# autosome-ru/pasio

Measured on NVIDIA B200. Metric: whole-contig segmentation throughput, default pasio pipeline (nt/s); DP cell updates/s in dp_cells_per_s, higher is better.
Workload: dtype f64

## Files before the change

include/pasio_b200.h:

```cpp
#ifndef PASIO_B200_H
#define PASIO_B200_H

#include <stdint.h>

#ifdef __cplusplus
extern "C" {
#endif

typedef struct pasio_ctx pasio_ctx;

typedef enum pasio_status {
    PASIO_OK = 0,
    PASIO_E_CUDA = -1,
    PASIO_E_ARG = -2,
    PASIO_E_COUNTS = -3,
    PASIO_E_CANDIDATES = -4,
    PASIO_E_TABLE_TOO_SHORT = -5,
    PASIO_E_STATE = -6,
    PASIO_E_TOO_LARGE = -7,
    PASIO_E_NOMEM = -8
} pasio_status;

enum { PASIO_TAB_LOG = 0,
       PASIO_TAB_LGAMMA = 1,
       PASIO_TAB_LGAMMA_ALPHA = 2   };

enum { PASIO_CONSTRAINT_NONE = 0, PASIO_CONSTRAINT_ZEROS = 1, PASIO_CONSTRAINT_CONSTANTS = 2 };

enum { PASIO_TUNE_WINDOW_PRUNE = 0,
       PASIO_TUNE_WINDOW_PHASES = 1,
       PASIO_TUNE_EXACT_PRUNE = 2,
       PASIO_TUNE_EXACT_LAG = 3,
       PASIO_TUNE_EXACT_RING = 4,
       PASIO_TUNE_LOGFAC_EXACT = 5,
       PASIO_TUNE_WINDOW_SPECULATE = 6,
       PASIO_TUNE_UPLOAD_NARROW = 7,
       PASIO_TUNE_LOGFAC_EAGER = 8,
       PASIO_TUNE_EXACT_NBLOCK = 9,
       PASIO_TUNE_COUNT = 10 };

int pasio_ctx_create(int device, pasio_ctx **out);
int pasio_ctx_destroy(pasio_ctx *ctx);
const char *pasio_last_error(const pasio_ctx *ctx);
int pasio_abi_version(void);

int pasio_set_params(pasio_ctx *ctx, int alpha_is_int, double alpha, double beta,
                     double segment_creation_cost);
int pasio_table_upload(pasio_ctx *ctx, int table_id, const double *values, int64_t n);
int pasio_table_need(const pasio_ctx *ctx, int64_t *n_log, int64_t *n_lgamma, int64_t *n_lgamma_alpha);

int pasio_contig_load(pasio_ctx *ctx, const int64_t *counts, int64_t n,
                      const int64_t *offsets, int64_t n_contigs);
int pasio_contig_load_rle(pasio_ctx *ctx, const int64_t *starts, const int64_t *values,
                          int64_t n_runs, const int64_t *offsets, int64_t n_contigs);
int pasio_contig_load_round(pasio_ctx *ctx, const int64_t *counts, int64_t n, int64_t window_size,
                            int64_t window_shift, int constraint, int64_t *n_in, int64_t *n_out, int64_t *cells);

int pasio_contig_load_device(pasio_ctx *ctx, const int64_t *d_counts_device, int64_t n,
                             const int64_t *offsets, int64_t n_contigs);
int pasio_contig_info(const pasio_ctx *ctx, int64_t *n, int64_t *total_count, int64_t *n_contigs);
int pasio_cumsum_at(pasio_ctx *ctx, const int64_t *positions, int64_t m, int64_t *out);

int pasio_candidates_set(pasio_ctx *ctx, const int64_t *cands, int64_t m);
int pasio_candidates_count(const pasio_ctx *ctx, int64_t *m);
int pasio_candidates_download(pasio_ctx *ctx, int64_t *out, int64_t capacity, int64_t *m);

int pasio_filter_candidates(pasio_ctx *ctx, int constraint, int64_t *n_in, int64_t *n_out);

int pasio_round(pasio_ctx *ctx, int64_t window_size, int64_t window_shift, int constraint,
                int64_t *n_in, int64_t *n_out, int64_t *cells);
int pasio_round_stats(const pasio_ctx *ctx, int64_t *cells, int64_t *cells_skipped);
int pasio_exact_task_plan(int64_t n_candidates, int lag, int nblock, int32_t *triples, int64_t cap, int64_t *n_tasks);
int pasio_upload_stats(const pasio_ctx *ctx, int64_t *wire_bytes);
int pasio_set_tuning(pasio_ctx *ctx, int key, int value);
int pasio_rounds(pasio_ctx *ctx, int64_t window_size, int64_t window_shift, int constraint,
                 int64_t max_rounds, int64_t *rounds_done, int64_t *n_out, int64_t *cells,
                 int64_t *sizes, int64_t sizes_cap);
int pasio_set_penalties(pasio_ctx *ctx, const double *split_number_penalty, int64_t n_split_number_penalty,
                        double first_column_refund, const double *length_penalty, int64_t n_length_penalty);

int pasio_square_split(pasio_ctx *ctx, int64_t *out_splits, int64_t cap, int64_t *n_splits,
                       double *score, double *prefix_scores, int64_t *previous_splits);
int pasio_square_split_regularized(pasio_ctx *ctx, const double *length_penalty, int64_t n_length_penalty,
                                   const double *split_number_penalty, int64_t n_split_number_penalty,
                                   double first_column_refund, int64_t *out_splits, int64_t cap, int64_t *n_splits,
                                   double *score, double *prefix_scores, int64_t *previous_splits);
int pasio_suffix_scores(pasio_ctx *ctx, int64_t stop, double *out);

int pasio_segment_scores(pasio_ctx *ctx, double *scores, int64_t *segment_counts,
                         double *mean_counts, double *logfac_cumsum, int64_t capacity,
                         int64_t *n_segments);

int pasio_segment_scores_sum(pasio_ctx *ctx, double *total);

int pasio_segment_lmm(pasio_ctx *ctx, double *lmm, int64_t capacity, double *sum_logfac);
int pasio_logfac_prefetch(pasio_ctx *ctx);

int pasio_host_alloc(int64_t bytes, void **out);
int pasio_host_free(void *ptr);

int64_t pasio_bedgraph_runs(const int64_t *starts, const int64_t *stops, const int64_t *counts,
                            const uint8_t *new_chrom, int64_t n, int split_at_gaps, int64_t *run_len,
                            int64_t *run_val, int64_t *group_line, int64_t *group_run, int64_t *n_runs);

int64_t pasio_bedgraph_count_lines(const char *buf, int64_t len);
int pasio_bedgraph_parse(const char *buf, int64_t len, int64_t cap, int64_t *starts, int64_t *stops,
                         int64_t *counts, int64_t *name_off, int32_t *name_len, uint8_t *new_chrom,
                         int64_t *n_out, int64_t *float_counts);
int64_t pasio_format_segments(const char *chrom, int64_t offset, const int64_t *splits, int64_t n_splits,
                              const double *means, const double *lmm, int mode, char *out, int64_t cap);

int64_t pasio_format_segments_batch(const char *names, const int64_t *name_off, const int64_t *shift,
                                    const int64_t *first_split, int64_t n_contigs, const int64_t *splits,
                                    const double *means, const double *lmm, int mode, char *out, int64_t cap);


int pasio_timing_reset(pasio_ctx *ctx, int enable);
void *pasio_stream(pasio_ctx *ctx);
int pasio_fp64_peak(pasio_ctx *ctx, double *instr_per_sec);
int pasio_timing_get(pasio_ctx *ctx, int family, double *ms, int64_t *launches);

#ifdef __cplusplus
}
#endif
#endif
```

pasio_b200/_native.py:

```python
import ctypes
import os
import threading

import numpy as np

_HERE = os.path.dirname(os.path.abspath(__file__))
LIB_PATH = os.environ.get('PASIO_B200_LIB') or os.path.join(_HERE, 'libpasio_b200.so')

OK = 0
E_CUDA, E_ARG, E_COUNTS, E_CANDIDATES, E_TABLE_TOO_SHORT, E_STATE, E_TOO_LARGE, E_NOMEM = range(-1, -9, -1)
TAB_LOG, TAB_LGAMMA, TAB_LGAMMA_ALPHA = 0, 1, 2
CONSTRAINTS = {'none': 0, 'zeros': 1, 'constants': 2}
TUNE = {'window_prune': 0, 'window_phases': 1, 'exact_prune': 2, 'exact_lag': 3, 'exact_ring': 4, 'logfac_exact': 5,
        'window_speculate': 6, 'upload_narrow': 7,
        'logfac_eager': 8, 'exact_nblock': 9}
TIMING_FAMILIES = ['scan', 'window_dp', 'compact', 'exact_dp', 'score', 'h2d', 'd2h']

_i64 = ctypes.c_int64
_i64p = ctypes.POINTER(ctypes.c_int64)
_f64p = ctypes.POINTER(ctypes.c_double)
_vp = ctypes.c_void_p

SIGNATURES = {
    'pasio_ctx_create': (ctypes.c_int, [ctypes.c_int, ctypes.POINTER(_vp)]),
    'pasio_ctx_destroy': (ctypes.c_int, [_vp]),
    'pasio_last_error': (ctypes.c_char_p, [_vp]),
    'pasio_abi_version': (ctypes.c_int, []),
    'pasio_set_params': (ctypes.c_int, [_vp, ctypes.c_int, ctypes.c_double, ctypes.c_double, ctypes.c_double]),
    'pasio_table_upload': (ctypes.c_int, [_vp, ctypes.c_int, _f64p, _i64]),
    'pasio_table_need': (ctypes.c_int, [_vp, _i64p, _i64p, _i64p]),
    'pasio_contig_load': (ctypes.c_int, [_vp, _i64p, _i64, _i64p, _i64]),
    'pasio_contig_load_round': (ctypes.c_int, [_vp, _i64p, _i64, _i64, _i64, ctypes.c_int, _i64p, _i64p, _i64p]),
    'pasio_contig_load_rle': (ctypes.c_int, [_vp, _i64p, _i64p, _i64, _i64p, _i64]),
    'pasio_contig_load_device': (ctypes.c_int, [_vp, _vp, _i64, _i64p, _i64]),
    'pasio_contig_info': (ctypes.c_int, [_vp, _i64p, _i64p, _i64p]),
    'pasio_cumsum_at': (ctypes.c_int, [_vp, _i64p, _i64, _i64p]),
    'pasio_candidates_set': (ctypes.c_int, [_vp, _i64p, _i64]),
    'pasio_candidates_count': (ctypes.c_int, [_vp, _i64p]),
    'pasio_candidates_download': (ctypes.c_int, [_vp, _i64p, _i64, _i64p]),
    'pasio_filter_candidates': (ctypes.c_int, [_vp, ctypes.c_int, _i64p, _i64p]),
    'pasio_round': (ctypes.c_int, [_vp, _i64, _i64, ctypes.c_int, _i64p, _i64p, _i64p]),
    'pasio_round_stats': (ctypes.c_int, [_vp, _i64p, _i64p]),
    'pasio_exact_task_plan': (ctypes.c_int, [_i64, ctypes.c_int, ctypes.c_int, ctypes.POINTER(ctypes.c_int32), _i64, _i64p]),
    'pasio_upload_stats': (ctypes.c_int, [_vp, _i64p]),
    'pasio_set_tuning': (ctypes.c_int, [_vp, ctypes.c_int, ctypes.c_int]),
    'pasio_rounds': (ctypes.c_int, [_vp, _i64, _i64, ctypes.c_int, _i64, _i64p, _i64p, _i64p, _i64p, _i64]),
    'pasio_set_penalties': (ctypes.c_int, [_vp, _f64p, _i64, ctypes.c_double, _f64p, _i64]),
    'pasio_square_split': (ctypes.c_int, [_vp, _i64p, _i64, _i64p, _f64p, _f64p, _i64p]),
    'pasio_square_split_regularized': (ctypes.c_int, [_vp, _f64p, _i64, _f64p, _i64, ctypes.c_double, _i64p, _i64, _i64p, _f64p,
                                                     _f64p, _i64p]),
    'pasio_suffix_scores': (ctypes.c_int, [_vp, _i64, _f64p]),
    'pasio_segment_scores': (ctypes.c_int, [_vp, _f64p, _i64p, _f64p, _f64p, _i64, _i64p]),
    'pasio_segment_scores_sum': (ctypes.c_int, [_vp, _f64p]),
    'pasio_segment_lmm': (ctypes.c_int, [_vp, _f64p, _i64, _f64p]),
    'pasio_logfac_prefetch': (ctypes.c_int, [_vp]),
    'pasio_host_alloc': (ctypes.c_int, [_i64, ctypes.POINTER(_vp)]),
    'pasio_host_free': (ctypes.c_int, [_vp]),
    'pasio_bedgraph_count_lines': (_i64, [ctypes.c_void_p, _i64]),
    'pasio_bedgraph_parse': (ctypes.c_int, [ctypes.c_void_p, _i64, _i64, _i64p, _i64p, _i64p, _i64p,
                                            ctypes.POINTER(ctypes.c_int32), ctypes.POINTER(ctypes.c_uint8), _i64p, _i64p]),
    'pasio_bedgraph_runs': (_i64, [_i64p, _i64p, _i64p, ctypes.POINTER(ctypes.c_uint8), _i64, ctypes.c_int, _i64p, _i64p, _i64p,
                                   _i64p, _i64p]),
    'pasio_format_segments': (_i64, [ctypes.c_char_p, _i64, _i64p, _i64, _f64p, _f64p, ctypes.c_int,
                                     ctypes.c_char_p, _i64]),
    'pasio_format_segments_batch': (_i64, [ctypes.c_char_p, _i64p, _i64p, _i64p, _i64, _i64p, _f64p, _f64p, ctypes.c_int,
                                           ctypes.c_char_p, _i64]),
    'pasio_timing_reset': (ctypes.c_int, [_vp, ctypes.c_int]),
    'pasio_timing_get': (ctypes.c_int, [_vp, ctypes.c_int, _f64p, _i64p]),
    'pasio_stream': (_vp, [_vp]),
    'pasio_fp64_peak': (ctypes.c_int, [_vp, _f64p]),
}

_lib = None
_lib_lock = threading.Lock()


def load_library():
    global _lib
    with _lib_lock:
        if _lib is None:
            if not os.path.exists(LIB_PATH):
                raise RuntimeError('pasio_b200: %s is missing -- build it with `python -c "import __graft_entry__ as g; '
                                   'g.build()"` or `make -C pasio_b200/csrc`; there is no CPU fallback' % LIB_PATH)
            lib = ctypes.CDLL(LIB_PATH)
            for name, (res, args) in SIGNATURES.items():
                fn = getattr(lib, name)
                fn.restype = res
                fn.argtypes = args
            _lib = lib
    return _lib


def _ptr(arr, ct):
    return arr.ctypes.data_as(ctypes.POINTER(ct))


class PasioDeviceError(RuntimeError):
    pass


class _PinnedPool(object):

    def __init__(self, lib):
        self.lib = lib
        self.free = {}
        self.lock = threading.Lock()
        self.total = 0

    @staticmethod
    def _capacity(nbytes):
        cap = 1 << 16
        while cap < nbytes:
            cap <<= 1
        return cap

    def empty(self, n, dtype):
        import weakref
        dtype = np.dtype(dtype)
        nbytes = max(1, int(n) * dtype.itemsize)
        cap = self._capacity(nbytes)
        with self.lock:
            bucket = self.free.get(cap)
            ptr = bucket.pop() if bucket else None
        if ptr is None:
            if self.total + cap > (8 << 30):
                return np.empty(int(n), dtype=dtype)
            out = _vp()
            if self.lib.pasio_host_alloc(cap, ctypes.byref(out)) != OK:
                return np.empty(int(n), dtype=dtype)
            ptr = out.value
            self.total += cap
        buf = (ctypes.c_char * cap).from_address(ptr)
        arr = np.frombuffer(buf, dtype=dtype, count=int(n))
        weakref.finalize(buf, self._give_back, cap, ptr)
        return arr

    def _give_back(self, cap, ptr):
        with self.lock:
            self.free.setdefault(cap, []).append(ptr)


class Engine(object):

    def __init__(self, device=0):
        self.lib = load_library()
        handle = _vp()
        rc = self.lib.pasio_ctx_create(int(device), ctypes.byref(handle))
        if rc != OK:
            raise PasioDeviceError('pasio_b200: cannot create a device context (%s); the LogML path has no CPU '
                                   'fallback' % self.lib.pasio_last_error(None).decode())
        self.ctx = handle
        self.device = device
        self._params = None
        self._tables = {}
        self._scorer_source = None
        self._penalty_spec = None
        self._penalties = None
        self._penalty_host = None
        self._loaded = None
        self._loaded_print = None
        self._cands_print = None
        self._loaded_offsets = None
        self._cands_obj = None
        self._pool = _PinnedPool(self.lib)

    def close(self):
        if self.ctx:
            self.lib.pasio_ctx_destroy(self.ctx)
            self.ctx = None

    def _check(self, rc):
        if rc == OK:
            return
        msg = self.lib.pasio_last_error(self.ctx).decode()
        if rc in (E_COUNTS, E_CANDIDATES):
            raise AssertionError(msg)
        if rc == E_ARG:
            raise ValueError(msg)
        if rc == E_NOMEM:
            raise MemoryError(msg)
        raise PasioDeviceError('pasio_b200 error %d: %s' % (rc, msg))

    def use_scorer(self, source, penalties=None):
        alpha = source.alpha
        is_int = isinstance(alpha, (int, np.integer)) and not isinstance(alpha, bool)
        params = (int(is_int), float(alpha), float(source.log_computer.shift), float(source.segment_creation_cost))
        if params != self._params:
            self._check(self.lib.pasio_set_params(self.ctx, *params))
            self._params = params
        comps = {TAB_LOG: source.log_computer, TAB_LGAMMA: source.log_gamma_computer,
                 TAB_LGAMMA_ALPHA: source.log_gamma_alpha_computer}
        for tid, comp in comps.items():
            have = self._tables.get(tid)
            if have is None or have[0] is not comp:
                self._upload_table(tid, comp, comp.cache_size)
# ... 47 lines not shown
        n = len(arr)
        if n == 0:
            return (0,)
        step = max(1, n // 4096)
        return (n, int(arr[0]), int(arr[-1]), int(np.asarray(arr[::step]).sum()))

    def load(self, counts, offsets=None):
        if (self._loaded is counts and offsets is None and self._loaded_offsets is None
                and self._loaded_print == self._fingerprint(counts)):
            return
        assert isinstance(counts, np.ndarray)
        assert counts.dtype == int
        assert len(counts) > 0
        c = np.ascontiguousarray(counts)
        self._loaded = None
        self._cands_obj = None
        if offsets is None:
            rc = self.lib.pasio_contig_load(self.ctx, _ptr(c, ctypes.c_int64), len(c), None, 1)
        else:
            off = np.ascontiguousarray(offsets, dtype=np.int64)
            rc = self.lib.pasio_contig_load(self.ctx, _ptr(c, ctypes.c_int64), len(c), _ptr(off, ctypes.c_int64),
                                            len(off) - 1)
        self._check(rc)
        self._loaded = counts
        self._loaded_print = self._fingerprint(counts)
        self._loaded_offsets = None if offsets is None else np.array(offsets, dtype=np.int64)

    def load_and_round(self, counts, window_size, window_shift, constraint, want_logfac=False):
        assert isinstance(counts, np.ndarray)
        assert counts.dtype == int
        assert len(counts) > 0
        c = np.ascontiguousarray(counts)
        self._loaded = None
        self._cands_obj = None
        n_in, n_out, cells = _i64(0), _i64(0), _i64(0)
        self.set_tuning('logfac_eager', 1 if want_logfac else 0)
        self._sync_penalties()
        try:
            rc = self.lib.pasio_contig_load_round(self.ctx, _ptr(c, ctypes.c_int64), len(c), window_size, window_shift,
                                                  CONSTRAINTS[constraint], ctypes.byref(n_in), ctypes.byref(n_out),
                                                  ctypes.byref(cells))
        finally:
            if want_logfac:
                self.set_tuning('logfac_eager', 0)
        if rc != E_TABLE_TOO_SHORT:
            self._check(rc)
        self._loaded = counts
        self._loaded_print = self._fingerprint(counts)
        self._loaded_offsets = None
        if rc == E_TABLE_TOO_SHORT:
            self._grow_tables()
            return self.round(window_size, window_shift, constraint)
        return n_in.value, n_out.value, cells.value

    def load_device(self, device_ptr, n, owner=None, offsets=None):
        self._loaded = None
        self._cands_obj = None
        if offsets is None:
            rc = self.lib.pasio_contig_load_device(self.ctx, _vp(device_ptr), n, None, 1)
        else:
            off = np.ascontiguousarray(offsets, dtype=np.int64)
            rc = self.lib.pasio_contig_load_device(self.ctx, _vp(device_ptr), n, _ptr(off, ctypes.c_int64), len(off) - 1)
        self._check(rc)
        self._loaded = owner if owner is not None else object()
        self._loaded_offsets = None if offsets is None else np.array(offsets, dtype=np.int64)

    def invalidate(self):
        self._loaded = None
        self._cands_obj = None

    def stream_handle(self):
        return self.lib.pasio_stream(self.ctx)

    def fp64_peak(self):
        v = ctypes.c_double(0)
        self._check(self.lib.pasio_fp64_peak(self.ctx, ctypes.byref(v)))
        return v.value

    def load_rle(self, starts, values, offsets=None):
        starts = np.ascontiguousarray(starts, dtype=np.int64)
        values = np.ascontiguousarray(values, dtype=np.int64)
        self._loaded = None
        self._cands_obj = None
        if offsets is None:
            rc = self.lib.pasio_contig_load_rle(self.ctx, _ptr(starts, ctypes.c_int64), _ptr(values, ctypes.c_int64),
                                                len(values), None, 1)
        else:
            off = np.ascontiguousarray(offsets, dtype=np.int64)
            rc = self.lib.pasio_contig_load_rle(self.ctx, _ptr(starts, ctypes.c_int64), _ptr(values, ctypes.c_int64),
                                                len(values), _ptr(off, ctypes.c_int64), len(off) - 1)
        self._check(rc)
        self._loaded = object()
        self._loaded_offsets = None if offsets is None else np.array(offsets, dtype=np.int64)

    def info(self):
        n, total, k = _i64(0), _i64(0), _i64(0)
        self._check(self.lib.pasio_contig_info(self.ctx, ctypes.byref(n), ctypes.byref(total), ctypes.byref(k)))
        return n.value, total.value, k.value

    def set_candidates(self, cands):
        if cands is None:
            self._check(self.lib.pasio_candidates_set(self.ctx, None, 0))
            self._cands_obj = None
            return
        if self._cands_obj is cands and self._cands_print == self._fingerprint(cands):
            return
        c = np.ascontiguousarray(cands, dtype=np.int64)
        self._cands_obj = None
        self._check(self.lib.pasio_candidates_set(self.ctx, _ptr(c, ctypes.c_int64), len(c)))
        self._cands_obj = cands
        self._cands_print = self._fingerprint(cands)

    def candidates(self):
        m = _i64(0)
        self._check(self.lib.pasio_candidates_count(self.ctx, ctypes.byref(m)))
        out = self._pool.empty(m.value, np.int64)
        self._check(self.lib.pasio_candidates_download(self.ctx, _ptr(out, ctypes.c_int64), len(out), None))
        self._cands_obj = out
        self._cands_print = self._fingerprint(out)
        return out

    def candidate_count(self):
        m = _i64(0)
        self._check(self.lib.pasio_candidates_count(self.ctx, ctypes.byref(m)))
        return m.value

    def filter_candidates(self, constraint):
        a, b = _i64(0), _i64(0)
        self._cands_obj = None
        self._check(self.lib.pasio_filter_candidates(self.ctx, CONSTRAINTS[constraint], ctypes.byref(a), ctypes.byref(b)))
        return a.value, b.value

    def round(self, window_size, window_shift, constraint):
        n_in, n_out, cells = _i64(0), _i64(0), _i64(0)
        self._cands_obj = None
        self._sync_penalties()
        self._retry(lambda: self.lib.pasio_round(self.ctx, window_size, window_shift, CONSTRAINTS[constraint],
                                                 ctypes.byref(n_in), ctypes.byref(n_out), ctypes.byref(cells)))
        return n_in.value, n_out.value, cells.value

    def set_tuning(self, key, value):
        self._check(self.lib.pasio_set_tuning(self.ctx, TUNE[key], int(value)))

    def upload_stats(self):
        b = _i64(0)
        self._check(self.lib.pasio_upload_stats(self.ctx, ctypes.byref(b)))
        return b.value

    def round_stats(self):
        a, b = _i64(0), _i64(0)
        self._check(self.lib.pasio_round_stats(self.ctx, ctypes.byref(a), ctypes.byref(b)))
        return a.value, b.value

    def rounds(self, window_size, window_shift, constraint, num_rounds=None, first=None):
        n, _, _ = self.info()
        limit = max(1, n if num_rounds is None else num_rounds)
        self._cands_obj = None
        sizes, cells_total = [], 0
        if first is not None:
            sizes.append(first[0])
            cells_total += first[2]
            limit -= 1
            if first[0] == first[1] or limit == 0:
                return sizes, self.candidate_count(), cells_total
        while limit > 0:
            done, n_out, cells = _i64(0), _i64(0), _i64(0)
            buf = np.zeros(64, dtype=np.int64)
            step = min(limit, 64)
            self._sync_penalties()
            rc = self.lib.pasio_rounds(self.ctx, window_size, window_shift, CONSTRAINTS[constraint], step,
                                       ctypes.byref(done), ctypes.byref(n_out), ctypes.byref(cells),
                                       _ptr(buf, ctypes.c_int64), len(buf))
            sizes.extend(buf[:done.value].tolist())
            cells_total += cells.value
            limit -= done.value
            if rc == E_TABLE_TOO_SHORT:
                self._grow_tables()
                continue
            self._check(rc)
            if done.value < step or (done.value > 0 and sizes[-1] == n_out.value):
                break
        return sizes, self.candidate_count(), cells_total

    def _check_exact_limits(self):
        n, total, _ = self.info()
        if total + (self._params[1] if self._params else 0) >= 2 ** 31 - 2:
            raise PasioDeviceError('pasio_b200: the exact SquareSplitter DP over a whole contig needs the total count (%d) below '
                                   '2^31; use the default `rounds` algorithm for deep-coverage contigs' % total)

    def square_split(self, want_arrays=False):
        self._check_exact_limits()
        m = self.candidate_count()
        splits = np.empty(m, dtype=np.int64)
        n_splits, score = _i64(0), ctypes.c_double(0.0)
        P = np.empty(m) if want_arrays else None
        prev = np.empty(m, dtype=np.int64) if want_arrays else None
        self._cands_obj = None
        self._retry(lambda: self.lib.pasio_square_split(
            self.ctx, _ptr(splits, ctypes.c_int64), m, ctypes.byref(n_splits), ctypes.byref(score),
            _ptr(P, ctypes.c_double) if want_arrays else None,
            _ptr(prev, ctypes.c_int64) if want_arrays else None))
        out = splits[:n_splits.value].copy()
        self._cands_obj = out
        self._cands_print = self._fingerprint(out)
        if want_arrays:
            return np.float64(score.value), out, P, prev
        return np.float64(score.value), out

    def square_split_regularized(self, length_penalty=None, split_number_penalty=None, first_column_refund=0.0):
        self._check_exact_limits()
        m = self.candidate_count()
        splits = np.empty(m, dtype=np.int64)
        n_splits, score = _i64(0), ctypes.c_double(0.0)
        lp = None if length_penalty is None else np.ascontiguousarray(length_penalty, dtype=np.float64)
        sp = None if split_number_penalty is None else np.ascontiguousarray(split_number_penalty, dtype=np.float64)
        self._cands_obj = None
        self._retry(lambda: self.lib.pasio_square_split_regularized(
            self.ctx, None if lp is None else _ptr(lp, ctypes.c_double), 0 if lp is None else len(lp),
            None if sp is None else _ptr(sp, ctypes.c_double), 0 if sp is None else len(sp), float(first_column_refund),
            _ptr(splits, ctypes.c_int64), m, ctypes.byref(n_splits), ctypes.byref(score), None, None))
        out = splits[:n_splits.value].copy()
        self._cands_obj = out
        self._cands_print = self._fingerprint(out)
        return np.float64(score.value), out

    def suffix_scores(self, stop):
        out = np.empty(stop)
        if stop > 0:
            self._retry(lambda: self.lib.pasio_suffix_scores(self.ctx, stop, _ptr(out, ctypes.c_double)))
        return out

    def cumsum_at_candidates(self):
        m = self.candidate_count()
        out = np.empty(m, dtype=np.int64)
        self._check(self.lib.pasio_cumsum_at(self.ctx, None, m, _ptr(out, ctypes.c_int64)))
        return out

    def segment_scores(self, scores=True, counts=False, means=False, logfac=False):
        m = self.candidate_count()
        nseg = m - 1
        s = self._pool.empty(nseg, np.float64) if scores else None
        c = self._pool.empty(nseg, np.int64) if counts else None
        mu = self._pool.empty(nseg, np.float64) if means else None
        lf = self._pool.empty(m, np.float64) if logfac else None
        nout = _i64(0)
        self._retry(lambda: self.lib.pasio_segment_scores(
            self.ctx, _ptr(s, ctypes.c_double) if scores else None, _ptr(c, ctypes.c_int64) if counts else None,
            _ptr(mu, ctypes.c_double) if means else None, _ptr(lf, ctypes.c_double) if logfac else None,
            max(nseg, m if logfac else 0), ctypes.byref(nout)))
        return s, c, mu, lf

    def segment_scores_sum(self):
        total = ctypes.c_double(0.0)
        self._retry(lambda: self.lib.pasio_segment_scores_sum(self.ctx, ctypes.byref(total)))
        return np.float64(total.value)

    def logfac_prefetch(self):
        self._check(self.lib.pasio_logfac_prefetch(self.ctx))

    def segment_lmm(self):
        nseg = self.candidate_count() - 1
        out = self._pool.empty(nseg, np.float64)
        total = ctypes.c_double(0.0)
        self._retry(lambda: self.lib.pasio_segment_lmm(self.ctx, _ptr(out, ctypes.c_double), nseg, ctypes.byref(total)))
        return out, total.value

    def timing_reset(self, enable=True):
        self._check(self.lib.pasio_timing_reset(self.ctx, int(enable)))

    def timing(self):
        out = {}
        for k, name in enumerate(TIMING_FAMILIES):
            ms, n = ctypes.c_double(0), _i64(0)
            self._check(self.lib.pasio_timing_get(self.ctx, k, ctypes.byref(ms), ctypes.byref(n)))
            out[name] = (ms.value, n.value)
        return out


def parse_bedgraph_text(data, front=0, length=None):
    lib = load_library()
    nbytes = len(data) if length is None else int(length)
    if isinstance(data, bytearray):
        data = (ctypes.c_char * len(data)).from_buffer(data) if len(data) else None
    cap = lib.pasio_bedgraph_count_lines(data, nbytes)
    starts = np.empty(front + cap, dtype=np.int64)
    stops = np.empty(front + cap, dtype=np.int64)
    counts = np.empty(front + cap, dtype=np.int64)
    name_off = np.empty(front + cap, dtype=np.int64)
    name_len = np.empty(front + cap, dtype=np.int32)
    new_chrom = np.empty(front + cap, dtype=np.uint8)
    n, nfloat = _i64(0), _i64(0)
    rc = lib.pasio_bedgraph_parse(data, nbytes, cap, _ptr(starts[front:], ctypes.c_int64), _ptr(stops[front:], ctypes.c_int64),
                                  _ptr(counts[front:], ctypes.c_int64), _ptr(name_off[front:], ctypes.c_int64),
                                  _ptr(name_len[front:], ctypes.c_int32), _ptr(new_chrom[front:], ctypes.c_uint8),
                                  ctypes.byref(n), ctypes.byref(nfloat))
    if rc != OK:
        raise ValueError('malformed bedgraph line %d (need: chrom start stop count)' % (n.value + 1))
    k = front + n.value
    return dict(starts=starts[:k], stops=stops[:k], counts=counts[:k], name_off=name_off[:k], name_len=name_len[:k],
                new_chrom=new_chrom[:k], n_float=nfloat.value)


def bedgraph_runs(rec, split_at_gaps):
    lib = load_library()
    n = len(rec['starts'])
    run_len = np.empty(2 * n, dtype=np.int64)
# ... 87 lines not shown
```

pasio_b200/csrc/api.cu:

```cuda
#include "common.cuh"

#include <algorithm>
#include <thread>
#include <atomic>
#include <chrono>
#include <memory>
#include <cstdarg>
#include <cstdlib>
#include <cstdio>
#include <cstring>

static thread_local std::string g_create_error;

int pasio_fail(pasio_ctx *ctx, int code, const char *fmt, ...)
{
    char buf[512];
    va_list ap;
    va_start(ap, fmt);
    vsnprintf(buf, sizeof buf, fmt, ap);
    va_end(ap);
    if (ctx) ctx->err = buf; else g_create_error = buf;
    return code;
}

// ... 234 lines not shown
    }

    void work(int t)
    {
        cudaSetDevice(ctx->device);
        bool used[2] = {false, false};
        int which = 0;
        while (!cancel.load(std::memory_order_relaxed)) {
            const i64 sidx = next_slice.fetch_add(1);
            if (sidx >= n_slices) break;
            const i64 e0 = sidx * (i64)SLICE, e1 = std::min<i64>(n, e0 + (i64)SLICE), len = e1 - e0;
            const int buf = 2 * t + which;
            which ^= 1;
            int32_t *hst = (int32_t *)ctx->nstage_host + (size_t)buf * SLICE;
            int32_t *dev = (int32_t *)ctx->nstage_dev + (size_t)buf * SLICE;
            i64 *dst = ctx->counts.as<i64>() + e0;
            bool ok = true;
            if (plain_mode.load(std::memory_order_relaxed)) {
                ok = cudaMemcpyAsync(dst, src + e0, (size_t)len * 8, cudaMemcpyHostToDevice, ctx->stream_copy) == cudaSuccess;
                wire_bytes.fetch_add(len * 8);
                which ^= 1;
                if (!ok) { cudaGetLastError(); failed.store(1); cancel.store(1); }
                const i64 qp = e0 / chunk_elems;
                if (left_in_chunk[(size_t)qp].fetch_sub(1) == 1) {
                    if (cudaEventRecord(ctx->chunk_events[(size_t)qp], ctx->stream_copy) != cudaSuccess) { cudaGetLastError(); failed.store(1); }
                    recorded[(size_t)qp].store(1, std::memory_order_release);
                }
                continue;
            }
            if (used[buf & 1]) ok = cudaEventSynchronize(ctx->nstage_free[(size_t)buf]) == cudaSuccess;
            const uint64_t bits = ok ? pasio_narrow_slice8(reinterpret_cast<uint8_t *>(hst), src + e0, (size_t)len) : 0;
            const bool sw = limit_bits < 25;
            const int lim8 = sw ? limit_bits : 8, lim16 = sw ? limit_bits + 3 : 16, lim32 = sw ? limit_bits + 6 : 31;
            if (ok && (bits >> lim8) == 0 && (len & 15) == 0) {
                ok = cudaMemcpyAsync(dev, hst, (size_t)len, cudaMemcpyHostToDevice, ctx->stream_copy) == cudaSuccess;
                if (ok) {
                    ok = cudaEventRecord(ctx->nstage_free[(size_t)buf], ctx->stream_copy) == cudaSuccess;
                    used[buf & 1] = true;
                    const i64 n16 = len / 16;
                    widen_counts8_kernel<<<(unsigned)std::min<i64>((n16 + 255) / 256, 296), 256, 0, ctx->stream_copy>>>(
                        reinterpret_cast<const uint4 *>(dev), reinterpret_cast<longlong2 *>(dst), n16);
                    ok = ok && cudaGetLastError() == cudaSuccess;
                    wire_bytes.fetch_add(len);
                }
            } else if (ok && (bits >> lim16) == 0 && (len & 7) == 0) {
                pasio_narrow_slice16(reinterpret_cast<uint16_t *>(hst), src + e0, (size_t)len);
                ok = cudaMemcpyAsync(dev, hst, (size_t)len * 2, cudaMemcpyHostToDevice, ctx->stream_copy) == cudaSuccess;
                if (ok) {
                    ok = cudaEventRecord(ctx->nstage_free[(size_t)buf], ctx->stream_copy) == cudaSuccess;
                    used[buf & 1] = true;
                    const i64 n8 = len / 8;
                    widen_counts16_kernel<<<(unsigned)std::min<i64>((n8 + 255) / 256, 296), 256, 0, ctx->stream_copy>>>(
                        reinterpret_cast<const uint4 *>(dev), reinterpret_cast<longlong2 *>(dst), n8);
                    ok = ok && cudaGetLastError() == cudaSuccess;
                    wire_bytes.fetch_add(len * 2);
                }
            } else if (ok && (bits >> lim32) == 0 && (len & 3) == 0) {
                narrow_slice(hst, src + e0, (size_t)len);
                ok = cudaMemcpyAsync(dev, hst, (size_t)len * 4, cudaMemcpyHostToDevice, ctx->stream_copy) == cudaSuccess;
                if (ok) {
                    ok = cudaEventRecord(ctx->nstage_free[(size_t)buf], ctx->stream_copy) == cudaSuccess;
                    used[buf & 1] = true;
                    const i64 n4 = len / 4;
                    widen_counts_kernel<<<(unsigned)std::min<i64>((n4 + 255) / 256, 296), 256, 0, ctx->stream_copy>>>(
                        reinterpret_cast<const int4 *>(dev), reinterpret_cast<longlong2 *>(dst), n4);
                    ok = ok && cudaGetLastError() == cudaSuccess;
                    wire_bytes.fetch_add(len * 4);
                }
            } else if (ok) {
                ok = cudaMemcpyAsync(dst, src + e0, (size_t)len * 8, cudaMemcpyHostToDevice, ctx->stream_copy) == cudaSuccess;
                wire_bytes.fetch_add(len * 8);
            }
            if (!ok) { cudaGetLastError(); failed.store(1); cancel.store(1); }
            if (src_pinned && packed_elems.fetch_add(len) + len >= ((i64)64 << 20) && !decided.exchange(1)) {
                const double secs = std::chrono::duration<double>(std::chrono::steady_clock::now() - t_start).count();
                if ((double)packed_elems.load() * 8.0 < PLAIN_RATE * secs) plain_mode.store(1);
            }
            const i64 q = e0 / chunk_elems;
            if (left_in_chunk[(size_t)q].fetch_sub(1) == 1) {
                if (cudaEventRecord(ctx->chunk_events[(size_t)q], ctx->stream_copy) != cudaSuccess) { cudaGetLastError(); failed.store(1); }
                recorded[(size_t)q].store(1, std::memory_order_release);
            }
        }
    }

    bool wait_recorded(i64 q)
    {
        while (!recorded[(size_t)q].load(std::memory_order_acquire)) {
            if (failed.load() || cancel.load()) return false;
            std::this_thread::sleep_for(std::chrono::microseconds(20));
        }
        return !failed.load();
    }

    void finish()
    {
        for (auto &th : threads) th.join();
        threads.clear();
    }
    ~NarrowUpload()
    {
        if (!threads.empty()) { cancel.store(1); finish(); }
    }
};
}

static void drop_borrowed_counts(pasio_ctx *ctx)
{
    if (ctx->counts_borrowed) { ctx->counts.p = nullptr; ctx->counts.bytes = 0; ctx->counts_borrowed = false; }
}

#define NEED_CTX(ctx) do { if (!(ctx)) return PASIO_E_ARG; cudaSetDevice((ctx)->device); } while (0)

extern "C" int pasio_abi_version(void) { return PASIO_ABI_VERSION; }

extern "C" const char *pasio_last_error(const pasio_ctx *ctx)
{
    return ctx ? ctx->err.c_str() : g_create_error.c_str();
}

extern "C" int pasio_ctx_create(int device, pasio_ctx **out)
{
    if (!out) return pasio_fail(nullptr, PASIO_E_ARG, "out is NULL");
    *out = nullptr;
    int count = 0;
    cudaError_t e = cudaGetDeviceCount(&count);
    if (e != cudaSuccess || count == 0)
        return pasio_fail(nullptr, PASIO_E_CUDA, "no CUDA device: %s (pasio_b200 has no CPU fallback)",
                          e != cudaSuccess ? cudaGetErrorString(e) : "device count is 0");
    if (device < 0 || device >= count)
        return pasio_fail(nullptr, PASIO_E_ARG, "device %d out of range (have %d)", device, count);
    cudaDeviceProp prop;
    e = cudaGetDeviceProperties(&prop, device);
    if (e != cudaSuccess) return pasio_fail(nullptr, PASIO_E_CUDA, "cudaGetDeviceProperties: %s", cudaGetErrorString(e));
    if (prop.major != 10)
        return pasio_fail(nullptr, PASIO_E_CUDA, "device %d is sm_%d%d; this library is built for sm_100a only",
                          device, prop.major, prop.minor);
    e = cudaSetDevice(device);
    if (e != cudaSuccess) return pasio_fail(nullptr, PASIO_E_CUDA, "cudaSetDevice: %s", cudaGetErrorString(e));
    pasio_ctx *ctx = new pasio_ctx();
    ctx->device = device;
    ctx->sm_count = prop.multiProcessorCount;
    ctx->smem_optin = (int)prop.sharedMemPerBlockOptin;
    int prio_lo = 0, prio_hi = 0;
    cudaDeviceGetStreamPriorityRange(&prio_lo, &prio_hi);
    if (cudaStreamCreateWithPriority(&ctx->stream, cudaStreamNonBlocking, prio_hi) != cudaSuccess ||
        cudaStreamCreateWithPriority(&ctx->stream2, cudaStreamNonBlocking, 0) != cudaSuccess ||
        cudaStreamCreateWithFlags(&ctx->stream_copy, cudaStreamNonBlocking) != cudaSuccess ||
        cudaStreamCreateWithPriority(&ctx->stream_lx, cudaStreamNonBlocking, 0) != cudaSuccess ||
        cudaEventCreateWithFlags(&ctx->ev_lx0, cudaEventDisableTiming) != cudaSuccess ||
        cudaEventCreateWithFlags(&ctx->ev_lx1, cudaEventDisableTiming) != cudaSuccess ||
        cudaEventCreateWithFlags(&ctx->ev_fork, cudaEventDisableTiming) != cudaSuccess ||
        cudaEventCreateWithFlags(&ctx->ev_join, cudaEventDisableTiming) != cudaSuccess ||
        cudaMallocHost((void **)&ctx->h_scalars, 16 * sizeof(i64)) != cudaSuccess ||
        pasio_reserve(ctx, ctx->scalars, 16 * sizeof(i64)) != PASIO_OK) {
        g_create_error = "context allocation failed: " + ctx->err;
        delete ctx;
        return PASIO_E_CUDA;
    }
    memset(ctx->h_scalars, 0, 16 * sizeof(i64));
    auto env_int = [](const char *name, int dflt) { const char *v = getenv(name); return v ? atoi(v) : dflt; };
    ctx->tune[PASIO_TUNE_WINDOW_PRUNE] = env_int("PASIO_WD_PRUNE", 1);
    ctx->tune[PASIO_TUNE_WINDOW_PHASES] = env_int("PASIO_WD_PHASES", 1);
    ctx->tune[PASIO_TUNE_EXACT_PRUNE] = env_int("PASIO_XD_PRUNE", 1);
    ctx->tune[PASIO_TUNE_EXACT_LAG] = env_int("PASIO_XD_LAG", 5);
    ctx->tune[PASIO_TUNE_EXACT_RING] = env_int("PASIO_XD_RING", 1);
    ctx->tune[PASIO_TUNE_LOGFAC_EXACT] = env_int("PASIO_B200_EXACT_LMM", 1);
    ctx->tune[PASIO_TUNE_WINDOW_SPECULATE] = env_int("PASIO_WD_SPECULATE", 1);
    ctx->tune[PASIO_TUNE_UPLOAD_NARROW] = env_int("PASIO_B200_UPLOAD_NARROW", 1);
    ctx->tune[PASIO_TUNE_LOGFAC_EAGER] = env_int("PASIO_B200_LOGFAC_EAGER", 0);
    ctx->tune[PASIO_TUNE_EXACT_NBLOCK] = env_int("PASIO_XD_NBLOCK", 3);
    if (ctx->tune[PASIO_TUNE_EXACT_LAG] < 3 || ctx->tune[PASIO_TUNE_EXACT_LAG] > 5) ctx->tune[PASIO_TUNE_EXACT_LAG] = 5;
    *out = ctx;
    return PASIO_OK;
}

extern "C" int pasio_ctx_destroy(pasio_ctx *ctx)
{
    if (!ctx) return PASIO_OK;
    cudaSetDevice(ctx->device);
    cudaStreamSynchronize(ctx->stream);
    drop_borrowed_counts(ctx);
    DevBuf *bufs[] = {&ctx->tab[0], &ctx->tab[1], &ctx->tab[2], &ctx->counts, &ctx->cg, &ctx->cpbits, &ctx->keepbits,
                      &ctx->bounds, &ctx->brank, &ctx->cand[0], &ctx->cand[1], &ctx->candC[0], &ctx->candC[1], &ctx->win_st, &ctx->win_en, &ctx->win_small, &ctx->win_medium, &ctx->win_large, &ctx->win_flags,
                      &ctx->blocksum, &ctx->tilestate, &ctx->scalars, &ctx->dpL, &ctx->dpC, &ctx->dpP, &ctx->dpPrev,
                      &ctx->dpPart, &ctx->dpPartArg, &ctx->dpMark, &ctx->dpJump, &ctx->fscan, &ctx->logfac_full,
                      &ctx->xpRing, &ctx->xpRec, &ctx->xpTasks, &ctx->regLR, &ctx->regNR, &ctx->lxPos, &ctx->lxSum, &ctx->lxFirst, &ctx->lxState};
    for (DevBuf *b : bufs) if (b->p) cudaFree(b->p);
    for (auto &s : ctx->spans) { cudaEventDestroy(s.a); cudaEventDestroy(s.b); }
    for (auto e : ctx->event_pool) cudaEventDestroy(e);
    if (ctx->h_scalars) cudaFreeHost(ctx->h_scalars);
    for (int k = 0; k < 3; ++k) {
        if (ctx->stage[k]) cudaFreeHost(ctx->stage[k]);
        if (k == 0) {
            if (ctx->nstage_host) cudaFreeHost(ctx->nstage_host);
            if (ctx->nstage_dev) cudaFree(ctx->nstage_dev);
            for (cudaEvent_t e : ctx->nstage_free) cudaEventDestroy(e);
        }
        if (ctx->stage_free[k]) cudaEventDestroy(ctx->stage_free[k]);
    }
    if (ctx->ev_fork) cudaEventDestroy(ctx->ev_fork);
    if (ctx->ev_join) cudaEventDestroy(ctx->ev_join);
    if (ctx->stream2) cudaStreamDestroy(ctx->stream2);
    if (ctx->stream_copy) cudaStreamDestroy(ctx->stream_copy);
    if (ctx->stream_lx) { cudaStreamSynchronize(ctx->stream_lx); cudaStreamDestroy(ctx->stream_lx); }
    if (ctx->ev_lx0) cudaEventDestroy(ctx->ev_lx0);
    if (ctx->ev_lx1) cudaEventDestroy(ctx->ev_lx1);
    for (auto e : ctx->chunk_events) cudaEventDestroy(e);
    cudaStreamDestroy(ctx->stream);
    delete ctx;
    return PASIO_OK;
}

extern "C" int pasio_set_params(pasio_ctx *ctx, int alpha_is_int, double alpha, double beta, double pen)
{
    NEED_CTX(ctx);
    if (!(alpha >= 0) || !(beta >= 0)) return pasio_fail(ctx, PASIO_E_ARG, "alpha and beta must be >= 0");
    if (alpha_is_int && (alpha != (double)(i64)alpha || alpha > 1e9))
        return pasio_fail(ctx, PASIO_E_ARG, "alpha_is_int set but alpha=%g is not a small integer", alpha);
    ctx->alpha_is_int = alpha_is_int ? 1 : 0;
    ctx->alpha = alpha;
    ctx->alpha_int = alpha_is_int ? (i64)alpha : 0;
    ctx->beta = beta;
    ctx->pen = pen;
    ctx->have_params = true;
    return PASIO_OK;
}

extern "C" int pasio_table_upload(pasio_ctx *ctx, int id, const double *values, int64_t n)
{
    NEED_CTX(ctx);
    if (id < 0 || id > 2 || !values || n < 1) return pasio_fail(ctx, PASIO_E_ARG, "bad table upload (id=%d n=%lld)", id, (long long)n);
    PASIO_TRY(pasio_reserve(ctx, ctx->tab[id], (size_t)n * 8));
    PASIO_TRY(h2d(ctx, ctx->tab[id].p, values, (size_t)n * 8));
    CUDA_TRY(ctx, cudaStreamSynchronize(ctx->stream));
    ctx->ntab[id] = n;
    return PASIO_OK;
}

extern "C" int pasio_table_need(const pasio_ctx *ctx, int64_t *n_log, int64_t *n_lgamma, int64_t *n_lgamma_alpha)
{
    if (!ctx) return PASIO_E_ARG;
    if (n_log) *n_log = ctx->need[PASIO_TAB_LOG];
    if (n_lgamma) *n_lgamma = ctx->need[PASIO_TAB_LGAMMA];
    if (n_lgamma_alpha) *n_lgamma_alpha = ctx->need[PASIO_TAB_LGAMMA_ALPHA];
    return PASIO_OK;
}

static bool penalties_on(const pasio_ctx *ctx) { return ctx->pen_num || ctx->pen_len; }

static int check_dp_tables(pasio_ctx *ctx, i64 max_span, i64 max_cnt, bool with_penalties = false)
{
    if (!ctx->have_params) return pasio_fail(ctx, PASIO_E_STATE, "pasio_set_params has not been called");
    if (max_cnt + ctx->alpha_int >= 2147483647LL)
        return pasio_fail(ctx, PASIO_E_TOO_LARGE, "count %lld does not fit the 32-bit DP index", (long long)max_cnt);
    const i64 need_log = max_span + 1;
    const int gid = ctx->alpha_is_int ? PASIO_TAB_LGAMMA : PASIO_TAB_LGAMMA_ALPHA;
    const i64 need_g = max_cnt + ctx->alpha_int + 1;
    bool bad = false;
    if (ctx->ntab[PASIO_TAB_LOG] < need_log) { ctx->need[PASIO_TAB_LOG] = need_log; bad = true; }
    if (ctx->ntab[gid] < need_g) { ctx->need[gid] = need_g; bad = true; }
    if (with_penalties && ctx->pen_len && ctx->n_pen_lr < need_log) { ctx->need[PASIO_TAB_LOG] = need_log; bad = true; }
    if (bad)
        return pasio_fail(ctx, PASIO_E_TABLE_TOO_SHORT, "tables too short: need log>=%lld, lgamma[%d]>=%lld (have %lld, %lld%s)",
                          (long long)need_log, gid, (long long)need_g, (long long)ctx->ntab[PASIO_TAB_LOG],
                          (long long)ctx->ntab[gid], with_penalties && ctx->pen_len ? ", length penalty as long as log" : "");
    return PASIO_OK;
}

extern "C" int pasio_set_penalties(pasio_ctx *ctx, const double *split_number_penalty, int64_t n_split_number_penalty,
                                   double first_column_refund, const double *length_penalty, int64_t n_length_penalty)
{
    NEED_CTX(ctx);
    if ((split_number_penalty && n_split_number_penalty < 1) || (length_penalty && n_length_penalty < 1))
        return pasio_fail(ctx, PASIO_E_ARG, "a penalty table needs at least one entry");
    ctx->pen_num = ctx->pen_len = false;
    if (split_number_penalty) {
        PASIO_TRY(pasio_reserve(ctx, ctx->penNR, (size_t)n_split_number_penalty * 8));
        PASIO_TRY(h2d(ctx, ctx->penNR.p, split_number_penalty, (size_t)n_split_number_penalty * 8));
    }
    if (length_penalty) {
        PASIO_TRY(pasio_reserve(ctx, ctx->penLR, (size_t)n_length_penalty * 8));
        PASIO_TRY(h2d(ctx, ctx->penLR.p, length_penalty, (size_t)n_length_penalty * 8));
    }
    CUDA_TRY(ctx, cudaStreamSynchronize(ctx->stream));
    ctx->pen_num = split_number_penalty != nullptr;
    ctx->n_pen_nr = ctx->pen_num ? n_split_number_penalty : 0;
    ctx->pen_refund = ctx->pen_num ? first_column_refund : 0.0;
    ctx->pen_len = length_penalty != nullptr;
    ctx->n_pen_lr = ctx->pen_len ? n_length_penalty : 0;
    return PASIO_OK;
}

static int finish_load(pasio_ctx *ctx, const int64_t *offsets, int64_t n_contigs)
{
    const i64 n = ctx->n;
    ctx->h_bounds.resize((size_t)n_contigs + 1);
    if (offsets) {
        for (i64 c = 0; c <= n_contigs; ++c) {
            if (offsets[c] < 0 || offsets[c] > n || (c > 0 && offsets[c] <= offsets[c - 1]))
                return pasio_fail(ctx, PASIO_E_ARG, "contig offsets must be strictly ascending within [0, n] (empty contigs are not allowed)");
            ctx->h_bounds[(size_t)c] = (int32_t)offsets[c];
        }
        if (offsets[0] != 0 || offsets[n_contigs] != n)
            return pasio_fail(ctx, PASIO_E_ARG, "offsets[0] must be 0 and offsets[n_contigs] must be n");
    } else {
        ctx->h_bounds[0] = 0;
        ctx->h_bounds[1] = (int32_t)n;
    }
    ctx->n_contigs = n_contigs;
    const size_t bit_bytes = (size_t)((n + 1 + 4095) / 4096) * 512 + 16;
    PASIO_TRY(pasio_reserve(ctx, ctx->cg, (size_t)(n + 2) * 8));
    PASIO_TRY(pasio_reserve(ctx, ctx->cpbits, bit_bytes));
// ... 120 lines not shown
    if (window_size < 1 || window_shift < 1 || window_size > 2147483000LL || window_shift > 2147483000LL)
        return pasio_fail(ctx, PASIO_E_ARG, "window_size and window_shift must be positive");
    if (constraint < 0 || constraint > 2) return pasio_fail(ctx, PASIO_E_ARG, "unknown constraint %d", constraint);
    PASIO_TRY(check_load_args(ctx, n, nullptr, 1));
    ctx->n = n;
    drop_borrowed_counts(ctx);
    PASIO_TRY(pasio_reserve(ctx, ctx->counts, (size_t)n * 8 + 16));
    ctx->h_bounds.assign({0, (int32_t)n});
    ctx->n_contigs = 1;
    const size_t bit_alloc = (size_t)((n + 1 + 4095) / 4096) * 512 + 16;
    PASIO_TRY(pasio_reserve(ctx, ctx->cg, (size_t)(n + 2) * 8));
    PASIO_TRY(pasio_reserve(ctx, ctx->cpbits, bit_alloc));
    PASIO_TRY(pasio_reserve(ctx, ctx->keepbits, bit_alloc));
    PASIO_TRY(pasio_reserve(ctx, ctx->bounds, 2 * 4));
    PASIO_TRY(pasio_reserve(ctx, ctx->brank, 2 * 4));
    PASIO_TRY(h2d(ctx, ctx->bounds.p, ctx->h_bounds.data(), 2 * 4));
    const size_t bit_bytes = (size_t)((n + 1 + 31) / 32 + 2) * 4;
    CUDA_TRY(ctx, cudaMemsetAsync(ctx->keepbits.p, 0, bit_bytes, ctx->stream));
    i64 n_tiles = 0, tile_elems = 0;
    PASIO_TRY(launch_scan_prepare(ctx, &n_tiles, &tile_elems));
    ctx->implicit_all = true;
    ctx->m = n + 1;
    ctx->cur = 0;
    ctx->n_small = ctx->n_medium = ctx->n_large = -1;

    const i64 chunk_tiles = (i64)(32 << 20) / tile_elems;
    const i64 n_chunks = (n_tiles + chunk_tiles - 1) / chunk_tiles;
    while ((i64)ctx->chunk_events.size() < n_chunks) {
        cudaEvent_t e;
        CUDA_TRY(ctx, cudaEventCreateWithFlags(&e, cudaEventDisableTiming));
        ctx->chunk_events.push_back(e);
    }
    CUDA_TRY(ctx, cudaEventRecord(ctx->ev_fork, ctx->stream));
    CUDA_TRY(ctx, cudaStreamWaitEvent(ctx->stream_copy, ctx->ev_fork, 0));
    i64 queued = 0;
    auto queue_copies = [&](i64 upto) -> int {
        for (; queued < upto && queued < n_chunks; ++queued) {
            const i64 e0 = queued * chunk_tiles * tile_elems, e1 = std::min<i64>(n, (queued + 1) * chunk_tiles * tile_elems);
            if (e1 > e0) {
                TimingScope ts(ctx, TF_H2D, 1, ctx->stream_copy);
                PASIO_TRY(upload(ctx, ctx->counts.as<i64>() + e0, counts + e0, (size_t)(e1 - e0) * 8, ctx->stream_copy));
            }
            CUDA_TRY(ctx, cudaEventRecord(ctx->chunk_events[(size_t)queued], ctx->stream_copy));
        }
        return PASIO_OK;
    };

    const bool eager = ctx->tune[PASIO_TUNE_LOGFAC_EXACT] && ctx->tune[PASIO_TUNE_LOGFAC_EAGER] && ctx->ntab[PASIO_TAB_LGAMMA] > 2;
    if (eager) {
        CUDA_TRY(ctx, cudaStreamWaitEvent(ctx->stream_lx, ctx->ev_fork, 0));
        PASIO_TRY(launch_logfac_exact_begin(ctx, ctx->stream_lx));
    }
    NarrowUpload narrow;
    std::unique_ptr<TimingScope> narrow_span;
    bool narrow_on = false;
    if (ctx->tune[PASIO_TUNE_UPLOAD_NARROW] && n >= ((i64)1 << 24) && (chunk_tiles * tile_elems) % (i64)NarrowUpload::SLICE == 0) {
        narrow_span.reset(new TimingScope(ctx, TF_H2D, 1, ctx->stream_copy));
        if (ctx->tune[PASIO_TUNE_UPLOAD_NARROW] >= 2 && ctx->tune[PASIO_TUNE_UPLOAD_NARROW] < 31) narrow.limit_bits = ctx->tune[PASIO_TUNE_UPLOAD_NARROW];
        narrow_on = narrow.start(ctx, counts, n, chunk_tiles * tile_elems, n_chunks) == 0;
        if (!narrow_on) narrow_span.reset();
    }
    auto stop_upload = [&]() {
        if (narrow_on) { narrow.cancel.store(1); narrow.finish(); narrow_span.reset(); }
        if (eager) cudaStreamSynchronize(ctx->stream_lx);
    };

    const i64 nwin_total = (ctx->m - 1 + window_shift - 1) / window_shift;
    i64 w_done = 0;
    int table_rc = ctx->have_params ? PASIO_OK : pasio_fail(ctx, PASIO_E_STATE, "pasio_set_params has not been called");
    bool first_dp = true;
    for (i64 c = 0; c < n_chunks; ++c) {
        if (narrow_on) {
            if (!narrow.wait_recorded(c)) {
                stop_upload();
                cudaStreamSynchronize(ctx->stream_copy);
                return pasio_fail(ctx, PASIO_E_CUDA, "narrowed upload failed: %s", cudaGetErrorString(cudaGetLastError()));
            }
        } else {
            PASIO_TRY(queue_copies(c + 3));
        }
        CUDA_TRY(ctx, cudaStreamWaitEvent(ctx->stream, ctx->chunk_events[(size_t)c], 0));
        if (eager) {
            CUDA_TRY(ctx, cudaStreamWaitEvent(ctx->stream_lx, ctx->chunk_events[(size_t)c], 0));
            PASIO_TRY(launch_logfac_exact_chunk(ctx, c * chunk_tiles * tile_elems, std::min<i64>(n, (c + 1) * chunk_tiles * tile_elems),
                                                ctx->stream_lx));
        }
        const i64 t1 = std::min<i64>(n_tiles, (c + 1) * chunk_tiles);
        PASIO_TRY(launch_scan_tiles(ctx, t1 - c * chunk_tiles));
        const i64 scanned = t1 * tile_elems;
        i64 w_ready = nwin_total;
        if (c + 1 < n_chunks) {
            w_ready = scanned > window_size ? (scanned - window_size - 1) / window_shift + 1 : 0;
            if (w_ready > nwin_total) w_ready = nwin_total;
        }
        if (table_rc == PASIO_OK && w_ready > w_done) {
            i64 max_span = 0, max_cnt = 0;
            CUDA_TRY(ctx, cudaMemcpyAsync(ctx->h_scalars + 1, ctx->scalars.as<i64>() + 1, 8, cudaMemcpyDeviceToHost, ctx->stream));
            PASIO_TRY(launch_window_prepass(ctx, w_ready - w_done, (int)window_size, (int)window_shift, &max_span, &max_cnt,
                                            constraint, w_done));
            if (ctx->h_scalars[1]) {
                stop_upload();
                cudaStreamSynchronize(ctx->stream_copy);
                return pasio_fail(ctx, PASIO_E_COUNTS, "counts must be >= 0");
            }
            table_rc = check_dp_tables(ctx, max_span, max_cnt, true);
            if (table_rc == PASIO_OK) {
                if (penalties_on(ctx))
                    PASIO_TRY(launch_window_dp_reg(ctx, w_ready - w_done, (int)window_size, (int)window_shift, constraint, !first_dp));
                else
                    PASIO_TRY(launch_window_dp(ctx, w_ready - w_done, (int)window_size, (int)window_shift, constraint, w_done,
                                               !first_dp));
                first_dp = false;
            } else if (table_rc != PASIO_E_TABLE_TOO_SHORT) {
                return table_rc;
            }
            w_done = w_ready;
        }
    }
    if (narrow_on) {
        narrow.finish();
        narrow_span.reset();
        ctx->last_wire_bytes = narrow.wire_bytes.load();
        if (narrow.failed.load()) {
            cudaStreamSynchronize(ctx->stream_copy);
            return pasio_fail(ctx, PASIO_E_CUDA, "narrowed upload failed: %s", cudaGetErrorString(cudaGetLastError()));
        }
    } else {
        ctx->last_wire_bytes = n * 8;
    }
    PASIO_TRY(d2h(ctx, ctx->h_scalars, ctx->scalars.p, 3 * sizeof(i64)));
    CUDA_TRY(ctx, cudaStreamSynchronize(ctx->stream_copy));
    if (ctx->h_scalars[1]) return pasio_fail(ctx, PASIO_E_COUNTS, "counts must be >= 0");
    ctx->total = ctx->h_scalars[0];
    ctx->max_count = ctx->h_scalars[2];
    ctx->have_contig = true;
    if (eager) {
        CUDA_TRY(ctx, cudaEventRecord(ctx->ev_lx1, ctx->stream_lx));
        ctx->logfac_ready = true;
        ctx->logfac_is_exact = true;
        ctx->logfac_pending = true;
        ctx->logfac_eager = true;
    }
    PASIO_TRY(launch_boundary_ranks(ctx));
    ctx->h_brank = ctx->h_bounds;
    if (n_in) *n_in = ctx->m;
    if (n_out) *n_out = ctx->m;
    if (cells) *cells = 0;
    if (table_rc != PASIO_OK) return table_rc;

    const int nxt = 1 - ctx->cur;
    PASIO_TRY(pasio_reserve(ctx, ctx->cand[nxt], (size_t)ctx->m * 4));
    i64 m_new = 0;
    PASIO_TRY(launch_compact_keepbits(ctx, nxt, &m_new));
    PASIO_TRY(d2h(ctx, ctx->h_scalars + 10, ctx->scalars.as<i64>() + 10, 24));
    if (cells) *cells = ctx->h_scalars[10];
    ctx->last_cells = ctx->h_scalars[10];
    ctx->last_cells_skipped = ctx->h_scalars[12];
    ctx->cur = nxt;
    ctx->implicit_all = false;
    ctx->m = m_new;
    if (n_out) *n_out = m_new;
    return refresh_boundary_ranks(ctx);
}

extern "C" int pasio_contig_info(const pasio_ctx *ctx, int64_t *n, int64_t *total_count, int64_t *n_contigs)
{
    if (!ctx || !ctx->have_contig) return PASIO_E_STATE;
    if (n) *n = ctx->n;
    if (total_count) *total_count = ctx->total;
    if (n_contigs) *n_contigs = ctx->n_contigs;
    return PASIO_OK;
}

extern "C" int pasio_cumsum_at(pasio_ctx *ctx, const int64_t *positions, int64_t m, int64_t *out)
{
    NEED_CTX(ctx);
    if (!ctx->have_contig) return pasio_fail(ctx, PASIO_E_STATE, "no contig loaded");
    if (m < 0 || !out) return pasio_fail(ctx, PASIO_E_ARG, "bad arguments");
    if (m == 0) return PASIO_OK;
    PASIO_TRY(pasio_reserve(ctx, ctx->dpP, (size_t)m * 8));
    if (positions) {
        for (i64 k = 0; k < m; ++k)
            if (positions[k] < 0 || positions[k] > ctx->n) return pasio_fail(ctx, PASIO_E_ARG, "position out of range");
        PASIO_TRY(pasio_reserve(ctx, ctx->dpJump, (size_t)m * 8));
        PASIO_TRY(h2d(ctx, ctx->dpJump.p, positions, (size_t)m * 8));
        PASIO_TRY(launch_gather_i64(ctx, ctx->cg.as<i64>(), nullptr, ctx->dpJump.as<i64>(), m, ctx->dpP.as<i64>()));
    } else {
        if (m != ctx->m) return pasio_fail(ctx, PASIO_E_ARG, "m must equal the candidate count");
        PASIO_TRY(launch_gather_i64(ctx, ctx->cg.as<i64>(), cur_cand(ctx), nullptr, m, ctx->dpP.as<i64>()));
    }
    return d2h(ctx, out, ctx->dpP.p, (size_t)m * 8);
}

__global__ void narrow_candidates_kernel(const i64 *__restrict__ in, i64 m, i64 n, int32_t *__restrict__ out, i64 *bad)
{
    for (i64 k = (i64)blockIdx.x * blockDim.x + threadIdx.x; k < m; k += (i64)gridDim.x * blockDim.x) {
        i64 v = in[k];
        if (v < 0 || v > n) { *bad = 1; v = 0; }
        out[k] = (int32_t)v;
    }
}

static int refresh_boundary_ranks(pasio_ctx *ctx)
{
    PASIO_TRY(launch_boundary_ranks(ctx));
    if (ctx->n_contigs > 1) {
        ctx->h_brank.resize((size_t)ctx->n_contigs + 1);
        PASIO_TRY(d2h(ctx, ctx->h_brank.data(), ctx->brank.p, (size_t)(ctx->n_contigs + 1) * 4));
    }
    return PASIO_OK;
}

extern "C" int pasio_candidates_set(pasio_ctx *ctx, const int64_t *cands, int64_t m)
{
    NEED_CTX(ctx);
    if (!ctx->have_contig) return pasio_fail(ctx, PASIO_E_STATE, "no contig loaded");
    if (!cands) {
        ctx->implicit_all = true;
        ctx->m = ctx->n + 1;
        return refresh_boundary_ranks(ctx);
    }
    if (m < 2 || m > ctx->n + 1) return pasio_fail(ctx, PASIO_E_CANDIDATES, "need 2 <= len(candidates) <= n+1");
    PASIO_TRY(pasio_reserve(ctx, ctx->dpJump, (size_t)m * 8));
    PASIO_TRY(pasio_reserve(ctx, ctx->cand[ctx->cur], (size_t)m * 4));
    PASIO_TRY(h2d(ctx, ctx->dpJump.p, cands, (size_t)m * 8));
    i64 *d_bad = ctx->scalars.as<i64>() + 5;
    CUDA_TRY(ctx, cudaMemsetAsync(d_bad, 0, 8, ctx->stream));
    narrow_candidates_kernel<<<ctx->sm_count * 4, 256, 0, ctx->stream>>>(ctx->dpJump.as<i64>(), m, ctx->n,
                                                                        ctx->cand[ctx->cur].as<int32_t>(), d_bad);
    CUDA_TRY(ctx, cudaGetLastError());
    PASIO_TRY(d2h(ctx, ctx->h_scalars + 5, d_bad, 8));
    if (ctx->h_scalars[5]) { ctx->implicit_all = true; ctx->m = ctx->n + 1; return pasio_fail(ctx, PASIO_E_CANDIDATES, "candidate out of range"); }
    ctx->implicit_all = false;
    ctx->m = m;
    PASIO_TRY(pasio_reserve(ctx, ctx->candC[ctx->cur], (size_t)m * 8));
    PASIO_TRY(launch_gather_i64(ctx, ctx->cg.as<i64>(), ctx->cand[ctx->cur].as<int32_t>(), nullptr, m, ctx->candC[ctx->cur].as<i64>()));
    PASIO_TRY(refresh_boundary_ranks(ctx));
    i64 bad = 0;
    PASIO_TRY(launch_validate_candidates(ctx, &bad));
    if (bad) {
        ctx->implicit_all = true;
        ctx->m = ctx->n + 1;
        refresh_boundary_ranks(ctx);
        return pasio_fail(ctx, PASIO_E_CANDIDATES,
                          "candidates must start at 0, end at len(counts), ascend strictly and contain every contig boundary");
    }
    return PASIO_OK;
}

extern "C" int pasio_candidates_count(const pasio_ctx *ctx, int64_t *m)
{
    if (!ctx || !ctx->have_contig || !m) return PASIO_E_STATE;
    *m = ctx->m;
    return PASIO_OK;
}

__global__ void widen_candidates_kernel(const int32_t *__restrict__ in, i64 m, i64 *__restrict__ out)
{
    for (i64 k = (i64)blockIdx.x * blockDim.x + threadIdx.x; k < m; k += (i64)gridDim.x * blockDim.x)
        out[k] = in ? (i64)in[k] : k;
}

extern "C" int pasio_candidates_download(pasio_ctx *ctx, int64_t *out, int64_t capacity, int64_t *m)
{
    NEED_CTX(ctx);
    if (!ctx->have_contig) return pasio_fail(ctx, PASIO_E_STATE, "no contig loaded");
    if (m) *m = ctx->m;
    if (!out) return PASIO_OK;
    if (capacity < ctx->m) return pasio_fail(ctx, PASIO_E_ARG, "capacity %lld < %lld candidates", (long long)capacity, (long long)ctx->m);
    PASIO_TRY(pasio_reserve(ctx, ctx->dpJump, (size_t)ctx->m * 8));
    widen_candidates_kernel<<<ctx->sm_count * 4, 256, 0, ctx->stream>>>(cur_cand(ctx), ctx->m, ctx->dpJump.as<i64>());
    CUDA_TRY(ctx, cudaGetLastError());
    return d2h(ctx, out, ctx->dpJump.p, (size_t)ctx->m * 8);
}

extern "C" int pasio_filter_candidates(pasio_ctx *ctx, int constraint, int64_t *n_in, int64_t *n_out)
{
    NEED_CTX(ctx);
    if (!ctx->have_contig) return pasio_fail(ctx, PASIO_E_STATE, "no contig loaded");
    if (ctx->n_contigs != 1) return pasio_fail(ctx, PASIO_E_STATE, "pasio_filter_candidates works on a single-contig context");
    if (constraint < 0 || constraint > 2) return pasio_fail(ctx, PASIO_E_ARG, "unknown constraint %d", constraint);
    if (n_in) *n_in = ctx->m;
    PASIO_TRY(launch_filter_candidates(ctx, constraint));
    const int nxt = 1 - ctx->cur;
    PASIO_TRY(pasio_reserve(ctx, ctx->cand[nxt], (size_t)ctx->m * 4));
    i64 m_new = 0;
    PASIO_TRY(launch_compact_keepbits(ctx, nxt, &m_new));
    ctx->cur = nxt;
    ctx->implicit_all = false;
    ctx->m = m_new;
    if (n_out) *n_out = m_new;
    return refresh_boundary_ranks(ctx);
}

static int build_window_table(pasio_ctx *ctx, i64 wsize, i64 wshift, i64 *nwin_out)
{
    if (ctx->n_contigs == 1) {
        *nwin_out = (ctx->m - 1 + wshift - 1) / wshift;
        return PASIO_OK;
    }
    ctx->h_win_st.clear();
    ctx->h_win_en.clear();
    for (i64 c = 0; c < ctx->n_contigs; ++c) {
        const i64 b0 = ctx->h_brank[(size_t)c], b1 = ctx->h_brank[(size_t)c + 1];
        const i64 mc = b1 - b0 + 1;
        for (i64 st = 0; st < mc - 1; st += wshift) {
            i64 en = st + wsize + 1;
            if (en > mc) en = mc;
            ctx->h_win_st.push_back((int32_t)(b0 + st));
            ctx->h_win_en.push_back((int32_t)(b0 + en));
        }
    }
    const size_t nw = ctx->h_win_st.size();
    PASIO_TRY(pasio_reserve(ctx, ctx->win_st, nw * 4));
    PASIO_TRY(pasio_reserve(ctx, ctx->win_en, nw * 4));
    PASIO_TRY(h2d(ctx, ctx->win_st.p, ctx->h_win_st.data(), nw * 4));
    PASIO_TRY(h2d(ctx, ctx->win_en.p, ctx->h_win_en.data(), nw * 4));
    CUDA_TRY(ctx, cudaStreamSynchronize(ctx->stream));
    *nwin_out = (i64)nw;
    return PASIO_OK;
}

extern "C" int pasio_round(pasio_ctx *ctx, int64_t window_size, int64_t window_shift, int constraint,
                           int64_t *n_in, int64_t *n_out, int64_t *cells)
{
    NEED_CTX(ctx);
    if (!ctx->have_contig) return pasio_fail(ctx, PASIO_E_STATE, "no contig loaded");
    if (window_size < 1 || window_shift < 1 || window_size > 2147483000LL || window_shift > 2147483000LL)
        return pasio_fail(ctx, PASIO_E_ARG, "window_size and window_shift must be positive");
    if (constraint < 0 || constraint > 2) return pasio_fail(ctx, PASIO_E_ARG, "unknown constraint %d", constraint);
    if (n_in) *n_in = ctx->m;
    if (n_out) *n_out = ctx->m;
    if (cells) *cells = 0;
    i64 nwin = 0;
    PASIO_TRY(build_window_table(ctx, window_size, window_shift, &nwin));
    i64 max_span = 0, max_cnt = 0;
    PASIO_TRY(launch_window_prepass(ctx, nwin, (int)window_size, (int)window_shift, &max_span, &max_cnt, constraint));
    static const bool debug = getenv("PASIO_DEBUG") != nullptr;
    if (debug)
        fprintf(stderr, "[pasio_round] n=%lld contigs=%lld m=%lld implicit=%d nwin=%lld size=%lld shift=%lld max_span=%lld max_cnt=%lld ntab=%lld,%lld,%lld\n",
                (long long)ctx->n, (long long)ctx->n_contigs, (long long)ctx->m, (int)ctx->implicit_all, (long long)nwin,
                (long long)window_size, (long long)window_shift, (long long)max_span, (long long)max_cnt,
                (long long)ctx->ntab[0], (long long)ctx->ntab[1], (long long)ctx->ntab[2]);
    if (max_cnt > ctx->total || max_span > ctx->n)
        return pasio_fail(ctx, PASIO_E_CUDA, "internal inconsistency before the window DP: window count %lld / span %lld exceed "
                          "contig total %lld / length %lld (m=%lld, implicit=%d, windows=%lld)", (long long)max_cnt,
                          (long long)max_span, (long long)ctx->total, (long long)ctx->n, (long long)ctx->m,
                          (int)ctx->implicit_all, (long long)nwin);
    PASIO_TRY(check_dp_tables(ctx, max_span, max_cnt, true));

    const size_t bit_bytes = (size_t)((ctx->n + 1 + 31) / 32 + 2) * 4;
    CUDA_TRY(ctx, cudaMemsetAsync(ctx->keepbits.p, 0, bit_bytes, ctx->stream));
    if (penalties_on(ctx)) PASIO_TRY(launch_window_dp_reg(ctx, nwin, (int)window_size, (int)window_shift, constraint));
    else PASIO_TRY(launch_window_dp(ctx, nwin, (int)window_size, (int)window_shift, constraint));

    const int nxt = 1 - ctx->cur;
    PASIO_TRY(pasio_reserve(ctx, ctx->cand[nxt], (size_t)ctx->m * 4));
    i64 m_new = 0;
    PASIO_TRY(launch_compact_keepbits(ctx, nxt, &m_new));
    PASIO_TRY(d2h(ctx, ctx->h_scalars + 10, ctx->scalars.as<i64>() + 10, 24));
    if (cells) *cells = ctx->h_scalars[10];
    ctx->last_cells = ctx->h_scalars[10];
    ctx->last_cells_skipped = ctx->h_scalars[12];
    ctx->cur = nxt;
    ctx->implicit_all = false;
    ctx->m = m_new;
    if (n_out) *n_out = m_new;
    return refresh_boundary_ranks(ctx);
}

extern "C" int pasio_rounds(pasio_ctx *ctx, int64_t window_size, int64_t window_shift, int constraint,
                            int64_t max_rounds, int64_t *rounds_done, int64_t *n_out, int64_t *cells,
                            int64_t *sizes, int64_t sizes_cap)
{
    NEED_CTX(ctx);
    if (!ctx->have_contig) return pasio_fail(ctx, PASIO_E_STATE, "no contig loaded");
    i64 limit = max_rounds <= 0 ? ctx->n : max_rounds;
    if (limit < 1) limit = 1;
    i64 done = 0, total_cells = 0;
    int rc = PASIO_OK;
    while (done < limit) {
        int64_t a = 0, b = 0, c = 0;
        rc = pasio_round(ctx, window_size, window_shift, constraint, &a, &b, &c);
        if (rc != PASIO_OK) break;
        if (sizes && done < sizes_cap) sizes[done] = a;
        ++done;
        total_cells += c;
        if (a == b) break;
    }
    if (rounds_done) *rounds_done = done;
    if (n_out) *n_out = ctx->m;
    if (cells) *cells = total_cells;
    return rc;
}

extern "C" int pasio_upload_stats(const pasio_ctx *ctx, int64_t *wire_bytes)
{
    if (!ctx || !wire_bytes) return PASIO_E_ARG;
    *wire_bytes = ctx->last_wire_bytes;
    return PASIO_OK;
}

extern "C" int pasio_round_stats(const pasio_ctx *ctx, int64_t *cells, int64_t *cells_skipped)
{
    if (!ctx) return PASIO_E_ARG;
    if (cells) *cells = ctx->last_cells;
    if (cells_skipped) *cells_skipped = ctx->last_cells_skipped;
    return PASIO_OK;
}

extern "C" int pasio_set_tuning(pasio_ctx *ctx, int key, int value)
{
    if (!ctx) return PASIO_E_ARG;
    if (key < 0 || key >= PASIO_TUNE_COUNT) return pasio_fail(ctx, PASIO_E_ARG, "unknown tuning key %d", key);
    if (key == PASIO_TUNE_EXACT_LAG && (value < 3 || value > 5)) return pasio_fail(ctx, PASIO_E_ARG, "exact lag must be 3, 4 or 5");
    ctx->tune[key] = value;
    if (key == PASIO_TUNE_LOGFAC_EXACT) {
        if (ctx->logfac_pending) { cudaStreamSynchronize(ctx->stream_lx); ctx->logfac_pending = false; }
        ctx->logfac_ready = false;
        ctx->logfac_eager = false;
    }
    return PASIO_OK;
}

static int finish_square_split(pasio_ctx *ctx, i64 N, int64_t *out_splits, int64_t cap, int64_t *n_splits, double *score,
                               double *prefix_scores, int64_t *previous_splits)
{
    if (score) PASIO_TRY(d2h(ctx, score, ctx->dpP.as<double>() + (N - 1), 8));
    if (prefix_scores) PASIO_TRY(d2h(ctx, prefix_scores, ctx->dpP.p, (size_t)N * 8));
    if (previous_splits) {
        std::vector<int> tmp((size_t)N);
        PASIO_TRY(d2h(ctx, tmp.data(), ctx->dpPrev.p, (size_t)N * 4));
        for (i64 k = 0; k < N; ++k) previous_splits[k] = tmp[(size_t)k];
    }
    PASIO_TRY(launch_backtrace_mark(ctx, N));
    const int nxt = 1 - ctx->cur;
    PASIO_TRY(pasio_reserve(ctx, ctx->cand[nxt], (size_t)N * 4));
    i64 m_new = 0;
    PASIO_TRY(launch_compact_keepbits(ctx, nxt, &m_new));
    ctx->cur = nxt;
    ctx->implicit_all = false;
    ctx->m = m_new;
    PASIO_TRY(refresh_boundary_ranks(ctx));
    if (n_splits) *n_splits = m_new;
    if (out_splits) {
        if (cap < m_new) return pasio_fail(ctx, PASIO_E_ARG, "capacity %lld < %lld splits", (long long)cap, (long long)m_new);
        return pasio_candidates_download(ctx, out_splits, cap, nullptr);
    }
    return PASIO_OK;
}

extern "C" int pasio_square_split(pasio_ctx *ctx, int64_t *out_splits, int64_t cap, int64_t *n_splits,
                                  double *score, double *prefix_scores, int64_t *previous_splits)
{
    NEED_CTX(ctx);
    if (!ctx->have_contig) return pasio_fail(ctx, PASIO_E_STATE, "no contig loaded");
    if (ctx->n_contigs != 1) return pasio_fail(ctx, PASIO_E_STATE, "pasio_square_split works on a single-contig context");
    const i64 N = ctx->m;
    PASIO_TRY(check_dp_tables(ctx, ctx->n, ctx->total));
    PASIO_TRY(launch_gather_candidates(ctx));
    PASIO_TRY(launch_exact_dp(ctx, N));
    return finish_square_split(ctx, N, out_splits, cap, n_splits, score, prefix_scores, previous_splits);
}

extern "C" int pasio_square_split_regularized(pasio_ctx *ctx, const double *length_penalty, int64_t n_length_penalty,
                                              const double *split_number_penalty, int64_t n_split_number_penalty,
                                              double first_column_refund, int64_t *out_splits, int64_t cap, int64_t *n_splits,
                                              double *score, double *prefix_scores, int64_t *previous_splits)
{
    NEED_CTX(ctx);
    if (!ctx->have_contig) return pasio_fail(ctx, PASIO_E_STATE, "no contig loaded");
    if (ctx->n_contigs != 1) return pasio_fail(ctx, PASIO_E_STATE, "pasio_square_split_regularized works on a single-contig context");
    const i64 N = ctx->m;
    if (length_penalty && n_length_penalty < ctx->n + 1)
        return pasio_fail(ctx, PASIO_E_ARG, "length penalty table needs %lld entries (0 .. contig length)", (long long)(ctx->n + 1));
    if (split_number_penalty && n_split_number_penalty < N)
        return pasio_fail(ctx, PASIO_E_ARG, "split-number penalty table needs %lld entries (one per candidate)", (long long)N);
    PASIO_TRY(check_dp_tables(ctx, ctx->n, ctx->total));
    PASIO_TRY(launch_gather_candidates(ctx));
    const double *d_lr = nullptr, *d_nr = nullptr;
    if (length_penalty) {
        PASIO_TRY(pasio_reserve(ctx, ctx->regLR, (size_t)(ctx->n + 1) * 8));
        PASIO_TRY(h2d(ctx, ctx->regLR.p, length_penalty, (size_t)(ctx->n + 1) * 8));
        d_lr = ctx->regLR.as<double>();
    }
    if (split_number_penalty) {
        PASIO_TRY(pasio_reserve(ctx, ctx->regNR, (size_t)N * 8));
        PASIO_TRY(h2d(ctx, ctx->regNR.p, split_number_penalty, (size_t)N * 8));
        d_nr = ctx->regNR.as<double>();
    }
    PASIO_TRY(launch_regularized_dp(ctx, N, d_lr, d_nr, first_column_refund));
    CUDA_TRY(ctx, cudaStreamSynchronize(ctx->stream));
    return finish_square_split(ctx, N, out_splits, cap, n_splits, score, prefix_scores, previous_splits);
}

extern "C" int pasio_suffix_scores(pasio_ctx *ctx, int64_t stop, double *out)
{
    NEED_CTX(ctx);
    if (!ctx->have_contig) return pasio_fail(ctx, PASIO_E_STATE, "no contig loaded");
    if (stop < 0 || stop >= ctx->m || !out) return pasio_fail(ctx, PASIO_E_ARG, "stop out of range");
    if (stop == 0) return PASIO_OK;
    i64 ends[2] = {0, stop};
    i64 pos[2] = {0, stop};
    if (!ctx->implicit_all) {
        int32_t p32[2];
        PASIO_TRY(d2h(ctx, &p32[0], ctx->cand[ctx->cur].as<int32_t>() + ends[0], 4));
        PASIO_TRY(d2h(ctx, &p32[1], ctx->cand[ctx->cur].as<int32_t>() + ends[1], 4));
        pos[0] = p32[0];
        pos[1] = p32[1];
    }
    i64 c[2];
    PASIO_TRY(d2h(ctx, &c[0], ctx->cg.as<i64>() + pos[0], 8));
    PASIO_TRY(d2h(ctx, &c[1], ctx->cg.as<i64>() + pos[1], 8));
    PASIO_TRY(check_dp_tables(ctx, pos[1] - pos[0], c[1] - c[0]));
    PASIO_TRY(pasio_reserve(ctx, ctx->dpP, (size_t)stop * 8));
    PASIO_TRY(launch_suffix_row(ctx, stop, ctx->dpP.as<double>()));
    return d2h(ctx, out, ctx->dpP.p, (size_t)stop * 8);
}

static int ensure_logfac(pasio_ctx *ctx)
{
    if (ctx->logfac_pending) {
        CUDA_TRY(ctx, cudaStreamWaitEvent(ctx->stream, ctx->ev_lx1, 0));
        ctx->logfac_pending = false;
    }
    if (ctx->logfac_eager) {
        ctx->logfac_eager = false;
        CUDA_TRY(ctx, cudaEventSynchronize(ctx->ev_lx1));
        bool usable = false;
        PASIO_TRY(logfac_exact_chunks_result(ctx, &usable));
        if (!usable) ctx->logfac_ready = false;
    }
    if (ctx->logfac_ready) return PASIO_OK;
    if (ctx->tune[PASIO_TUNE_LOGFAC_EXACT]) {
        PASIO_TRY(launch_logfac_exact(ctx));
    } else {
        PASIO_TRY(pasio_reserve(ctx, ctx->logfac_full, (size_t)(ctx->n + 1) * 8));
        PASIO_TRY(launch_logfac_scan(ctx, ctx->logfac_full.as<double>()));
    }
    ctx->logfac_ready = true;
    ctx->logfac_is_exact = ctx->tune[PASIO_TUNE_LOGFAC_EXACT] != 0;
    return PASIO_OK;
}

extern "C" int pasio_logfac_prefetch(pasio_ctx *ctx)
{
    NEED_CTX(ctx);
    if (!ctx->have_contig) return pasio_fail(ctx, PASIO_E_STATE, "no contig loaded");
    if (ctx->logfac_ready || ctx->logfac_pending || !ctx->tune[PASIO_TUNE_LOGFAC_EXACT]) return PASIO_OK;
    if (ctx->max_count + 2 > ctx->ntab[PASIO_TAB_LGAMMA]) return PASIO_OK;
    CUDA_TRY(ctx, cudaEventRecord(ctx->ev_lx0, ctx->stream));
    CUDA_TRY(ctx, cudaStreamWaitEvent(ctx->stream_lx, ctx->ev_lx0, 0));
    PASIO_TRY(launch_logfac_exact(ctx, ctx->stream_lx));
    CUDA_TRY(ctx, cudaEventRecord(ctx->ev_lx1, ctx->stream_lx));
    ctx->logfac_ready = true;
    ctx->logfac_is_exact = true;
    ctx->logfac_pending = true;
    return PASIO_OK;
}

// ... 204 lines not shown
```

pasio_b200/csrc/common.cuh:

```cuda
#pragma once

#include <cuda_runtime.h>
#include <stdint.h>
#include <string>
#include <vector>

#include "../../include/pasio_b200.h"

typedef long long i64;
typedef unsigned long long u64;

#define PASIO_ABI_VERSION 1

struct DevBuf {
    void *p = nullptr;
    size_t bytes = 0;
    template <typename T> T *as() const { return reinterpret_cast<T *>(p); }
};

enum TimingFamily { TF_SCAN = 0, TF_WINDOW_DP = 1, TF_COMPACT = 2, TF_EXACT_DP = 3, TF_SCORE = 4,
                    TF_H2D = 5, TF_D2H = 6, TF_COUNT = 7 };

struct TimedSpan { int family; cudaEvent_t a, b; };

struct pasio_ctx {
    int device = 0;
    int sm_count = 0;
    int smem_optin = 0;
    cudaStream_t stream = nullptr;
    cudaStream_t stream2 = nullptr;
    cudaEvent_t ev_fork = nullptr, ev_join = nullptr;
    cudaStream_t stream_copy = nullptr;
    cudaStream_t stream_lx = nullptr;
    cudaEvent_t ev_lx0 = nullptr, ev_lx1 = nullptr;
    bool logfac_eager = false;
    bool logfac_pending = false;
    std::vector<cudaEvent_t> chunk_events;
    void *stage[3] = {nullptr, nullptr, nullptr};
    cudaEvent_t stage_free[3] = {nullptr, nullptr, nullptr};
    bool stage_used[3] = {false, false, false};
    int stage_next = 0;
    void *nstage_host = nullptr;
    void *nstage_dev = nullptr;
    std::vector<cudaEvent_t> nstage_free;
    int nstage_threads = 0;
    i64 last_wire_bytes = 0;
    std::string err;

    bool have_params = false;
    int alpha_is_int = 1;
    i64 alpha_int = 1;
    double alpha = 1.0, beta = 1.0, pen = 0.0;

    DevBuf tab[3];
    i64 ntab[3] = {0, 0, 0};
    i64 need[3] = {0, 0, 0};

    bool have_contig = false;
    i64 n = 0;
    i64 total = 0;
    i64 max_count = 0;
    bool logfac_ready = false;
    bool logfac_is_exact = false;
    i64 n_contigs = 0;
    std::vector<int32_t> h_bounds;
    DevBuf counts;
    bool counts_borrowed = false;
    DevBuf cg;
    DevBuf cpbits;
    DevBuf keepbits;
    DevBuf bounds;
    DevBuf brank;

    bool implicit_all = true;
    DevBuf cand[2];
    DevBuf candC[2];
    int cur = 0;
    i64 m = 0;

    DevBuf win_st, win_en;
    DevBuf win_flags;
    DevBuf win_small, win_medium, win_large;
    i64 n_small = 0, n_medium = 0, n_large = 0;
    i64 n_large_p1 = 0;
    std::vector<int32_t> h_win_st, h_win_en, h_brank;

    DevBuf blocksum, tilestate, scalars, dpL, dpC, dpP, dpPrev, dpPart, dpPartArg, dpMark, dpJump, fscan, logfac_full;
    DevBuf xpRing, xpRec, xpTasks, regLR, regNR;

    bool pen_num = false, pen_len = false;
    DevBuf penNR, penLR;
    i64 n_pen_nr = 0, n_pen_lr = 0;
    double pen_refund = 0.0;
    DevBuf lxPos, lxSum, lxFirst, lxState;
    i64 lx_terms = 0;
    i64 scan_tiles_done = 0;

    int tune[PASIO_TUNE_COUNT];
    i64 *h_scalars = nullptr;

    i64 last_cells = 0, last_cells_skipped = 0;
    std::vector<i64> pw_leaf_start;
    i64 pw_n = -1;
    std::vector<double> pw_leaf_sum;

    bool timing = false;
    std::vector<TimedSpan> spans;
    std::vector<cudaEvent_t> event_pool;
    double fam_ms[TF_COUNT] = {0};
    i64 fam_launches[TF_COUNT] = {0};
};

int pasio_fail(pasio_ctx *ctx, int code, const char *fmt, ...);
int pasio_reserve(pasio_ctx *ctx, DevBuf &b, size_t bytes);

#define CUDA_TRY(ctx, call)                                                                     \
    do {                                                                                        \
        cudaError_t e__ = (call);                                                               \
        if (e__ != cudaSuccess)                                                                 \
            return pasio_fail((ctx), PASIO_E_CUDA, "%s failed: %s (%s:%d)", #call,              \
                              cudaGetErrorString(e__), __FILE__, __LINE__);                     \
    } while (0)

#define PASIO_TRY(call)                    \
    do {                                   \
        int rc__ = (call);                 \
        if (rc__ != PASIO_OK) return rc__; \
    } while (0)

struct TimingScope {
    pasio_ctx *ctx;
    int idx;
    cudaStream_t on;
    TimingScope(pasio_ctx *c, int family, i64 launches = 1, cudaStream_t stream = nullptr);
    ~TimingScope();
};


int launch_scan_counts(pasio_ctx *ctx);
int launch_scan_prepare(pasio_ctx *ctx, i64 *n_tiles, i64 *tile_elems);
int launch_scan_tiles(pasio_ctx *ctx, i64 tiles);
int launch_expand_rle(pasio_ctx *ctx, const i64 *d_starts, const i64 *d_values, i64 n_runs);
int launch_logfac_scan(pasio_ctx *ctx, double *d_out, cudaStream_t stream = nullptr);

int launch_compact_keepbits(pasio_ctx *ctx, int slot, i64 *h_count);
int launch_boundary_ranks(pasio_ctx *ctx);
int launch_window_prepass(pasio_ctx *ctx, i64 nwin, int wsize, int wshift, i64 *h_max_span, i64 *h_max_cnt,
                          int classify_constraint = -1, i64 w_begin = 0);
constexpr int WD_SMALL_MAX_CANDIDATES = 160, WD_MEDIUM_MAX_CANDIDATES = 512;
int small_window_max_candidates();
int medium_window_max_candidates();
int launch_validate_candidates(pasio_ctx *ctx, i64 *h_bad);
int launch_filter_candidates(pasio_ctx *ctx, int constraint);

int launch_window_dp(pasio_ctx *ctx, i64 nwin, int wsize, int wshift, int constraint, i64 w_begin = 0,
                     bool keep_cell_counters = false);
int window_dp_max_candidates(pasio_ctx *ctx);

int launch_window_dp_reg(pasio_ctx *ctx, i64 nwin, int wsize, int wshift, int constraint, bool keep_cell_counters = false);
int window_dp_reg_max_candidates(pasio_ctx *ctx);

int launch_exact_dp(pasio_ctx *ctx, i64 N);
int launch_exact_dp_pruned(pasio_ctx *ctx, i64 N, int lag);
int launch_regularized_dp(pasio_ctx *ctx, i64 N, const double *d_lr, const double *d_nr, double add0);
int launch_gather_candidates(pasio_ctx *ctx);
int launch_backtrace_mark(pasio_ctx *ctx, i64 N);
int launch_suffix_row(pasio_ctx *ctx, i64 stop, double *d_out);

int launch_segment_scores(pasio_ctx *ctx, double *d_scores, i64 *d_segcounts, double *d_means);
int launch_pairwise_leaves(pasio_ctx *ctx, const double *d_values, const i64 *d_leaf_start, i64 n_leaves, double *d_leaf_sum);
int launch_gather_i64(pasio_ctx *ctx, const i64 *d_src, const int32_t *d_idx32, const i64 *d_idx64, i64 m, i64 *d_out);
int launch_gather_f64_at_cands(pasio_ctx *ctx, const double *d_src, double *d_out);
int launch_lmm(pasio_ctx *ctx, const double *d_scores, const double *d_logfac_full, double *d_lmm);

int launch_logfac_exact(pasio_ctx *ctx, cudaStream_t stream = nullptr);
int launch_logfac_exact_begin(pasio_ctx *ctx, cudaStream_t stream);
int launch_logfac_exact_chunk(pasio_ctx *ctx, i64 p0, i64 p1, cudaStream_t stream);
int logfac_exact_chunks_result(pasio_ctx *ctx, bool *usable);
int launch_lmm_exact(pasio_ctx *ctx, const double *d_scores, double *d_lmm);
int launch_logfac_at_candidates_exact(pasio_ctx *ctx, double *d_out);
int logfac_exact_total(pasio_ctx *ctx, double *h_out);

static inline const int32_t *cur_cand(const pasio_ctx *ctx) {
    return ctx->implicit_all ? nullptr : ctx->cand[ctx->cur].as<int32_t>();
}
static inline const i64 *cur_cand_cg(const pasio_ctx *ctx) {
    return ctx->implicit_all ? nullptr : ctx->candC[ctx->cur].as<i64>();
}

struct WinGeom {
    const int32_t *st_tab;
    const int32_t *en_tab;
    i64 m;
    int wsize, wshift;
};
WinGeom make_geom(const pasio_ctx *ctx, int wsize, int wshift);

#ifdef __CUDACC__
__device__ __forceinline__ void window_range(const WinGeom &g, i64 w, i64 &st, i64 &en) {
    if (g.st_tab) {
        st = __ldg(g.st_tab + w);
        en = __ldg(g.en_tab + w);
    } else {
        st = w * g.wshift;
        en = min(st + (i64)g.wsize + 1, g.m);
    }
}
__device__ __forceinline__ double u32_to_double(int v) {
    return __dsub_rn(__hiloint2double(0x43300000, v), 4503599627370496.0);
}
__device__ __forceinline__ bool bit_test(const uint32_t *__restrict__ bits, i64 p) {
    return (__ldg(bits + (p >> 5)) >> (p & 31)) & 1u;
}
#endif
```

pasio_b200/csrc/dp_core.cuh:

```cuda
#pragma once
#include "common.cuh"

template <bool AI>
struct RowConst {
    int cjx;
    int lj;
    double aj;
};

template <bool AI>
__device__ __forceinline__ RowConst<AI> make_row(int cj, int lj, int alpha_int, double alpha)
{
    RowConst<AI> r;
    r.lj = lj;
    if (AI) {
        r.cjx = cj + alpha_int;
        r.aj = 0.0;
    } else {
        r.cjx = cj;
        r.aj = __dadd_rn(alpha, u32_to_double(cj));
    }
    return r;
}

// ... 20 lines not shown
{
#pragma unroll
    for (int off = RPW; off < 32; off <<= 1) {
        const double ob = __shfl_xor_sync(0xffffffffu, best, off);
        const int oa = __shfl_xor_sync(0xffffffffu, arg, off);
        if (ob > best || (ob == best && oa < arg)) { best = ob; arg = oa; }
    }
}

template <bool AI, int U, int RPL, bool LGS = false>
__device__ __forceinline__ void sweep_columns(int i0, int i1, int phase, int stride, const ColRec *sCol,
                                              const RowConst<AI> (&r)[RPL],
                                              const double *__restrict__ gtab, const double *__restrict__ ltab,
                                              double (&best)[RPL], int (&arg)[RPL])
{
    int i = i0 + phase;
    for (; i + (U - 1) * stride < i1; i += U * stride) {
        double g[U][RPL], lg[U][RPL], pc[U];
        int sx[U][RPL];
#pragma unroll
        for (int u = 0; u < U; ++u) {
            const ColRec a = sCol[i + u * stride];
            pc[u] = a.P;
#pragma unroll
            for (int k = 0; k < RPL; ++k) {
                const int idx = r[k].cjx - a.C;
                g[u][k] = __ldg(gtab + idx);
                lg[u][k] = LGS ? ltab[r[k].lj - a.L] : __ldg(ltab + (r[k].lj - a.L));
                sx[u][k] = AI ? idx : a.C;
            }
        }
#pragma unroll
        for (int u = 0; u < U; ++u)
#pragma unroll
            for (int k = 0; k < RPL; ++k) {
                const double s = AI ? u32_to_double(sx[u][k]) : __dsub_rn(r[k].aj, u32_to_double(sx[u][k]));
                const double t = __dadd_rn(__dsub_rn(g[u][k], __dmul_rn(s, lg[u][k])), pc[u]);
                if (t > best[k]) { best[k] = t; arg[k] = i + u * stride; }
            }
    }
    for (; i < i1; i += stride) {
        const ColRec a = sCol[i];
#pragma unroll
        for (int k = 0; k < RPL; ++k) {
            const double t = __dadd_rn(self_score<AI, LGS>(a.C, a.L, r[k], gtab, ltab), a.P);
            if (t > best[k]) { best[k] = t; arg[k] = i; }
        }
    }
}

constexpr int DP_JB = 32;
constexpr int DP_RPW = 4;

template <bool AI, int NW, int U, int RPL>
__device__ __forceinline__ void block_rect_tri(int jb, int N, int col0, const ColRec *sCol,
                                               double *sPartV, int *sPartA, double *sTri,
                                               const double *__restrict__ gtab, const double *__restrict__ ltab,
                                               int alpha_int, double alpha)
{
    constexpr int RPW = DP_RPW;
    constexpr int CPW = 32 / RPW;
    constexpr int NG = DP_JB / (RPW * RPL);
    constexpr int NQ = NW / NG;
    static_assert(NW % NG == 0 && NQ >= 1, "warps must tile the row groups");
    const int lane = threadIdx.x & 31, warp = threadIdx.x >> 5;
    const int grp = warp % NG, q = warp / NG;
    const int rr = lane % RPW, cc = lane / RPW;
    {
        RowConst<AI> r[RPL];
        double best[RPL];
        int arg[RPL];
        const int ncol = jb - col0;
        const int chunk = (ncol + NQ - 1) / NQ;
        const int i0 = col0 + q * chunk;
        const int i1 = min(i0 + chunk, jb);
#pragma unroll
        for (int k = 0; k < RPL; ++k) {
            const int j = min(jb + grp * RPW * RPL + k * RPW + rr, N - 1);
            const ColRec me = sCol[j];
            r[k] = make_row<AI>(me.C, me.L, alpha_int, alpha);
            best[k] = -INFINITY;
            arg[k] = i0 + cc;
        }
        sweep_columns<AI, U, RPL>(i0, i1, cc, CPW, sCol, r, gtab, ltab, best, arg);
#pragma unroll
        for (int k = 0; k < RPL; ++k) {
            merge_column_phases<RPW>(best[k], arg[k]);
            if (cc == 0) {
                const int row = grp * RPW * RPL + k * RPW + rr;
                sPartV[q * 32 + row] = best[k];
                sPartA[q * 32 + row] = arg[k];
            }
        }
    }
    {
        const ColRec me = sCol[min(jb + lane, N - 1)];
        const RowConst<AI> r = make_row<AI>(me.C, me.L, alpha_int, alpha);
        static_assert(DP_JB % NW == 0, "warps must tile the triangle rows");
        double w[DP_JB / NW];
#pragma unroll
        for (int kk = 0; kk < DP_JB / NW; ++kk) {
            const int k = warp + kk * NW;
            w[kk] = 0.0;
            if (k < lane && jb + lane < N) {
                const ColRec a = sCol[jb + k];
                w[kk] = self_score<AI>(a.C, a.L, r, gtab, ltab);
            }
        }
#pragma unroll
        for (int kk = 0; kk < DP_JB / NW; ++kk) {
            const int k = warp + kk * NW;
            if (k < lane && jb + lane < N) sTri[k * DP_JB + lane] = w[kk];
        }
    }
    __syncthreads();
}

template <int NQ>
__device__ __forceinline__ void block_chain(int jb, int N, ColRec *sCol, unsigned short *sPrev16, int *sPrev32,
                                            const double *sPartV, const int *sPartA, const double *sTri, double pen,
                                            double init_best, int init_arg, int arg_offset, double *sLB)
{
    const int lane = threadIdx.x & 31;
    double best = init_best;
    int arg = init_arg;
#pragma unroll
    for (int w = 0; w < NQ; ++w) {
        const double v = sPartV[w * 32 + lane];
        if (v > best) { best = v; arg = sPartA[w * 32 + lane] + arg_offset; }
    }
    double mine = 0.0, lb = 0.0;
    const int rows = min(DP_JB, N - jb);
#pragma unroll 8
    for (int k = 0; k < rows; ++k) {
        const double pf = __dadd_rn(best, pen);
        const double pk = __shfl_sync(0xffffffffu, pf, k);
        if (lane == k) { mine = pf; lb = best; }
        if (lane > k) {
            const double t = __dadd_rn(sTri[k * DP_JB + lane], pk);
            if (t > best) { best = t; arg = jb + k + arg_offset; }
        }
    }
    if (jb + lane < N) {
        sCol[jb + lane].P = mine;
        if (sPrev16) sPrev16[jb + lane] = (unsigned short)arg;
        else sPrev32[jb + lane] = arg;
        if (sLB) sLB[lane] = lb;
    }
}

template <int NQ>
__device__ __forceinline__ bool block_chain_speculative(int jb, int N, ColRec *sCol, unsigned short *sPrev16,
                                                        const double *sPartV, const int *sPartA, const double *sTri,
                                                        double pen, double init_best, int init_arg)
{
    const int lane = threadIdx.x & 31;
    double best = init_best;
    int arg = init_arg;
#pragma unroll
    for (int w = 0; w < NQ; ++w) {
        const double v = sPartV[w * 32 + lane];
        if (v > best) { best = v; arg = sPartA[w * 32 + lane]; }
    }
    const int rows = min(DP_JB, N - jb);
    const double below = (lane >= 1 && lane < rows) ? sTri[(lane - 1) * DP_JB + lane] : 0.0;
    double pk = __shfl_sync(0xffffffffu, __dadd_rn(best, pen), 0);
    double mine = pk;
#pragma unroll 8
    for (int k = 0; k < rows; ++k) {
        if (lane == k) mine = pk;
        if (lane > k) {
            const double t = __dadd_rn(sTri[k * DP_JB + lane], pk);
            if (t > best) { best = t; arg = jb + k; }
        }
        const double dn = __shfl_sync(0xffffffffu, below, (k + 1) & 31);
        pk = __dadd_rn(__dadd_rn(dn, pk), pen);
    }
    const bool as_assumed = lane == 0 || lane >= rows || arg == jb + lane - 1;
    if (!__all_sync(0xffffffffu, as_assumed)) return false;
    if (lane < rows) {
        sCol[jb + lane].P = mine;
        sPrev16[jb + lane] = (unsigned short)arg;
    }
    return true;
}

template <bool AI, int NW, int U, int RPL>
__device__ __forceinline__ void dp_block_step(int jb, int N, int col0, ColRec *sCol,
                                              unsigned short *sPrev16, int *sPrev32,
                                              double *sPartV, int *sPartA, double *sTri,
                                              const double *__restrict__ gtab, const double *__restrict__ ltab,
                                              int alpha_int, double alpha, double pen,
                                              double init_best, int init_arg, int arg_offset)
{
    constexpr int NQ = NW / (DP_JB / (DP_RPW * RPL));
    block_rect_tri<AI, NW, U, RPL>(jb, N, col0, sCol, sPartV, sPartA, sTri, gtab, ltab, alpha_int, alpha);
    if ((threadIdx.x >> 5) == 0)
        block_chain<NQ>(jb, N, sCol, sPrev16, sPrev32, sPartV, sPartA, sTri, pen, init_best, init_arg, arg_offset, nullptr);
    __syncthreads();
}
```

pasio_b200/csrc/window_dp.cu:

```cuda
#include "dp_core.cuh"
#include "bound.cuh"
#include <cstdio>
#include <cstdlib>

namespace {

constexpr int WD_THREADS = 256;
constexpr int WD_WARPS = WD_THREADS / 32;
constexpr int WD_FARW = WD_WARPS - 1;
constexpr int NEAR_Q = 4;
constexpr int PR_CB = 32;
constexpr int PR_FB = 8;
constexpr int PR_MIN_N = 256;
constexpr int PR_DENSE = 28;

#ifdef PASIO_WD_PROF
__device__ unsigned long long g_wd_prof[16];
struct ProfAcc { long long t0; long long a0, a1, a2, a3, a4, a5, a6, a7; };
#define PROF_DECL ProfAcc prof = {clock64(), 0, 0, 0, 0, 0, 0, 0, 0}
__device__ __forceinline__ long long prof_clock()
{
    unsigned dummy;
    long long t;
    asm volatile("ld.volatile.shared.u32 %0, [%1];" : "=r"(dummy) : "r"(0u) : "memory");
    asm volatile("mov.u64 %0, %%clock64;" : "=l"(t) : "r"(dummy) : "memory");
    return t;
}
#define PROF_T(i) do { const long long t1__ = prof_clock(); prof.a##i += t1__ - prof.t0; prof.t0 = t1__; } while (0)
#define PROF_FLUSH do { if (threadIdx.x == 0 || threadIdx.x == 32) { unsigned long long *g__ = g_wd_prof + (threadIdx.x ? 8 : 0); \
    atomicAdd(g__ + 0, (unsigned long long)prof.a0); atomicAdd(g__ + 1, (unsigned long long)prof.a1); \
    atomicAdd(g__ + 2, (unsigned long long)prof.a2); atomicAdd(g__ + 3, (unsigned long long)prof.a3); \
    atomicAdd(g__ + 4, (unsigned long long)prof.a4); atomicAdd(g__ + 5, (unsigned long long)prof.a5); \
    atomicAdd(g__ + 6, (unsigned long long)prof.a6); atomicAdd(g__ + 7, (unsigned long long)prof.a7); } \
    prof.a0 = prof.a1 = prof.a2 = prof.a3 = prof.a4 = prof.a5 = prof.a6 = prof.a7 = 0; } while (0)
#define PROF_ARGS , ProfAcc &prof
#define PROF_PASS , prof
#else
#define PROF_DECL
#define PROF_T(i) do { } while (0)
#define PROF_FLUSH do { } while (0)
#define PROF_ARGS
#define PROF_PASS
#endif

struct WinDpParams {
    WinGeom geom;
    i64 nwin;
    const int32_t *cand;
    const i64 *cg;
    const i64 *cgc;
    const uint32_t *cpbits;
    uint32_t *keepbits;
    const double *gtab;
    const double *ltab;
    int constraint;
    int alpha_int;
    double alpha;
    double pen;
    int cap;
    u64 *cells;
    u64 *cells_skipped;
    unsigned *work_counter;
    const int32_t *list;
    i64 w_begin;
    i64 n_p1, list_len;
    unsigned char *done_flags;
    int p1_stride;
    int skip_covered;
    int speculate;
    int n_lg;
};

__host__ __device__ inline size_t window_smem_bytes(int cap)
{
    const size_t capr = (size_t)((cap + 31) & ~31);
    return capr * 16
           + NEAR_Q * 32 * 8
           + DP_JB * DP_JB * 8
           + NEAR_Q * 32 * 4
           + 24 * 4
           + capr * 2
           + (capr / PR_CB) * sizeof(CoarseRec)
           + 2 * 32 * sizeof(float4)
           + capr * 2
           + 2 * ((capr / PR_CB) * 2 + 16)
           + 2 * WD_FARW * 32 * (8 + 4)
           + 8 * 8;
}

__device__ __forceinline__ int2 col_lc(const ColRec *sCol, int i)
{
    return *reinterpret_cast<const int2 *>(sCol + i);
}

template <bool AI>
__device__ __forceinline__ void compute_row_lb(int jbp, int jb, int N, const ColRec *sCol, float4 *sRow, double *sRowStat,
                                               double delta_path, double pen,
                                               const double *__restrict__ gtab, const double *__restrict__ ltab,
                                               int alpha_int, double alpha)
{
    const int lane = threadIdx.x & 31;
    const int jrow = min(jb + lane, N - 1);
    const int2 me = col_lc(sCol, jrow);
    const RowConst<AI> rme = make_row<AI>(me.y, me.x, alpha_int, alpha);
    const int jp = jbp + lane;
    const int2 pm = col_lc(sCol, jp), pb = col_lc(sCol, jp - 1), before = col_lc(sCol, jrow - 1);
    const RowConst<AI> rp = make_row<AI>(pm.y, pm.x, alpha_int, alpha);
    const double wp = self_score<AI>(pb.y, pb.x, rp, gtab, ltab) + pen;
    double run = self_score<AI>(before.y, before.x, rme, gtab, ltab) + (lane ? pen : 0.0);
    const double tot_prev = warp_sum(wp);
#pragma unroll
    for (int d = 1; d < 32; d <<= 1) {
        const double o = __shfl_up_sync(0xffffffffu, run, d);
        if (lane >= d) run += o;
    }
    double path = (sCol[jbp - 1].P + tot_prev) + run - delta_path;
    if (!(fabs(path) < 1e30)) path = -INFINITY;
    float lbf = (float)path;
    sRow[lane] = make_float4(lbf, (float)me.y, (float)me.x, 0.f);
    double ab = (jb + lane < N && path > -1e300) ? fabs(path) : 0.0;
#pragma unroll
    for (int off = 16; off > 0; off >>= 1) ab = fmax(ab, __shfl_xor_sync(0xffffffffu, ab, off));
    if (lane == 0) *sRowStat = ab;
}

__device__ __forceinline__ double tilted_row_min(const float4 *sRow, int r0, int r1, double a, double b, double lbabs,
                                                 int c_max, int l_max)
{
    const float af = (float)a, bf = (float)b;
    float m = INFINITY;
#pragma unroll 4
    for (int r = r0; r <= r1; ++r) {
        const float4 rr = sRow[r];
        m = fminf(m, fmaf(af, rr.y, fmaf(bf, rr.z, rr.x)));
    }
    const double err = (lbabs + fabs(a) * (double)c_max + fabs(b) * (double)l_max) * 9.5367431640625e-07;
    return (double)m - err;
}

template <bool AI>
__device__ __forceinline__ u64 far_pass(int jb, int N, int nfar, const ColRec *sCol, const CoarseRec *sCoarse,
                                        const float4 *sRow, double lbabs, unsigned short *sList, unsigned short *sDense,
                                        unsigned short *sSurv, int *sListCount ,
                                        double *sFarVW, int *sFarAW, double delta,
                                        const double *__restrict__ gtab, const double *__restrict__ ltab,
                                        int alpha_int, double alpha PROF_ARGS)
{
    const int lane = threadIdx.x & 31, w7 = (threadIdx.x >> 5) - 1;
    const int nrows = min(DP_JB, N - jb);
    const int2 rowF = col_lc(sCol, jb), rowL = col_lc(sCol, jb + nrows - 1);
    const int2 me = col_lc(sCol, min(jb + lane, N - 1));
    const RowConst<AI> rme = make_row<AI>(me.y, me.x, alpha_int, alpha);

    double best = -INFINITY;
    int arg = 0x7fffffff;
    if (w7 == 0 && lane < nrows) {
        const ColRec a0 = sCol[0];
        best = __dadd_rn(self_score<AI>(a0.C, a0.L, rme, gtab, ltab), a0.P);
        arg = 0;
    }
    u64 skipped = 0;

    const int rg = lane >> 2, q = lane & 3;
    const int r0 = 4 * rg, r1 = min(r0 + 3, nrows - 1);
    const bool act2 = r0 < nrows;
    const int2 gF = col_lc(sCol, jb + min(r0, nrows - 1)), gL = col_lc(sCol, jb + r1);

    auto level2 = [&](int cb1) {
        const CoarseRec *rec = sCoarse + cb1;
        const double a = rec->a, b = rec->b;
        bool surv2 = false;
        if (act2) {
            const int i0 = 1 + PR_CB * cb1 + PR_FB * q;
            const int2 cF = col_lc(sCol, i0), cL = col_lc(sCol, i0 + PR_FB - 1);
            const double m2 = tilted_box_max<AI>(gF.y - cL.y, gL.y - cF.y, gF.x - cL.x, gL.x - cF.x, a, b,
                                                 gtab, ltab, alpha_int, alpha);
            const double m3 = tilted_row_min(sRow, r0, r1, a, b, lbabs, gL.y, gL.x);
            surv2 = !(rec->mpt8[q] + m2 - m3 + delta < 0.0);
            if (!surv2) skipped += (u64)(PR_FB * (r1 - r0 + 1));
        }
        const unsigned mask2 = __ballot_sync(0xffffffffu, surv2);
        const int n2 = __popc(mask2);
        if (n2 >= PR_DENSE) {
            if (act2 && !surv2) skipped -= (u64)(PR_FB * (r1 - r0 + 1));
            if (lane == 0) sDense[atomicAdd(sListCount + 1, 1)] = (unsigned short)cb1;
        } else if (n2) {
            int slot = 0;
            if (lane == 0) slot = atomicAdd(sListCount, n2);
            slot = __shfl_sync(0xffffffffu, slot, 0);
            if (surv2) sList[slot + __popc(mask2 & ((1u << lane) - 1u))] = (unsigned short)((cb1 << 5) | lane);
        }
    };
    const int l1_warps = min(WD_FARW, (nfar + 31) / 32);
    const int n_direct = max(0, min(nfar, WD_FARW - l1_warps));
    const int nfar1 = nfar - n_direct;
    if (w7 >= l1_warps && w7 - l1_warps < n_direct) level2(nfar - 1 - (w7 - l1_warps));

    for (int base = 0; base + 32 * w7 < nfar1 && w7 < l1_warps; base += 32 * l1_warps) {
        const int cb = base + 32 * w7 + lane;
        bool surv1 = false;
        if (cb < nfar1) {
            const CoarseRec *rec = sCoarse + cb;
            const int4 ends = *reinterpret_cast<const int4 *>(rec);
            const double a1 = rec->a, b1 = rec->b;
            const double ub1 = rec->mpt + tilted_box_max<AI>(rowF.y - ends.y, rowL.y - ends.x, rowF.x - ends.w, rowL.x - ends.z,
                                                             a1, b1, gtab, ltab, alpha_int, alpha);
            const double m3 = tilted_row_min(sRow, 0, nrows - 1, a1, b1, lbabs, rowL.y, rowL.x);
            surv1 = !(ub1 - m3 + delta < 0.0);
            if (!surv1) skipped += (u64)(PR_CB * nrows);
        }
        const unsigned mask1 = __ballot_sync(0xffffffffu, surv1);
        if (mask1) {
            int slot = 0;
            if (lane == 0) slot = atomicAdd(sListCount + 2, __popc(mask1));
            slot = __shfl_sync(0xffffffffu, slot, 0);
            if (surv1) sSurv[slot + __popc(mask1 & ((1u << lane) - 1u))] = (unsigned short)cb;
        }
    }
    PROF_T(4);
    asm volatile("bar.sync 1, %0;" ::"n"(WD_FARW * 32) : "memory");
    const int nsurv = *reinterpret_cast<volatile int *>(sListCount + 2);

    for (int e = w7; e < nsurv; e += WD_FARW) level2(sSurv[e]);
    PROF_T(5);
    asm volatile("bar.sync 1, %0;" ::"n"(WD_FARW * 32) : "memory");
    const int total = *reinterpret_cast<volatile int *>(sListCount);
    const int ndense = *reinterpret_cast<volatile int *>(sListCount + 1);
    PROF_T(3);

    for (int e = w7; e < ndense; e += WD_FARW) {
        const int i0 = 1 + PR_CB * (int)sDense[e];
        const int rr = lane & 3, cph = lane >> 2;
#pragma unroll 1
        for (int g = 0; g < 4; ++g) {
            RowConst<AI> r[2];
            double bst[2];
            int ag[2];
#pragma unroll
            for (int k = 0; k < 2; ++k) {
                const int2 rl = col_lc(sCol, min(jb + g * 8 + k * 4 + rr, N - 1));
                r[k] = make_row<AI>(rl.y, rl.x, alpha_int, alpha);
                bst[k] = -INFINITY;
                ag[k] = i0 + cph;
            }
            sweep_columns<AI, 4, 2>(i0, i0 + PR_CB, cph, 8, sCol, r, gtab, ltab, bst, ag);
#pragma unroll
            for (int k = 0; k < 2; ++k) {
                merge_column_phases<4>(bst[k], ag[k]);
                const double v = __shfl_sync(0xffffffffu, bst[k], lane & 3);
                const int va = __shfl_sync(0xffffffffu, ag[k], lane & 3);
                if ((lane >> 2) == g * 2 + k && lane < nrows && (v > best || (v == best && va < arg))) { best = v; arg = va; }
            }
        }
    }

    constexpr int UX = 4;
    const int er = lane >> 3, ec = lane & 7;
    for (int e0 = w7 * UX; e0 < total; e0 += WD_FARW * UX) {
        double t[UX];
        int ta[UX], g4[UX];
#pragma unroll
        for (int u = 0; u < UX; ++u) {
            t[u] = -INFINITY;
            ta[u] = 0x7fffffff;
            g4[u] = 0;
            if (e0 + u < total) {
                const int ent = sList[e0 + u];
                const int l2 = ent & 31;
                g4[u] = 4 * (l2 >> 2);
                const int row = g4[u] + er;
                const int col = 1 + PR_CB * (ent >> 5) + PR_FB * (l2 & 3) + ec;
                ta[u] = col;
                if (row < nrows) {
                    const int2 rl = col_lc(sCol, jb + row);
                    const RowConst<AI> rc = make_row<AI>(rl.y, rl.x, alpha_int, alpha);
                    const ColRec cc = sCol[col];
                    t[u] = __dadd_rn(self_score<AI>(cc.C, cc.L, rc, gtab, ltab), cc.P);
                }
            }
        }
#pragma unroll
        for (int u = 0; u < UX; ++u) {
#pragma unroll
            for (int off = 1; off < 8; off <<= 1) {
                const double ob = __shfl_xor_sync(0xffffffffu, t[u], off);
                const int oa = __shfl_xor_sync(0xffffffffu, ta[u], off);
                if (ob > t[u] || (ob == t[u] && oa < ta[u])) { t[u] = ob; ta[u] = oa; }
            }
            const int rel = lane - g4[u];
            const double v = __shfl_sync(0xffffffffu, t[u], (rel & 3) * 8);
            const int va = __shfl_sync(0xffffffffu, ta[u], (rel & 3) * 8);
            if (rel >= 0 && rel < 4 && (v > best || (v == best && va < arg))) { best = v; arg = va; }
        }
    }
    sFarVW[lane] = best;
    sFarAW[lane] = arg;
    return skipped;
}

template <bool AI, int NW>
__device__ __forceinline__ void near_tri_farwarps(int w7 , int jb, int N, const ColRec *sCol, double *sPartV,
                                                  int *sPartA, double *sTri,
                                                  const double *__restrict__ gtab, const double *__restrict__ ltab,
                                                  int alpha_int, double alpha)
{
    const int lane = threadIdx.x & 31;
    const int rr = lane & 3, cc = lane >> 2;
    constexpr int NT = (16 + NW - 1) / NW;
    double tv[NT][2];
    int tcol[NT];
#pragma unroll
    for (int u = 0; u < NT; ++u) {
        const int t = w7 + u * NW;
        const int grp = t & 3, qc = (t >> 2) & 3;
        tcol[u] = jb - PR_CB + qc * 8 + cc;
        const ColRec a = sCol[tcol[u]];
#pragma unroll
        for (int k = 0; k < 2; ++k) {
            const int j = min(jb + grp * 8 + k * 4 + rr, N - 1);
            const int2 me = col_lc(sCol, j);
            const RowConst<AI> r = make_row<AI>(me.y, me.x, alpha_int, alpha);
            tv[u][k] = (t < 16) ? __dadd_rn(self_score<AI>(a.C, a.L, r, gtab, ltab), a.P) : -INFINITY;
        }
    }
    const int2 mt = col_lc(sCol, min(jb + lane, N - 1));
    const RowConst<AI> rt = make_row<AI>(mt.y, mt.x, alpha_int, alpha);
    constexpr int NK = (DP_JB + NW - 1) / NW;
    double w[NK];
#pragma unroll
    for (int kk = 0; kk < NK; ++kk) {
        const int k = w7 + kk * NW;
        w[kk] = 0.0;
        if (k < lane && jb + lane < N) {
            const int2 a = col_lc(sCol, jb + k);
            w[kk] = self_score<AI>(a.y, a.x, rt, gtab, ltab);
        }
    }
#pragma unroll
    for (int u = 0; u < NT; ++u) {
        const int t = w7 + u * NW;
#pragma unroll
        for (int k = 0; k < 2; ++k) {
            double best = tv[u][k];
            int arg = tcol[u];
            merge_column_phases<4>(best, arg);
            if (cc == 0 && t < 16) {
                const int row = (t & 3) * 8 + k * 4 + rr;
                sPartV[(t >> 2) * 32 + row] = best;
                sPartA[(t >> 2) * 32 + row] = arg;
            }
        }
    }
#pragma unroll
    for (int kk = 0; kk < NK; ++kk) {
        const int k = w7 + kk * NW;
        if (k < lane && jb + lane < N) sTri[k * DP_JB + lane] = w[kk];
    }
}

__device__ __forceinline__ void build_coarse_record(int jb, const ColRec *sCol, CoarseRec *rec, double tilt_scale_c,
                                                    double tilt_scale_l)
{
    const ColRec me = sCol[jb + (threadIdx.x & 31)];
    fit_column_record(me.C, me.L, me.P, rec, tilt_scale_c, tilt_scale_l);
}

template <bool AI, int U, int RPL, bool PRUNE>
__global__ void __launch_bounds__(WD_THREADS, 3)
window_dp_kernel(WinDpParams p)
{
    extern __shared__ __align__(16) unsigned char smem[];
    const int capr = (p.cap + 31) & ~31;
    ColRec *sCol = reinterpret_cast<ColRec *>(smem);
    double *sPartV = reinterpret_cast<double *>(sCol + capr);
    double *sTri = sPartV + NEAR_Q * 32;
    int *sPartA = reinterpret_cast<int *>(sTri + DP_JB * DP_JB);
    int *sMisc = sPartA + NEAR_Q * 32;
    unsigned short *sPrev = reinterpret_cast<unsigned short *>(sMisc + 24);
    CoarseRec *sCoarse = reinterpret_cast<CoarseRec *>(sPrev + capr);
    float4 *sRow = reinterpret_cast<float4 *>(sCoarse + capr / PR_CB);
    double *sFarV = reinterpret_cast<double *>(sRow + 2 * 32);
    int *sFarA = reinterpret_cast<int *>(sFarV + 2 * WD_FARW * 32);
    double *sScal = reinterpret_cast<double *>(sFarA + 2 * WD_FARW * 32);
    unsigned short *sList = reinterpret_cast<unsigned short *>(sScal + 8);
    int *sListCount = sMisc + 16;
    unsigned short *sJump = reinterpret_cast<unsigned short *>(sCoarse);
    unsigned char *sMark = reinterpret_cast<unsigned char *>(sTri);

    const int tid = threadIdx.x, lane = tid & 31, warp = tid >> 5;
    PROF_DECL;

    while (true) {
        PROF_T(7);
        PROF_FLUSH;
        if (tid == 0) sMisc[0] = (int)atomicAdd(p.work_counter, 1u);
        __syncthreads();
        const i64 widx = (unsigned)sMisc[0];
        if (widx >= p.nwin) break;
        const bool second = widx >= p.n_p1;
        const bool phase2 = second && p.skip_covered;
        const i64 w = !p.list ? p.w_begin + widx
                              : (second ? (i64)__ldg(p.list + (p.list_len - 1 - (widx - p.n_p1))) : (i64)__ldg(p.list + widx));
        if (phase2) {
            if (tid == 0) {
                const i64 rel = w - p.w_begin, lo = rel - rel % p.p1_stride, hi = lo + p.p1_stride;
                const volatile unsigned char *f = p.done_flags;
                while (!f[lo] || (hi < p.list_len && !f[hi])) __nanosleep(200);
                __threadfence();
                i64 skip_cells = -1;
                if (hi < p.list_len && (f[lo] & 2) && (f[hi] & 2)) {
                    i64 s0, e0, s1, e1, s2, e2;
                    window_range(p.geom, w, s0, e0);
                    window_range(p.geom, p.w_begin + lo, s1, e1);
                    window_range(p.geom, p.w_begin + hi, s2, e2);
                    if (s1 <= s0 && e1 >= s2 && e2 >= e0) skip_cells = (e0 - s0) * (e0 - s0 - 1) / 2;
                }
                if (skip_cells >= 0) {
                    atomicAdd(p.cells, (u64)skip_cells);
                    atomicAdd(p.cells_skipped, (u64)skip_cells);
                }
                sMisc[1] = skip_cells >= 0;
            }
            __syncthreads();
            if (sMisc[1]) continue;
        }
        int kept_all = 1;

        i64 st, en;
        window_range(p.geom, w, st, en);
        const int nq = (int)(en - st);
        const i64 first = p.cand ? (i64)__ldg(p.cand + st) : st;
        const i64 last = p.cand ? (i64)__ldg(p.cand + en - 1) : en - 1;
        const i64 cg_first = p.cand ? __ldg(p.cgc + st) : __ldg(p.cg + first);
        const bool all_zero = (p.constraint == PASIO_CONSTRAINT_ZEROS) && ((p.cand ? __ldg(p.cgc + en - 1) : __ldg(p.cg + last)) == cg_first);
        int count = 0;
        const bool by_words = !p.cand && p.constraint == PASIO_CONSTRAINT_CONSTANTS;
        if (by_words) {
            const i64 w0 = first >> 5, w1 = last >> 5;
            const int nwords = (int)(w1 - w0 + 1);
            for (int base = 0; base < nwords; base += WD_THREADS) {
                const int t = base + tid;
                unsigned word = 0;
                if (t < nwords) {
                    word = __ldg(p.cpbits + w0 + t);
                    if (t == 0) word = (word & (0xffffffffu << (first & 31))) | (1u << (first & 31));
                    if (t == nwords - 1) word = (word & (0xffffffffu >> (31 - (last & 31)))) | (1u << (last & 31));
                }
                int incl = __popc(word);
                const int mine = incl;
#pragma unroll
                for (int d = 1; d < 32; d <<= 1) {
                    const int o = __shfl_up_sync(0xffffffffu, incl, d);
                    if (lane >= d) incl += o;
                }
                if (lane == 31) sMisc[4 + warp] = incl;
                __syncthreads();
                int woff = 0, tot = 0;
#pragma unroll
                for (int w2 = 0; w2 < WD_WARPS; ++w2) {
                    const int c = sMisc[4 + w2];
                    if (w2 < warp) woff += c;
                    tot += c;
                }
                int k = count + woff + incl - mine;
                const i64 pos0 = (w0 + t) << 5;
                while (word) {
                    const i64 pos = pos0 + (__ffs(word) - 1);
                    word &= word - 1;
                    sCol[k].L = (int)(pos - first);
                    sCol[k].C = (int)(__ldg(p.cg + pos) - cg_first);
                    ++k;
                }
                count += tot;
                __syncthreads();
            }
        }
        for (int base = 0; !by_words && base < nq; base += WD_THREADS) {
            const int q = base + tid;
            i64 pos = 0;
            bool take = false;
            if (q < nq) {
                pos = p.cand ? (i64)__ldg(p.cand + st + q) : st + q;
                if (q == 0 || q == nq - 1 || p.constraint == PASIO_CONSTRAINT_NONE) take = true;
                else if (p.constraint == PASIO_CONSTRAINT_CONSTANTS) take = bit_test(p.cpbits, pos);
                else take = !all_zero;
                if (phase2 && !((__ldcg(p.keepbits + (pos >> 5)) >> (pos & 31)) & 1u)) kept_all = 0;
            }
            const unsigned bal = __ballot_sync(0xffffffffu, take);
            if (lane == 0) sMisc[4 + warp] = __popc(bal);
            __syncthreads();
            int woff = 0, tot = 0;
#pragma unroll
            for (int w2 = 0; w2 < WD_WARPS; ++w2) {
                const int c = sMisc[4 + w2];
                if (w2 < warp) woff += c;
                tot += c;
            }
            if (take) {
                const int k = count + woff + __popc(bal & ((1u << lane) - 1u));
                sCol[k].L = (int)(pos - first);
                sCol[k].C = (int)((p.cand ? __ldg(p.cgc + st + q) : __ldg(p.cg + pos)) - cg_first);
            }
            count += tot;
            __syncthreads();
        }
        const int N = count;
        PROF_T(0);
        if (phase2 && __syncthreads_and(kept_all)) {
            if (tid == 0) {
                const u64 c = (u64)N * (u64)(N - 1) / 2;
                atomicAdd(p.cells, c);
                atomicAdd(p.cells_skipped, c);
            }
            continue;
        }

        if (tid == 0) { sCol[0].P = 0.0; sPrev[0] = 0; }
        __syncthreads();
        u64 skipped = 0;
        if (PRUNE && tid == 0) {
            const ColRec z = sCol[N - 1];
            const int x = z.C + (AI ? p.alpha_int : 0);
            sScal[0] = fabs(__ldg(p.gtab + x)) + ((double)z.C + p.alpha) * fabs(__ldg(p.ltab + z.L)) + 1.0;
            sScal[1] = 0.0;
            sScal[2] = (double)z.C + p.alpha;
            sScal[3] = (double)z.L;
        }
        auto finish_block = [&](int jb) {
            if (jb + DP_JB <= N) build_coarse_record(jb, sCol, sCoarse + (jb - 1) / PR_CB, sScal[2], sScal[3]);
            double ab = jb + lane < N ? fabs(sCol[jb + lane].P) : 0.0;
#pragma unroll
            for (int off = 16; off > 0; off >>= 1) ab = fmax(ab, __shfl_xor_sync(0xffffffffu, ab, off));
            if (lane == 0) sScal[1] = fmax(sScal[1], ab);
        };
        auto far_delta = [&]() { return (sScal[0] + sScal[1] + fabs(p.pen) * DP_JB) * 5.684341886080802e-14; };
        auto prepare_rows = [&](int jbn) {
            const int par = ((jbn - 1) / DP_JB) & 1;
            const double delta_path = (sScal[0] + sScal[1] + fabs(p.pen) * DP_JB) * 1.8189894035458565e-12;
            compute_row_lb<AI>(jbn - DP_JB, jbn, N, sCol, sRow + 32 * par, sScal + 4 + par, delta_path, p.pen, p.gtab, p.ltab,
                               p.alpha_int, p.alpha);
            if (lane == 0) { sListCount[4 * par] = 0; sListCount[4 * par + 1] = 0; sListCount[4 * par + 2] = 0; }
        };
        auto run_far = [&](int jbf) {
            const int kf = (jbf - 1) / DP_JB, par = kf & 1;
            skipped += far_pass<AI>(jbf, N, kf - 1, sCol, sCoarse, sRow + 32 * par, sScal[4 + par], sList, sList + capr,
                                    sList + capr + capr / PR_CB + 8, sListCount + 4 * par, sFarV + (par * WD_FARW + warp - 1) * 32,
                                    sFarA + (par * WD_FARW + warp - 1) * 32,
                                    far_delta(), p.gtab, p.ltab, p.alpha_int, p.alpha PROF_PASS);
        };
        int jb = 1;
        const bool pipelined = PRUNE && N > PR_MIN_N && p.cand != nullptr;
        for (; jb < N && (!pipelined || jb < 1 + 2 * DP_JB); jb += DP_JB) {
            dp_block_step<AI, WD_WARPS, U, RPL>(jb, N, 0, sCol, sPrev, nullptr, sPartV, sPartA, sTri,
                                                p.gtab, p.ltab, p.alpha_int, p.alpha, p.pen, -INFINITY, 0, 0);
            if (pipelined && warp == 0) finish_block(jb);
        }
        PROF_T(6);
        if (pipelined && jb < N) {
            int spec_wait = 0, spec_back = 1;
            if (warp == 0) prepare_rows(jb);
            __syncthreads();
            if (warp > 0) run_far(jb);
            else if (jb + DP_JB < N) prepare_rows(jb + DP_JB);
            __syncthreads();
            for (; jb < N; jb += DP_JB) {
                const int k = (jb - 1) / DP_JB, buf = k & 1;
                near_tri_farwarps<AI, WD_WARPS>(warp, jb, N, sCol, sPartV, sPartA, sTri, p.gtab, p.ltab, p.alpha_int, p.alpha);
                PROF_T(1);
                __syncthreads();
                PROF_T(6);
                if (warp == 0) {
                    double fbest = -INFINITY;
                    int farg = 0;
#pragma unroll
                    for (int w2 = 0; w2 < WD_FARW; ++w2) {
                        const double v = sFarV[(buf * WD_FARW + w2) * 32 + lane];
                        const int a = sFarA[(buf * WD_FARW + w2) * 32 + lane];
                        if (v > fbest || (v == fbest && a < farg)) { fbest = v; farg = a; }
                    }
                    const double ib = jb + lane < N ? fbest : -INFINITY;
                    const int ia = jb + lane < N ? farg : 0;
                    bool resolved = false;
                    if (p.speculate && spec_wait == 0) {
                        resolved = block_chain_speculative<NEAR_Q>(jb, N, sCol, sPrev, sPartV, sPartA, sTri, p.pen, ib, ia);
                        if (resolved) spec_back = 1;
                        else { spec_wait = spec_back; spec_back = min(spec_back * 2, 16); }
                    } else if (spec_wait > 0) {
                        --spec_wait;
                    }
                    if (!resolved) block_chain<NEAR_Q>(jb, N, sCol, sPrev, nullptr, sPartV, sPartA, sTri, p.pen, ib, ia, 0, nullptr);
                    __syncwarp();
                    finish_block(jb);
                    if (jb + 2 * DP_JB < N) prepare_rows(jb + 2 * DP_JB);
                } else if (jb + DP_JB < N) {
                    run_far(jb + DP_JB);
                }
                PROF_T(2);
                __syncthreads();
                PROF_T(7);
            }
        }

        for (int k = tid; k < N; k += WD_THREADS) sMark[k] = (k == N - 1);
        __syncthreads();
        unsigned short *ja = sPrev, *jb2 = sJump;
        for (int reach = 1; reach < N; reach <<= 1) {
            for (int k = tid; k < N; k += WD_THREADS)
                if (sMark[k]) sMark[ja[k]] = 1;
            for (int k = tid; k < N; k += WD_THREADS) jb2[k] = ja[ja[k]];
            __syncthreads();
            unsigned short *t = ja; ja = jb2; jb2 = t;
        }
        int every = N == nq;
        for (int k = tid; k < N; k += WD_THREADS) {
            if (sMark[k]) {
                const i64 pos = first + sCol[k].L;
                atomicOr(p.keepbits + (pos >> 5), 1u << (pos & 31));
            } else {
                every = 0;
            }
        }
        if (!second && p.skip_covered && p.n_p1 < p.nwin) {
            __threadfence();
            every = __syncthreads_and(every);
            if (tid == 0) {
                __threadfence();
                *reinterpret_cast<volatile unsigned char *>(p.done_flags + (w - p.w_begin)) = every ? 3 : 1;
            }
        }
        if (tid == 0) atomicAdd(p.cells, (u64)N * (u64)(N - 1) / 2);
        if (PRUNE) {
#pragma unroll
            for (int off = 16; off > 0; off >>= 1) skipped += __shfl_xor_sync(0xffffffffu, skipped, off);
            if (lane == 0 && skipped) atomicAdd(p.cells_skipped, skipped);
        }
        __syncthreads();
    }
}

constexpr int SW_JB = 16;
constexpr int SW_SMALL_N = WD_SMALL_MAX_CANDIDATES, SW_SMALL_WARPS = 8, SW_SMALL_CTAS = 5;
constexpr int SW_MEDIUM_N = WD_MEDIUM_MAX_CANDIDATES, SW_MEDIUM_WARPS = 4, SW_MEDIUM_CTAS = 4;

template <int MAXN>
struct __align__(16) SmallWin {
    ColRec col[MAXN];
    double tri[SW_JB * SW_JB];
    unsigned short prev[MAXN];
    unsigned char mark[MAXN];
};

template <bool AI, int MAXN, int NWARPS, int CTAS, int U, bool LGS>
__global__ void __launch_bounds__(NWARPS * 32, CTAS)
small_window_dp_kernel(WinDpParams p)
{
    extern __shared__ __align__(16) unsigned char smem[];
    const int lane = threadIdx.x & 31;
    SmallWin<MAXN> &W = reinterpret_cast<SmallWin<MAXN> *>(smem)[threadIdx.x >> 5];
    u64 my_cells = 0;
    const double *lgt = p.ltab;
    if (LGS) {
        double *sLg = reinterpret_cast<double *>(smem + sizeof(SmallWin<MAXN>) * NWARPS);
        for (int k = threadIdx.x; k < p.n_lg; k += NWARPS * 32) sLg[k] = __ldg(p.ltab + k);
        __syncthreads();
        lgt = sLg;
    }

    while (true) {
        unsigned widx = 0;
        if (lane == 0) widx = atomicAdd(p.work_counter, 1u);
        widx = __shfl_sync(0xffffffffu, widx, 0);
        if ((i64)widx >= p.nwin) break;
        const i64 w = __ldg(p.list + widx);

        i64 st, en;
        window_range(p.geom, w, st, en);
        const int nq = (int)(en - st);
        const i64 first = p.cand ? (i64)__ldg(p.cand + st) : st;
        const i64 last = p.cand ? (i64)__ldg(p.cand + en - 1) : en - 1;
        const i64 cg_first = p.cand ? __ldg(p.cgc + st) : __ldg(p.cg + first);
        const bool all_zero = (p.constraint == PASIO_CONSTRAINT_ZEROS) && ((p.cand ? __ldg(p.cgc + en - 1) : __ldg(p.cg + last)) == cg_first);
        int count = 0;
        if (!p.cand && p.constraint == PASIO_CONSTRAINT_CONSTANTS) {
            const i64 w0 = first >> 5, w1 = last >> 5;
            const int nwords = (int)(w1 - w0 + 1);
            for (int base = 0; base < nwords; base += 32) {
                const int t = base + lane;
                unsigned word = 0;
                if (t < nwords) {
                    word = __ldg(p.cpbits + w0 + t);
                    if (t == 0) word = (word & (0xffffffffu << (first & 31))) | (1u << (first & 31));
                    if (t == nwords - 1) word = (word & (0xffffffffu >> (31 - (last & 31)))) | (1u << (last & 31));
                }
                int incl = __popc(word);
                const int mine = incl;
#pragma unroll
                for (int d = 1; d < 32; d <<= 1) {
                    const int o = __shfl_up_sync(0xffffffffu, incl, d);
                    if (lane >= d) incl += o;
                }
                int k = count + incl - mine;
                const i64 pos0 = (w0 + t) << 5;
                while (word) {
                    const i64 pos = pos0 + (__ffs(word) - 1);
                    word &= word - 1;
                    W.col[k].L = (int)(pos - first);
                    W.col[k].C = (int)(__ldg(p.cg + pos) - cg_first);
                    ++k;
                }
                count += __shfl_sync(0xffffffffu, incl, 31);
            }
        } else {
            for (int base = 0; base < nq; base += 32) {
                const int q = base + lane;
                i64 pos = 0;
                bool take = false;
                if (q < nq) {
                    pos = p.cand ? (i64)__ldg(p.cand + st + q) : st + q;
                    if (q == 0 || q == nq - 1 || p.constraint == PASIO_CONSTRAINT_NONE) take = true;
                    else if (p.constraint == PASIO_CONSTRAINT_CONSTANTS) take = bit_test(p.cpbits, pos);
                    else take = !all_zero;
                }
                const unsigned bal = __ballot_sync(0xffffffffu, take);
                if (take) {
                    const int k = count + __popc(bal & ((1u << lane) - 1u));
                    W.col[k].L = (int)(pos - first);
                    W.col[k].C = (int)((p.cand ? __ldg(p.cgc + st + q) : __ldg(p.cg + pos)) - cg_first);
                }
                count += __popc(bal);
            }
        }
        const int N = count;
        if (lane == 0) { W.col[0].P = 0.0; W.prev[0] = 0; }
        __syncwarp();

        const int r = lane & 15, ph = lane >> 4;
        for (int jb = 1; jb < N; jb += SW_JB) {
            const ColRec me = W.col[min(jb + r, N - 1)];
            RowConst<AI> rc[1] = {make_row<AI>(me.C, me.L, p.alpha_int, p.alpha)};
            double best[1] = {-INFINITY};
            int arg[1] = {ph};
            sweep_columns<AI, U, 1, LGS>(0, jb, ph, 2, W.col, rc, p.gtab, lgt, best, arg);
            {
                const double ob = __shfl_xor_sync(0xffffffffu, best[0], 16);
                const int oa = __shfl_xor_sync(0xffffffffu, arg[0], 16);
                if (ob > best[0] || (ob == best[0] && oa < arg[0])) { best[0] = ob; arg[0] = oa; }
            }
            for (int k = ph; k < r; k += 2)
                if (jb + r < N) {
                    const ColRec a = W.col[jb + k];
                    W.tri[k * SW_JB + r] = self_score<AI, LGS>(a.C, a.L, rc[0], p.gtab, lgt);
                }
            __syncwarp();
            double bst = best[0], mine = 0.0;
            int ag = arg[0];
            const int rows = min(SW_JB, N - jb);
#pragma unroll 4
            for (int k = 0; k < rows; ++k) {
                const double pf = __dadd_rn(bst, p.pen);
                const double pk = __shfl_sync(0xffffffffu, pf, k);
                if (r == k) mine = pf;
                if (r > k) {
                    const double t = __dadd_rn(W.tri[k * SW_JB + r], pk);
                    if (t > bst) { bst = t; ag = jb + k; }
                }
            }
            if (lane < SW_JB && jb + r < N) {
                W.col[jb + r].P = mine;
                W.prev[jb + r] = (unsigned short)ag;
            }
            __syncwarp();
        }

        for (int k = lane; k < N; k += 32) W.mark[k] = 0;
        __syncwarp();
        if (lane == 0) {
            int k = N - 1;
            while (true) {
                W.mark[k] = 1;
                if (k == 0) break;
                k = W.prev[k];
            }
        }
        __syncwarp();
        for (int k = lane; k < N; k += 32)
            if (W.mark[k]) {
                const i64 pos = first + W.col[k].L;
                atomicOr(p.keepbits + (pos >> 5), 1u << (pos & 31));
            }
        my_cells += (u64)N * (u64)(N - 1) / 2;
        __syncwarp();
    }
    if (lane == 0 && my_cells) atomicAdd(p.cells, my_cells);
}

}

int small_window_max_candidates() { return SW_SMALL_N; }
int medium_window_max_candidates() { return SW_MEDIUM_N; }

int window_dp_max_candidates(pasio_ctx *ctx)
{
    int cap = 32;
    while (cap + 32 <= 8192 && window_smem_bytes(cap + 32) <= (size_t)ctx->smem_optin) cap += 32;
    return cap;
}

int launch_window_dp(pasio_ctx *ctx, i64 nwin, int wsize, int wshift, int constraint, i64 w_begin, bool keep_cell_counters)
{
    WinDpParams p;
    p.geom = make_geom(ctx, wsize, wshift);
    p.nwin = nwin;
    p.cand = cur_cand(ctx);
    p.cg = ctx->cg.as<i64>();
    p.cgc = cur_cand_cg(ctx);
    p.cpbits = ctx->cpbits.as<uint32_t>();
    p.keepbits = ctx->keepbits.as<uint32_t>();
    p.gtab = ctx->tab[ctx->alpha_is_int ? PASIO_TAB_LGAMMA : PASIO_TAB_LGAMMA_ALPHA].as<double>();
    p.ltab = ctx->tab[PASIO_TAB_LOG].as<double>();
    p.constraint = constraint;
    p.alpha_int = (int)ctx->alpha_int;
    p.alpha = ctx->alpha;
    p.pen = ctx->pen;
    i64 cap = (i64)wsize + 1;
    if (cap > ctx->m) cap = ctx->m;
    if (cap > 8192 || window_smem_bytes((int)cap) > (size_t)ctx->smem_optin)
        return pasio_fail(ctx, PASIO_E_TOO_LARGE, "window of %lld candidates does not fit one CTA's shared memory (max %d)",
                          (long long)cap, window_dp_max_candidates(ctx));
    p.cap = (int)cap;
    p.cells = ctx->scalars.as<u64>() + 10;
    p.cells_skipped = ctx->scalars.as<u64>() + 12;
    p.work_counter = ctx->scalars.as<unsigned>() + 2 * 11;
    p.w_begin = w_begin;
    if (keep_cell_counters) CUDA_TRY(ctx, cudaMemsetAsync(ctx->scalars.as<u64>() + 11, 0, 8, ctx->stream));
    else CUDA_TRY(ctx, cudaMemsetAsync(ctx->scalars.as<u64>() + 10, 0, 24, ctx->stream));
    CUDA_TRY(ctx, cudaMemsetAsync(ctx->scalars.as<u64>() + 15, 0, 8, ctx->stream));

    static const int small_env = getenv("PASIO_WD_SMALL") ? atoi(getenv("PASIO_WD_SMALL")) : 1;
    const int phase_env = ctx->tune[PASIO_TUNE_WINDOW_PHASES];
    const bool use_lists = small_env && ctx->n_small + ctx->n_medium + ctx->n_large == nwin;
    const i64 n_small = use_lists ? ctx->n_small : 0, n_medium = use_lists ? ctx->n_medium : 0;
    const i64 n_large = use_lists ? ctx->n_large : nwin;
    p.list = use_lists ? ctx->win_large.as<int32_t>() : nullptr;
    p.nwin = n_large;
    p.list_len = nwin;
    p.n_p1 = use_lists ? ctx->n_large_p1 : n_large;
    p.skip_covered = phase_env;
    p.speculate = ctx->tune[PASIO_TUNE_WINDOW_SPECULATE];
    p.done_flags = ctx->win_flags.as<unsigned char>();
    p.p1_stride = wshift > 0 && wsize / wshift > 1 ? wsize / wshift : 1;
    if (!use_lists) p.skip_covered = 0;
    ctx->n_small = ctx->n_medium = ctx->n_large = ctx->n_large_p1 = -1;
    TimingScope ts_all(ctx, TF_WINDOW_DP, 0);
    const bool fork = n_small + n_medium > 0 && n_small + n_medium <= 64;
    const bool serial_small = n_small + n_medium > 64;
    if (fork) CUDA_TRY(ctx, cudaEventRecord(ctx->ev_fork, ctx->stream));

    auto launch_small = [&](auto kern, const int32_t *list, i64 n, int nwarps, int ctas, size_t smem_bytes, unsigned *counter,
                            cudaStream_t stream) -> int {
        if (n <= 0) return PASIO_OK;
        WinDpParams ps = p;
        ps.list = list;
        ps.nwin = n;
        ps.n_p1 = n;
        ps.work_counter = counter;
        CUDA_TRY(ctx, cudaFuncSetAttribute(kern, cudaFuncAttributeMaxDynamicSharedMemorySize, (int)smem_bytes));
        int resident = ctas;
        CUDA_TRY(ctx, cudaOccupancyMaxActiveBlocksPerMultiprocessor(&resident, kern, nwarps * 32, smem_bytes));
        if (resident < 1) resident = 1;
        if (resident > ctas) resident = ctas;
        i64 g = (n + nwarps - 1) / nwarps;
        if (g > (i64)ctx->sm_count * resident) g = (i64)ctx->sm_count * resident;
        ctx->fam_launches[TF_WINDOW_DP] += 1;
        kern<<<(unsigned)g, nwarps * 32, smem_bytes, stream>>>(ps);
        CUDA_TRY(ctx, cudaGetLastError());
        return PASIO_OK;
    };
    static const int lgs_env = getenv("PASIO_WD_LGS") ? atoi(getenv("PASIO_WD_LGS")) : 0;
    const bool lgs = lgs_env && p.cand == nullptr && (i64)wsize + 2 <= 4096 && ctx->ntab[PASIO_TAB_LOG] >= (i64)wsize + 2;
    p.n_lg = lgs ? wsize + 2 : 0;
    const size_t lg_bytes = (size_t)((p.n_lg + 1) & ~1) * 8;
    auto launch_small_kernels = [&](cudaStream_t stream) -> int {
        unsigned *c_small = ctx->scalars.as<unsigned>() + 2 * 15, *c_medium = c_small + 1;
        const size_t sm_small = sizeof(SmallWin<SW_SMALL_N>) * SW_SMALL_WARPS + lg_bytes,
                     sm_medium = sizeof(SmallWin<SW_MEDIUM_N>) * SW_MEDIUM_WARPS + lg_bytes;
#define PASIO_SMALL_LAUNCH(AIV, LGV)                                                                                                          \
        PASIO_TRY(launch_small(small_window_dp_kernel<AIV, SW_SMALL_N, SW_SMALL_WARPS, SW_SMALL_CTAS, 4, LGV>, ctx->win_small.as<int32_t>(),   \
                               n_small, SW_SMALL_WARPS, SW_SMALL_CTAS, sm_small, c_small, stream));                                            \
        PASIO_TRY(launch_small(small_window_dp_kernel<AIV, SW_MEDIUM_N, SW_MEDIUM_WARPS, SW_MEDIUM_CTAS, 8, LGV>, ctx->win_medium.as<int32_t>(), \
                               n_medium, SW_MEDIUM_WARPS, SW_MEDIUM_CTAS, sm_medium, c_medium, stream));
        if (ctx->alpha_is_int) {
            if (lgs) { PASIO_SMALL_LAUNCH(true, true) } else { PASIO_SMALL_LAUNCH(true, false) }
        } else {
            if (lgs) { PASIO_SMALL_LAUNCH(false, true) } else { PASIO_SMALL_LAUNCH(false, false) }
        }
#undef PASIO_SMALL_LAUNCH
        return PASIO_OK;
    };
    if (serial_small) PASIO_TRY(launch_small_kernels(ctx->stream));

    i64 grid = 0;
    if (n_large > 0) {
        const size_t smem = window_smem_bytes(p.cap);
        const int prune_env = ctx->tune[PASIO_TUNE_WINDOW_PRUNE];
        const bool prune = prune_env != 0 && ctx->alpha >= 0.0009765625;
        void (*kern)(WinDpParams);
        if (ctx->alpha_is_int) kern = prune ? window_dp_kernel<true, 4, 2, true> : window_dp_kernel<true, 4, 2, false>;
        else kern = prune ? window_dp_kernel<false, 4, 2, true> : window_dp_kernel<false, 4, 2, false>;
        CUDA_TRY(ctx, cudaFuncSetAttribute(kern, cudaFuncAttributeMaxDynamicSharedMemorySize, (int)smem));
        int per_sm = 0;
        CUDA_TRY(ctx, cudaOccupancyMaxActiveBlocksPerMultiprocessor(&per_sm, kern, WD_THREADS, smem));
        if (per_sm < 1) per_sm = 1;
#ifdef PASIO_WD_PROF
        if (getenv("PASIO_WD_CTAS") && atoi(getenv("PASIO_WD_CTAS")) < per_sm) per_sm = atoi(getenv("PASIO_WD_CTAS"));
#endif
        grid = (i64)ctx->sm_count * per_sm;
        if (grid > n_large) grid = n_large;
        if (grid < 1) grid = 1;
        ctx->fam_launches[TF_WINDOW_DP] += 1;
        kern<<<(unsigned)grid, WD_THREADS, smem, ctx->stream>>>(p);
        CUDA_TRY(ctx, cudaGetLastError());
    }
    if (fork) {
        CUDA_TRY(ctx, cudaStreamWaitEvent(ctx->stream2, ctx->ev_fork, 0));
        PASIO_TRY(launch_small_kernels(ctx->stream2));
        CUDA_TRY(ctx, cudaEventRecord(ctx->ev_join, ctx->stream2));
        CUDA_TRY(ctx, cudaStreamWaitEvent(ctx->stream, ctx->ev_join, 0));
    }
#ifdef PASIO_WD_PROF
    {
        cudaStreamSynchronize(ctx->stream);
        unsigned long long h[16], z[16] = {0};
        cudaMemcpyFromSymbol(h, g_wd_prof, sizeof h);
        cudaMemcpyToSymbol(g_wd_prof, z, sizeof z);
        static const char *names[8] = {"compact", "X:work", "Y:work(chain|far L3)", "far:listwait", "far:L1", "far:L2", "wait@X+plain", "wait@Y+rest"};
        for (int side = 0; side < 2; ++side) {
            double tot = 0;
            for (int i = 0; i < 8; ++i) tot += (double)h[8 * side + i];
            fprintf(stderr, "[wd_prof %s] nwin=%lld grid=%lld:", side ? "warp1" : "warp0", (long long)nwin, (long long)grid);
            for (int i = 0; i < 8; ++i) if (h[8 * side + i]) fprintf(stderr, " %s=%.1f%%", names[i], 100.0 * (double)h[8 * side + i] / tot);
            fprintf(stderr, " | cycles/CTA=%.3g\n", tot / (double)grid);
        }
    }
#endif
    return PASIO_OK;
}
```

Before: 5.712 billion.

## Restructure window DP into chain, band-helper and verifier warps with speculative rollback

Reworks the window DP CTA. The old lockstep scheme of one chain warp plus far warps with block-wide syncs becomes a warp-specialised pipeline: one chain warp, four band-helper warps computing near-band partials and coarse records, and verifier warps that check far pruning bounds in batches against a ring of lower bounds. Warps coordinate through volatile shared-memory flags rather than __syncthreads. If verification finds a violation, the run rolls back to a plain step, and after a set number of rollbacks it falls back to plain stepping. This aims to remove per-block barrier stalls and overlap far-candidate work with the serial chain, at the cost of spin-waiting, more shared memory and possible rollback rework. Rollback and switchover counters are added and exposed through a new API.

Measured after the change: 6.815 billion (median of 6 runs). 1.19x the previous value.

```diff
diff --git a/include/pasio_b200.h b/include/pasio_b200.h
--- a/include/pasio_b200.h
+++ b/include/pasio_b200.h
@@ -70,6 +70,7 @@
 int pasio_round(pasio_ctx *ctx, int64_t window_size, int64_t window_shift, int constraint,
                 int64_t *n_in, int64_t *n_out, int64_t *cells);
 int pasio_round_stats(const pasio_ctx *ctx, int64_t *cells, int64_t *cells_skipped);
+int pasio_window_band_stats(const pasio_ctx *ctx, int64_t *rollbacks, int64_t *switchovers);
 int pasio_exact_task_plan(int64_t n_candidates, int lag, int nblock, int32_t *triples, int64_t cap, int64_t *n_tasks);
 int pasio_upload_stats(const pasio_ctx *ctx, int64_t *wire_bytes);
 int pasio_set_tuning(pasio_ctx *ctx, int key, int value);
diff --git a/pasio_b200/_native.py b/pasio_b200/_native.py
--- a/pasio_b200/_native.py
+++ b/pasio_b200/_native.py
@@ -41,6 +41,7 @@
     'pasio_filter_candidates': (ctypes.c_int, [_vp, ctypes.c_int, _i64p, _i64p]),
     'pasio_round': (ctypes.c_int, [_vp, _i64, _i64, ctypes.c_int, _i64p, _i64p, _i64p]),
     'pasio_round_stats': (ctypes.c_int, [_vp, _i64p, _i64p]),
+    'pasio_window_band_stats': (ctypes.c_int, [_vp, _i64p, _i64p]),
     'pasio_exact_task_plan': (ctypes.c_int, [_i64, ctypes.c_int, ctypes.c_int, ctypes.POINTER(ctypes.c_int32), _i64, _i64p]),
     'pasio_upload_stats': (ctypes.c_int, [_vp, _i64p]),
     'pasio_set_tuning': (ctypes.c_int, [_vp, ctypes.c_int, ctypes.c_int]),
@@ -394,6 +395,11 @@
         self._check(self.lib.pasio_round_stats(self.ctx, ctypes.byref(a), ctypes.byref(b)))
         return a.value, b.value
 
+    def band_stats(self):
+        a, b = _i64(0), _i64(0)
+        self._check(self.lib.pasio_window_band_stats(self.ctx, ctypes.byref(a), ctypes.byref(b)))
+        return a.value, b.value
+
     def rounds(self, window_size, window_shift, constraint, num_rounds=None, first=None):
         n, _, _ = self.info()
         limit = max(1, n if num_rounds is None else num_rounds)
diff --git a/pasio_b200/csrc/api.cu b/pasio_b200/csrc/api.cu
--- a/pasio_b200/csrc/api.cu
+++ b/pasio_b200/csrc/api.cu
@@ -410,13 +410,13 @@
         cudaEventCreateWithFlags(&ctx->ev_lx1, cudaEventDisableTiming) != cudaSuccess ||
         cudaEventCreateWithFlags(&ctx->ev_fork, cudaEventDisableTiming) != cudaSuccess ||
         cudaEventCreateWithFlags(&ctx->ev_join, cudaEventDisableTiming) != cudaSuccess ||
-        cudaMallocHost((void **)&ctx->h_scalars, 16 * sizeof(i64)) != cudaSuccess ||
-        pasio_reserve(ctx, ctx->scalars, 16 * sizeof(i64)) != PASIO_OK) {
+        cudaMallocHost((void **)&ctx->h_scalars, 18 * sizeof(i64)) != cudaSuccess ||
+        pasio_reserve(ctx, ctx->scalars, 18 * sizeof(i64)) != PASIO_OK) {
         g_create_error = "context allocation failed: " + ctx->err;
         delete ctx;
         return PASIO_E_CUDA;
     }
-    memset(ctx->h_scalars, 0, 16 * sizeof(i64));
+    memset(ctx->h_scalars, 0, 18 * sizeof(i64));
     auto env_int = [](const char *name, int dflt) { const char *v = getenv(name); return v ? atoi(v) : dflt; };
     ctx->tune[PASIO_TUNE_WINDOW_PRUNE] = env_int("PASIO_WD_PRUNE", 1);
     ctx->tune[PASIO_TUNE_WINDOW_PHASES] = env_int("PASIO_WD_PHASES", 1);
@@ -843,10 +843,12 @@
     PASIO_TRY(pasio_reserve(ctx, ctx->cand[nxt], (size_t)ctx->m * 4));
     i64 m_new = 0;
     PASIO_TRY(launch_compact_keepbits(ctx, nxt, &m_new));
-    PASIO_TRY(d2h(ctx, ctx->h_scalars + 10, ctx->scalars.as<i64>() + 10, 24));
+    PASIO_TRY(d2h(ctx, ctx->h_scalars + 10, ctx->scalars.as<i64>() + 10, 64));
     if (cells) *cells = ctx->h_scalars[10];
     ctx->last_cells = ctx->h_scalars[10];
     ctx->last_cells_skipped = ctx->h_scalars[12];
+    ctx->last_rollbacks = penalties_on(ctx) ? 0 : ctx->h_scalars[16];
+    ctx->last_switchovers = penalties_on(ctx) ? 0 : ctx->h_scalars[17];
     ctx->cur = nxt;
     ctx->implicit_all = false;
     ctx->m = m_new;
@@ -1049,10 +1051,12 @@
     PASIO_TRY(pasio_reserve(ctx, ctx->cand[nxt], (size_t)ctx->m * 4));
     i64 m_new = 0;
     PASIO_TRY(launch_compact_keepbits(ctx, nxt, &m_new));
-    PASIO_TRY(d2h(ctx, ctx->h_scalars + 10, ctx->scalars.as<i64>() + 10, 24));
+    PASIO_TRY(d2h(ctx, ctx->h_scalars + 10, ctx->scalars.as<i64>() + 10, 64));
     if (cells) *cells = ctx->h_scalars[10];
     ctx->last_cells = ctx->h_scalars[10];
     ctx->last_cells_skipped = ctx->h_scalars[12];
+    ctx->last_rollbacks = penalties_on(ctx) ? 0 : ctx->h_scalars[16];
+    ctx->last_switchovers = penalties_on(ctx) ? 0 : ctx->h_scalars[17];
     ctx->cur = nxt;
     ctx->implicit_all = false;
     ctx->m = m_new;
@@ -1097,6 +1101,14 @@
     if (!ctx) return PASIO_E_ARG;
     if (cells) *cells = ctx->last_cells;
     if (cells_skipped) *cells_skipped = ctx->last_cells_skipped;
+    return PASIO_OK;
+}
+
+extern "C" int pasio_window_band_stats(const pasio_ctx *ctx, int64_t *rollbacks, int64_t *switchovers)
+{
+    if (!ctx) return PASIO_E_ARG;
+    if (rollbacks) *rollbacks = ctx->last_rollbacks;
+    if (switchovers) *switchovers = ctx->last_switchovers;
     return PASIO_OK;
 }
 
diff --git a/pasio_b200/csrc/common.cuh b/pasio_b200/csrc/common.cuh
--- a/pasio_b200/csrc/common.cuh
+++ b/pasio_b200/csrc/common.cuh
@@ -100,6 +100,7 @@
     i64 *h_scalars = nullptr;
 
     i64 last_cells = 0, last_cells_skipped = 0;
+    i64 last_rollbacks = 0, last_switchovers = 0;
     std::vector<i64> pw_leaf_start;
     i64 pw_n = -1;
     std::vector<double> pw_leaf_sum;
diff --git a/pasio_b200/csrc/dp_core.cuh b/pasio_b200/csrc/dp_core.cuh
--- a/pasio_b200/csrc/dp_core.cuh
+++ b/pasio_b200/csrc/dp_core.cuh
@@ -196,7 +196,7 @@
 template <int NQ>
 __device__ __forceinline__ bool block_chain_speculative(int jb, int N, ColRec *sCol, unsigned short *sPrev16,
                                                         const double *sPartV, const int *sPartA, const double *sTri,
-                                                        double pen, double init_best, int init_arg)
+                                                        double pen, double init_best, int init_arg, double *sLB = nullptr)
 {
     const int lane = threadIdx.x & 31;
     double best = init_best;
@@ -225,6 +225,7 @@
     if (lane < rows) {
         sCol[jb + lane].P = mine;
         sPrev16[jb + lane] = (unsigned short)arg;
+        if (sLB) sLB[lane] = best;
     }
     return true;
 }
diff --git a/pasio_b200/csrc/window_dp.cu b/pasio_b200/csrc/window_dp.cu
--- a/pasio_b200/csrc/window_dp.cu
+++ b/pasio_b200/csrc/window_dp.cu
@@ -7,15 +7,25 @@
 
 constexpr int WD_THREADS = 256;
 constexpr int WD_WARPS = WD_THREADS / 32;
-constexpr int WD_FARW = WD_WARPS - 1;
-constexpr int NEAR_Q = 4;
+constexpr int WD_HELP = 4;
+constexpr int WD_VER = WD_WARPS - 1 - WD_HELP;
+constexpr int WD_VER_BAR = 1;
+constexpr int BAND_BLOCKS = 2;
+constexpr int RING = 16;
+constexpr int VG = 8;
+#ifndef PASIO_WD_MAX_ROLLBACKS
+#define PASIO_WD_MAX_ROLLBACKS 2
+#endif
+static_assert(VG <= 8 && 4 + VG <= 16, "a survivor entry keeps the row block in 3 bits; sScal holds 4 + VG values");
+constexpr int MAX_ROLLBACKS = PASIO_WD_MAX_ROLLBACKS;
 constexpr int PR_CB = 32;
 constexpr int PR_FB = 8;
 constexpr int PR_MIN_N = 256;
 constexpr int PR_DENSE = 28;
 
 #ifdef PASIO_WD_PROF
-__device__ unsigned long long g_wd_prof[16];
+constexpr int PROF_SIDES = 3;
+__device__ unsigned long long g_wd_prof[8 * PROF_SIDES];
 struct ProfAcc { long long t0; long long a0, a1, a2, a3, a4, a5, a6, a7; };
 #define PROF_DECL ProfAcc prof = {clock64(), 0, 0, 0, 0, 0, 0, 0, 0}
 __device__ __forceinline__ long long prof_clock()
@@ -27,20 +37,17 @@
     return t;
 }
 #define PROF_T(i) do { const long long t1__ = prof_clock(); prof.a##i += t1__ - prof.t0; prof.t0 = t1__; } while (0)
-#define PROF_FLUSH do { if (threadIdx.x == 0 || threadIdx.x == 32) { unsigned long long *g__ = g_wd_prof + (threadIdx.x ? 8 : 0); \
+#define PROF_FLUSH do { const int side__ = threadIdx.x == 0 ? 0 : threadIdx.x == 32 ? 1 : threadIdx.x == 32 * (1 + WD_HELP) ? 2 : -1; \
+    if (side__ >= 0) { unsigned long long *g__ = g_wd_prof + 8 * side__; \
     atomicAdd(g__ + 0, (unsigned long long)prof.a0); atomicAdd(g__ + 1, (unsigned long long)prof.a1); \
     atomicAdd(g__ + 2, (unsigned long long)prof.a2); atomicAdd(g__ + 3, (unsigned long long)prof.a3); \
     atomicAdd(g__ + 4, (unsigned long long)prof.a4); atomicAdd(g__ + 5, (unsigned long long)prof.a5); \
     atomicAdd(g__ + 6, (unsigned long long)prof.a6); atomicAdd(g__ + 7, (unsigned long long)prof.a7); } \
     prof.a0 = prof.a1 = prof.a2 = prof.a3 = prof.a4 = prof.a5 = prof.a6 = prof.a7 = 0; } while (0)
-#define PROF_ARGS , ProfAcc &prof
-#define PROF_PASS , prof
 #else
 #define PROF_DECL
 #define PROF_T(i) do { } while (0)
 #define PROF_FLUSH do { } while (0)
-#define PROF_ARGS
-#define PROF_PASS
 #endif
 
 struct WinDpParams {
@@ -60,6 +67,8 @@
     int cap;
     u64 *cells;
     u64 *cells_skipped;
+    u64 *rollbacks;
+    u64 *switchovers;
     unsigned *work_counter;
     const int32_t *list;
     i64 w_begin;
@@ -71,21 +80,32 @@
     int n_lg;
 };
 
+constexpr int SY_BASE = 16;
+constexpr int SY_CHAIN = SY_BASE + 0;
+constexpr int SY_BAND = SY_BASE + 1;
+constexpr int SY_REC = SY_BASE + 1 + WD_HELP;
+constexpr int SY_VER = SY_REC + 1;
+constexpr int SY_ABORT = SY_VER + 1;
+constexpr int SY_SURV = SY_ABORT + 1;
+constexpr int SY_KEND = SY_SURV + 1;
+constexpr int SY_VIO = SY_KEND + 1;
+constexpr int SY_SKIP = SY_VIO + 2 * VG;
+constexpr int SMISC_INTS = (SY_SKIP + 2 * VG + 3) & ~3;
+
 __host__ __device__ inline size_t window_smem_bytes(int cap)
 {
     const size_t capr = (size_t)((cap + 31) & ~31);
     return capr * 16
-           + NEAR_Q * 32 * 8
+           + 4 * 32 * 8
            + DP_JB * DP_JB * 8
-           + NEAR_Q * 32 * 4
-           + 24 * 4
+           + 4 * 32 * 4
+           + SMISC_INTS * 4
            + capr * 2
            + (capr / PR_CB) * sizeof(CoarseRec)
-           + 2 * 32 * sizeof(float4)
-           + capr * 2
-           + 2 * ((capr / PR_CB) * 2 + 16)
-           + 2 * WD_FARW * 32 * (8 + 4)
-           + 8 * 8;
+           + RING * 32 * 8
+           + VG * 32 * sizeof(float4)
+           + 16 * 8
+           + VG * (capr / PR_CB) * 2;
 }
 
 __device__ __forceinline__ int2 col_lc(const ColRec *sCol, int i)
@@ -93,36 +113,15 @@
     return *reinterpret_cast<const int2 *>(sCol + i);
 }
 
-template <bool AI>
-__device__ __forceinline__ void compute_row_lb(int jbp, int jb, int N, const ColRec *sCol, float4 *sRow, double *sRowStat,
-                                               double delta_path, double pen,
-                                               const double *__restrict__ gtab, const double *__restrict__ ltab,
-                                               int alpha_int, double alpha)
-{
-    const int lane = threadIdx.x & 31;
-    const int jrow = min(jb + lane, N - 1);
-    const int2 me = col_lc(sCol, jrow);
-    const RowConst<AI> rme = make_row<AI>(me.y, me.x, alpha_int, alpha);
-    const int jp = jbp + lane;
-    const int2 pm = col_lc(sCol, jp), pb = col_lc(sCol, jp - 1), before = col_lc(sCol, jrow - 1);
-    const RowConst<AI> rp = make_row<AI>(pm.y, pm.x, alpha_int, alpha);
-    const double wp = self_score<AI>(pb.y, pb.x, rp, gtab, ltab) + pen;
-    double run = self_score<AI>(before.y, before.x, rme, gtab, ltab) + (lane ? pen : 0.0);
-    const double tot_prev = warp_sum(wp);
-#pragma unroll
-    for (int d = 1; d < 32; d <<= 1) {
-        const double o = __shfl_up_sync(0xffffffffu, run, d);
-        if (lane >= d) run += o;
-    }
-    double path = (sCol[jbp - 1].P + tot_prev) + run - delta_path;
-    if (!(fabs(path) < 1e30)) path = -INFINITY;
-    float lbf = (float)path;
-    sRow[lane] = make_float4(lbf, (float)me.y, (float)me.x, 0.f);
-    double ab = (jb + lane < N && path > -1e300) ? fabs(path) : 0.0;
-#pragma unroll
-    for (int off = 16; off > 0; off >>= 1) ab = fmax(ab, __shfl_xor_sync(0xffffffffu, ab, off));
-    if (lane == 0) *sRowStat = ab;
-}
+__device__ __forceinline__ int vload(const int *p) { return *reinterpret_cast<const volatile int *>(p); }
+__device__ __forceinline__ void vstore(int *p, int v) { *reinterpret_cast<volatile int *>(p) = v; }
+__device__ __forceinline__ int vload_warp(const int *p)
+{
+    int v = 0;
+    if ((threadIdx.x & 31) == 0) v = vload(p);
+    return __shfl_sync(0xffffffffu, v, 0);
+}
+
 
 __device__ __forceinline__ double tilted_row_min(const float4 *sRow, int r0, int r1, double a, double b, double lbabs,
                                                  int c_max, int l_max)
@@ -139,230 +138,215 @@
 }
 
 template <bool AI>
-__device__ __forceinline__ u64 far_pass(int jb, int N, int nfar, const ColRec *sCol, const CoarseRec *sCoarse,
-                                        const float4 *sRow, double lbabs, unsigned short *sList, unsigned short *sDense,
-                                        unsigned short *sSurv, int *sListCount ,
-                                        double *sFarVW, int *sFarAW, double delta,
-                                        const double *__restrict__ gtab, const double *__restrict__ ltab,
-                                        int alpha_int, double alpha PROF_ARGS)
-{
-    const int lane = threadIdx.x & 31, w7 = (threadIdx.x >> 5) - 1;
-    const int nrows = min(DP_JB, N - jb);
-    const int2 rowF = col_lc(sCol, jb), rowL = col_lc(sCol, jb + nrows - 1);
-    const int2 me = col_lc(sCol, min(jb + lane, N - 1));
-    const RowConst<AI> rme = make_row<AI>(me.y, me.x, alpha_int, alpha);
-
+__device__ __forceinline__ bool band_help(int h, int k, int N, const ColRec *sCol, double *sPartV, int *sPartA, double *sTri,
+                                          int *sMisc, const double *__restrict__ gtab, const double *__restrict__ ltab,
+                                          int alpha_int, double alpha)
+{
+    const int lane = threadIdx.x & 31;
+    const int jb = 1 + DP_JB * k;
+    const int r = 8 * h + (lane & 7), c = lane >> 3;
+    const int2 me = col_lc(sCol, min(jb + r, N - 1));
+    const RowConst<AI> rc = make_row<AI>(me.y, me.x, alpha_int, alpha);
+    const int i0 = jb - BAND_BLOCKS * DP_JB + c;
     double best = -INFINITY;
-    int arg = 0x7fffffff;
-    if (w7 == 0 && lane < nrows) {
+    int arg = i0;
+    double sb[8];
+#pragma unroll
+    for (int u = 0; u < 8; ++u) {
+        const ColRec a = sCol[i0 + 4 * u];
+        const double t = __dadd_rn(self_score<AI>(a.C, a.L, rc, gtab, ltab), a.P);
+        if (t > best) { best = t; arg = i0 + 4 * u; }
+        const int2 b = col_lc(sCol, i0 + DP_JB + 4 * u);
+        sb[u] = self_score<AI>(b.y, b.x, rc, gtab, ltab);
+    }
+    const int2 mt = col_lc(sCol, min(jb + lane, N - 1));
+    const RowConst<AI> rt = make_row<AI>(mt.y, mt.x, alpha_int, alpha);
+    double tw[DP_JB / WD_HELP];
+#pragma unroll
+    for (int v = 0; v < DP_JB / WD_HELP; ++v) {
+        const int kk = h + WD_HELP * v;
+        tw[v] = 0.0;
+        if (kk < lane && jb + lane < N) {
+            const int2 a = col_lc(sCol, jb + kk);
+            tw[v] = self_score<AI>(a.y, a.x, rt, gtab, ltab);
+        }
+    }
+    while (vload_warp(sMisc + SY_CHAIN) < k) {
+        if (vload_warp(sMisc + SY_ABORT) >= 0) return false;
+    }
+    __threadfence_block();
+#pragma unroll
+    for (int u = 0; u < 8; ++u) {
+        const double t = __dadd_rn(sb[u], sCol[i0 + DP_JB + 4 * u].P);
+        if (t > best) { best = t; arg = i0 + DP_JB + 4 * u; }
+    }
+    merge_column_phases<8>(best, arg);
+    if (c == 0) {
+        sPartV[r] = best;
+        sPartA[r] = arg;
+    }
+#pragma unroll
+    for (int v = 0; v < DP_JB / WD_HELP; ++v) {
+        const int kk = h + WD_HELP * v;
+        if (kk < lane && jb + lane < N) sTri[kk * DP_JB + lane] = tw[v];
+    }
+    __syncwarp();
+    __threadfence_block();
+    if (lane == 0) vstore(sMisc + SY_BAND + h, k + 1);
+    return true;
+}
+
+__device__ __forceinline__ void build_coarse_record(int jb, const ColRec *sCol, CoarseRec *rec, double tilt_scale_c,
+                                                    double tilt_scale_l)
+{
+    const ColRec me = sCol[jb + (threadIdx.x & 31)];
+    fit_column_record(me.C, me.L, me.P, rec, tilt_scale_c, tilt_scale_l);
+}
+
+template <bool AI>
+__device__ __forceinline__ int verify_batch(int v, int kv, int par, int N, const ColRec *sCol, const CoarseRec *sCoarse,
+                                             const double *sRing, float4 *sRowV, double *sScal, unsigned short *sSurv, int *sMisc,
+                                             double pen, const double *__restrict__ gtab, const double *__restrict__ ltab,
+                                             int alpha_int, double alpha)
+{
+    const int lane = threadIdx.x & 31;
+    int *vio = sMisc + SY_VIO + VG * par;
+    unsigned *skipc = reinterpret_cast<unsigned *>(sMisc + SY_SKIP + VG * par);
+    if (v == 0) {
+        int kend;
+        while (true) {
+            kend = min(vload_warp(sMisc + SY_CHAIN), kv + VG);
+            if (kend > kv && vload_warp(sMisc + SY_REC) >= kend - 1 - BAND_BLOCKS) break;
+            __nanosleep(64);
+        }
+        if (lane == 0) {
+            sMisc[SY_KEND] = kend;
+            sMisc[SY_SURV] = 0;
+        }
+    }
+    asm volatile("bar.sync %0, %1;" ::"n"(WD_VER_BAR), "n"(WD_VER * 32) : "memory");
+    __threadfence_block();
+    const int kend = sMisc[SY_KEND], nb = kend - kv;
+    for (int bi = v; bi < nb; bi += WD_VER) {
+        const int jb = 1 + DP_JB * (kv + bi), rows = min(DP_JB, N - jb);
+        const bool valid = lane < rows;
+        const double m = sRing[((kv + bi) % RING) * 32 + lane];
+        const int2 me = col_lc(sCol, min(jb + lane, N - 1));
+        const double lb = fabs(m) < 1e30 ? m : -INFINITY;
+        sRowV[bi * 32 + lane] = make_float4((float)lb, (float)me.y, (float)me.x, 0.f);
+        double ab = valid && lb > -1e300 ? fabs(lb) : 0.0;
+#pragma unroll
+        for (int off = 16; off > 0; off >>= 1) ab = fmax(ab, __shfl_xor_sync(0xffffffffu, ab, off));
+        const RowConst<AI> rme = make_row<AI>(me.y, me.x, alpha_int, alpha);
         const ColRec a0 = sCol[0];
-        best = __dadd_rn(self_score<AI>(a0.C, a0.L, rme, gtab, ltab), a0.P);
-        arg = 0;
-    }
-    u64 skipped = 0;
-
-    const int rg = lane >> 2, q = lane & 3;
-    const int r0 = 4 * rg, r1 = min(r0 + 3, nrows - 1);
-    const bool act2 = r0 < nrows;
-    const int2 gF = col_lc(sCol, jb + min(r0, nrows - 1)), gL = col_lc(sCol, jb + r1);
-
-    auto level2 = [&](int cb1) {
-        const CoarseRec *rec = sCoarse + cb1;
-        const double a = rec->a, b = rec->b;
-        bool surv2 = false;
-        if (act2) {
-            const int i0 = 1 + PR_CB * cb1 + PR_FB * q;
-            const int2 cF = col_lc(sCol, i0), cL = col_lc(sCol, i0 + PR_FB - 1);
-            const double m2 = tilted_box_max<AI>(gF.y - cL.y, gL.y - cF.y, gF.x - cL.x, gL.x - cF.x, a, b,
-                                                 gtab, ltab, alpha_int, alpha);
-            const double m3 = tilted_row_min(sRow, r0, r1, a, b, lbabs, gL.y, gL.x);
-            surv2 = !(rec->mpt8[q] + m2 - m3 + delta < 0.0);
-            if (!surv2) skipped += (u64)(PR_FB * (r1 - r0 + 1));
-        }
-        const unsigned mask2 = __ballot_sync(0xffffffffu, surv2);
-        const int n2 = __popc(mask2);
-        if (n2 >= PR_DENSE) {
-            if (act2 && !surv2) skipped -= (u64)(PR_FB * (r1 - r0 + 1));
-            if (lane == 0) sDense[atomicAdd(sListCount + 1, 1)] = (unsigned short)cb1;
-        } else if (n2) {
-            int slot = 0;
-            if (lane == 0) slot = atomicAdd(sListCount, n2);
-            slot = __shfl_sync(0xffffffffu, slot, 0);
-            if (surv2) sList[slot + __popc(mask2 & ((1u << lane) - 1u))] = (unsigned short)((cb1 << 5) | lane);
-        }
-    };
-    const int l1_warps = min(WD_FARW, (nfar + 31) / 32);
-    const int n_direct = max(0, min(nfar, WD_FARW - l1_warps));
-    const int nfar1 = nfar - n_direct;
-    if (w7 >= l1_warps && w7 - l1_warps < n_direct) level2(nfar - 1 - (w7 - l1_warps));
-
-    for (int base = 0; base + 32 * w7 < nfar1 && w7 < l1_warps; base += 32 * l1_warps) {
-        const int cb = base + 32 * w7 + lane;
-        bool surv1 = false;
-        if (cb < nfar1) {
+        const double t = __dadd_rn(self_score<AI>(a0.C, a0.L, rme, gtab, ltab), a0.P);
+        const bool bad = __any_sync(0xffffffffu, valid && !(t < m));
+        if (lane == 0) {
+            sScal[4 + bi] = ab;
+            vio[bi] = bad;
+            skipc[bi] = 0;
+        }
+    }
+    asm volatile("bar.sync %0, %1;" ::"n"(WD_VER_BAR), "n"(WD_VER * 32) : "memory");
+    double mabs = sScal[1];
+    for (int bi = 0; bi < nb; ++bi) mabs = fmax(mabs, sScal[4 + bi]);
+    const double delta = (sScal[0] + mabs + fabs(pen) * DP_JB) * 5.684341886080802e-14;
+
+    const int total = nb * (kv - BAND_BLOCKS) + nb * (nb - 1) / 2;
+    for (int base = 32 * v; base < total; base += 32 * WD_VER) {
+        const int e = base + lane;
+        bool surv = false;
+        int bi = 0, cb = e;
+        if (e < total) {
+            while (cb >= kv + bi - BAND_BLOCKS) { cb -= kv + bi - BAND_BLOCKS; ++bi; }
+            const int jb = 1 + DP_JB * (kv + bi), nrows = min(DP_JB, N - jb);
+            const int2 rowF = col_lc(sCol, jb), rowL = col_lc(sCol, jb + nrows - 1);
             const CoarseRec *rec = sCoarse + cb;
             const int4 ends = *reinterpret_cast<const int4 *>(rec);
             const double a1 = rec->a, b1 = rec->b;
             const double ub1 = rec->mpt + tilted_box_max<AI>(rowF.y - ends.y, rowL.y - ends.x, rowF.x - ends.w, rowL.x - ends.z,
                                                              a1, b1, gtab, ltab, alpha_int, alpha);
-            const double m3 = tilted_row_min(sRow, 0, nrows - 1, a1, b1, lbabs, rowL.y, rowL.x);
-            surv1 = !(ub1 - m3 + delta < 0.0);
-            if (!surv1) skipped += (u64)(PR_CB * nrows);
-        }
-        const unsigned mask1 = __ballot_sync(0xffffffffu, surv1);
-        if (mask1) {
+            const double m3 = tilted_row_min(sRowV + 32 * bi, 0, nrows - 1, a1, b1, sScal[4 + bi], rowL.y, rowL.x);
+            surv = !(ub1 - m3 + delta < 0.0);
+            if (!surv) atomicAdd(skipc + bi, (unsigned)(PR_CB * nrows));
+        }
+        const unsigned mask = __ballot_sync(0xffffffffu, surv);
+        if (mask) {
             int slot = 0;
-            if (lane == 0) slot = atomicAdd(sListCount + 2, __popc(mask1));
+            if (lane == 0) slot = atomicAdd(sMisc + SY_SURV, __popc(mask));
             slot = __shfl_sync(0xffffffffu, slot, 0);
-            if (surv1) sSurv[slot + __popc(mask1 & ((1u << lane) - 1u))] = (unsigned short)cb;
-        }
-    }
-    PROF_T(4);
-    asm volatile("bar.sync 1, %0;" ::"n"(WD_FARW * 32) : "memory");
-    const int nsurv = *reinterpret_cast<volatile int *>(sListCount + 2);
-
-    for (int e = w7; e < nsurv; e += WD_FARW) level2(sSurv[e]);
-    PROF_T(5);
-    asm volatile("bar.sync 1, %0;" ::"n"(WD_FARW * 32) : "memory");
-    const int total = *reinterpret_cast<volatile int *>(sListCount);
-    const int ndense = *reinterpret_cast<volatile int *>(sListCount + 1);
-    PROF_T(3);
-
-    for (int e = w7; e < ndense; e += WD_FARW) {
-        const int i0 = 1 + PR_CB * (int)sDense[e];
-        const int rr = lane & 3, cph = lane >> 2;
-#pragma unroll 1
-        for (int g = 0; g < 4; ++g) {
-            RowConst<AI> r[2];
-            double bst[2];
-            int ag[2];
-#pragma unroll
-            for (int k = 0; k < 2; ++k) {
-                const int2 rl = col_lc(sCol, min(jb + g * 8 + k * 4 + rr, N - 1));
-                r[k] = make_row<AI>(rl.y, rl.x, alpha_int, alpha);
-                bst[k] = -INFINITY;
-                ag[k] = i0 + cph;
-            }
-            sweep_columns<AI, 4, 2>(i0, i0 + PR_CB, cph, 8, sCol, r, gtab, ltab, bst, ag);
-#pragma unroll
-            for (int k = 0; k < 2; ++k) {
-                merge_column_phases<4>(bst[k], ag[k]);
-                const double v = __shfl_sync(0xffffffffu, bst[k], lane & 3);
-                const int va = __shfl_sync(0xffffffffu, ag[k], lane & 3);
-                if ((lane >> 2) == g * 2 + k && lane < nrows && (v > best || (v == best && va < arg))) { best = v; arg = va; }
-            }
-        }
-    }
-
-    constexpr int UX = 4;
+            if (surv) sSurv[slot + __popc(mask & ((1u << lane) - 1u))] = (unsigned short)((bi << 8) | cb);
+        }
+    }
+    asm volatile("bar.sync %0, %1;" ::"n"(WD_VER_BAR), "n"(WD_VER * 32) : "memory");
+    const int nsurv = vload(sMisc + SY_SURV);
+
+    const int rg = lane >> 2, q = lane & 3;
     const int er = lane >> 3, ec = lane & 7;
-    for (int e0 = w7 * UX; e0 < total; e0 += WD_FARW * UX) {
-        double t[UX];
-        int ta[UX], g4[UX];
-#pragma unroll
-        for (int u = 0; u < UX; ++u) {
-            t[u] = -INFINITY;
-            ta[u] = 0x7fffffff;
-            g4[u] = 0;
-            if (e0 + u < total) {
-                const int ent = sList[e0 + u];
-                const int l2 = ent & 31;
-                g4[u] = 4 * (l2 >> 2);
-                const int row = g4[u] + er;
-                const int col = 1 + PR_CB * (ent >> 5) + PR_FB * (l2 & 3) + ec;
-                ta[u] = col;
-                if (row < nrows) {
-                    const int2 rl = col_lc(sCol, jb + row);
-                    const RowConst<AI> rc = make_row<AI>(rl.y, rl.x, alpha_int, alpha);
-                    const ColRec cc = sCol[col];
-                    t[u] = __dadd_rn(self_score<AI>(cc.C, cc.L, rc, gtab, ltab), cc.P);
-                }
-            }
-        }
-#pragma unroll
-        for (int u = 0; u < UX; ++u) {
-#pragma unroll
-            for (int off = 1; off < 8; off <<= 1) {
-                const double ob = __shfl_xor_sync(0xffffffffu, t[u], off);
-                const int oa = __shfl_xor_sync(0xffffffffu, ta[u], off);
-                if (ob > t[u] || (ob == t[u] && oa < ta[u])) { t[u] = ob; ta[u] = oa; }
-            }
-            const int rel = lane - g4[u];
-            const double v = __shfl_sync(0xffffffffu, t[u], (rel & 3) * 8);
-            const int va = __shfl_sync(0xffffffffu, ta[u], (rel & 3) * 8);
-            if (rel >= 0 && rel < 4 && (v > best || (v == best && va < arg))) { best = v; arg = va; }
-        }
-    }
-    sFarVW[lane] = best;
-    sFarAW[lane] = arg;
-    return skipped;
-}
-
-template <bool AI, int NW>
-__device__ __forceinline__ void near_tri_farwarps(int w7 , int jb, int N, const ColRec *sCol, double *sPartV,
-                                                  int *sPartA, double *sTri,
-                                                  const double *__restrict__ gtab, const double *__restrict__ ltab,
-                                                  int alpha_int, double alpha)
-{
-    const int lane = threadIdx.x & 31;
-    const int rr = lane & 3, cc = lane >> 2;
-    constexpr int NT = (16 + NW - 1) / NW;
-    double tv[NT][2];
-    int tcol[NT];
-#pragma unroll
-    for (int u = 0; u < NT; ++u) {
-        const int t = w7 + u * NW;
-        const int grp = t & 3, qc = (t >> 2) & 3;
-        tcol[u] = jb - PR_CB + qc * 8 + cc;
-        const ColRec a = sCol[tcol[u]];
-#pragma unroll
-        for (int k = 0; k < 2; ++k) {
-            const int j = min(jb + grp * 8 + k * 4 + rr, N - 1);
-            const int2 me = col_lc(sCol, j);
-            const RowConst<AI> r = make_row<AI>(me.y, me.x, alpha_int, alpha);
-            tv[u][k] = (t < 16) ? __dadd_rn(self_score<AI>(a.C, a.L, r, gtab, ltab), a.P) : -INFINITY;
-        }
-    }
-    const int2 mt = col_lc(sCol, min(jb + lane, N - 1));
-    const RowConst<AI> rt = make_row<AI>(mt.y, mt.x, alpha_int, alpha);
-    constexpr int NK = (DP_JB + NW - 1) / NW;
-    double w[NK];
-#pragma unroll
-    for (int kk = 0; kk < NK; ++kk) {
-        const int k = w7 + kk * NW;
-        w[kk] = 0.0;
-        if (k < lane && jb + lane < N) {
-            const int2 a = col_lc(sCol, jb + k);
-            w[kk] = self_score<AI>(a.y, a.x, rt, gtab, ltab);
-        }
-    }
-#pragma unroll
-    for (int u = 0; u < NT; ++u) {
-        const int t = w7 + u * NW;
-#pragma unroll
-        for (int k = 0; k < 2; ++k) {
-            double best = tv[u][k];
-            int arg = tcol[u];
-            merge_column_phases<4>(best, arg);
-            if (cc == 0 && t < 16) {
-                const int row = (t & 3) * 8 + k * 4 + rr;
-                sPartV[(t >> 2) * 32 + row] = best;
-                sPartA[(t >> 2) * 32 + row] = arg;
-            }
-        }
-    }
-#pragma unroll
-    for (int kk = 0; kk < NK; ++kk) {
-        const int k = w7 + kk * NW;
-        if (k < lane && jb + lane < N) sTri[k * DP_JB + lane] = w[kk];
-    }
-}
-
-__device__ __forceinline__ void build_coarse_record(int jb, const ColRec *sCol, CoarseRec *rec, double tilt_scale_c,
-                                                    double tilt_scale_l)
-{
-    const ColRec me = sCol[jb + (threadIdx.x & 31)];
-    fit_column_record(me.C, me.L, me.P, rec, tilt_scale_c, tilt_scale_l);
+    for (int e = v; e < nsurv; e += WD_VER) {
+        const int ent = sSurv[e], bi = ent >> 8, cb = ent & 255;
+        const int jb = 1 + DP_JB * (kv + bi), nrows = min(DP_JB, N - jb);
+        const double *mrow = sRing + ((kv + bi) % RING) * 32;
+        const CoarseRec *rec = sCoarse + cb;
+        const double a = rec->a, b = rec->b;
+        const int r0 = 4 * rg, r1 = min(r0 + 3, nrows - 1);
+        bool surv2 = false;
+        unsigned skip2 = 0;
+        if (r0 < nrows) {
+            const int2 gF = col_lc(sCol, jb + r0), gL = col_lc(sCol, jb + r1);
+            const int i0 = 1 + PR_CB * cb + PR_FB * q;
+            const int2 cF = col_lc(sCol, i0), cL = col_lc(sCol, i0 + PR_FB - 1);
+            const double m2 = tilted_box_max<AI>(gF.y - cL.y, gL.y - cF.y, gF.x - cL.x, gL.x - cF.x, a, b,
+                                                 gtab, ltab, alpha_int, alpha);
+            const double m3 = tilted_row_min(sRowV + 32 * bi, r0, r1, a, b, sScal[4 + bi], gL.y, gL.x);
+            surv2 = !(rec->mpt8[q] + m2 - m3 + delta < 0.0);
+            if (!surv2) skip2 = (unsigned)(PR_FB * (r1 - r0 + 1));
+        }
+        unsigned mask2 = __ballot_sync(0xffffffffu, surv2);
+        bool bad = false;
+        if (__popc(mask2) >= PR_DENSE) {
+            skip2 = 0;
+            if (lane < nrows) {
+                const int2 me = col_lc(sCol, jb + lane);
+                const RowConst<AI> rr = make_row<AI>(me.y, me.x, alpha_int, alpha);
+                const double m = mrow[lane];
+#pragma unroll 8
+                for (int cc = 0; cc < PR_CB; ++cc) {
+                    const ColRec col = sCol[1 + PR_CB * cb + cc];
+                    bad |= !(__dadd_rn(self_score<AI>(col.C, col.L, rr, gtab, ltab), col.P) < m);
+                }
+            }
+        } else {
+            while (mask2) {
+                double t[4], m[4];
+#pragma unroll
+                for (int u = 0; u < 4; ++u) {
+                    t[u] = -INFINITY;
+                    m[u] = INFINITY;
+                    if (mask2) {
+                        const int l2 = __ffs(mask2) - 1;
+                        mask2 &= mask2 - 1;
+                        const int row = 4 * (l2 >> 2) + er;
+                        if (row < nrows) {
+                            const int2 me = col_lc(sCol, jb + row);
+                            const RowConst<AI> rr = make_row<AI>(me.y, me.x, alpha_int, alpha);
+                            const ColRec col = sCol[1 + PR_CB * cb + PR_FB * (l2 & 3) + ec];
+                            t[u] = __dadd_rn(self_score<AI>(col.C, col.L, rr, gtab, ltab), col.P);
+                            m[u] = mrow[row];
+                        }
+                    }
+                }
+#pragma unroll
+                for (int u = 0; u < 4; ++u) bad |= !(t[u] < m[u]);
+            }
+        }
+        if (__any_sync(0xffffffffu, bad) && lane == 0) vio[bi] = 1;
+#pragma unroll
+        for (int off = 16; off > 0; off >>= 1) skip2 += __shfl_xor_sync(0xffffffffu, skip2, off);
+        if (lane == 0 && skip2) atomicAdd(skipc + bi, skip2);
+    }
+    asm volatile("bar.sync %0, %1;" ::"n"(WD_VER_BAR), "n"(WD_VER * 32) : "memory");
+    return kend;
 }
 
 template <bool AI, int U, int RPL, bool PRUNE>
@@ -373,17 +357,15 @@
     const int capr = (p.cap + 31) & ~31;
     ColRec *sCol = reinterpret_cast<ColRec *>(smem);
     double *sPartV = reinterpret_cast<double *>(sCol + capr);
-    double *sTri = sPartV + NEAR_Q * 32;
+    double *sTri = sPartV + 4 * 32;
     int *sPartA = reinterpret_cast<int *>(sTri + DP_JB * DP_JB);
-    int *sMisc = sPartA + NEAR_Q * 32;
-    unsigned short *sPrev = reinterpret_cast<unsigned short *>(sMisc + 24);
+    int *sMisc = sPartA + 4 * 32;
+    unsigned short *sPrev = reinterpret_cast<unsigned short *>(sMisc + SMISC_INTS);
     CoarseRec *sCoarse = reinterpret_cast<CoarseRec *>(sPrev + capr);
-    float4 *sRow = reinterpret_cast<float4 *>(sCoarse + capr / PR_CB);
-    double *sFarV = reinterpret_cast<double *>(sRow + 2 * 32);
-    int *sFarA = reinterpret_cast<int *>(sFarV + 2 * WD_FARW * 32);
-    double *sScal = reinterpret_cast<double *>(sFarA + 2 * WD_FARW * 32);
-    unsigned short *sList = reinterpret_cast<unsigned short *>(sScal + 8);
-    int *sListCount = sMisc + 16;
+    double *sRing = reinterpret_cast<double *>(sCoarse + capr / PR_CB);
+    float4 *sRowV = reinterpret_cast<float4 *>(sRing + RING * 32);
+    double *sScal = reinterpret_cast<double *>(sRowV + VG * 32);
+    unsigned short *sSurv = reinterpret_cast<unsigned short *>(sScal + 16);
     unsigned short *sJump = reinterpret_cast<unsigned short *>(sCoarse);
     unsigned char *sMark = reinterpret_cast<unsigned char *>(sTri);
 
@@ -533,72 +515,103 @@
             for (int off = 16; off > 0; off >>= 1) ab = fmax(ab, __shfl_xor_sync(0xffffffffu, ab, off));
             if (lane == 0) sScal[1] = fmax(sScal[1], ab);
         };
-        auto far_delta = [&]() { return (sScal[0] + sScal[1] + fabs(p.pen) * DP_JB) * 5.684341886080802e-14; };
-        auto prepare_rows = [&](int jbn) {
-            const int par = ((jbn - 1) / DP_JB) & 1;
-            const double delta_path = (sScal[0] + sScal[1] + fabs(p.pen) * DP_JB) * 1.8189894035458565e-12;
-            compute_row_lb<AI>(jbn - DP_JB, jbn, N, sCol, sRow + 32 * par, sScal + 4 + par, delta_path, p.pen, p.gtab, p.ltab,
-                               p.alpha_int, p.alpha);
-            if (lane == 0) { sListCount[4 * par] = 0; sListCount[4 * par + 1] = 0; sListCount[4 * par + 2] = 0; }
-        };
-        auto run_far = [&](int jbf) {
-            const int kf = (jbf - 1) / DP_JB, par = kf & 1;
-            skipped += far_pass<AI>(jbf, N, kf - 1, sCol, sCoarse, sRow + 32 * par, sScal[4 + par], sList, sList + capr,
-                                    sList + capr + capr / PR_CB + 8, sListCount + 4 * par, sFarV + (par * WD_FARW + warp - 1) * 32,
-                                    sFarA + (par * WD_FARW + warp - 1) * 32,
-                                    far_delta(), p.gtab, p.ltab, p.alpha_int, p.alpha PROF_PASS);
-        };
-        int jb = 1;
-        const bool pipelined = PRUNE && N > PR_MIN_N && p.cand != nullptr;
-        for (; jb < N && (!pipelined || jb < 1 + 2 * DP_JB); jb += DP_JB) {
+        auto plain_step = [&](int jb) {
             dp_block_step<AI, WD_WARPS, U, RPL>(jb, N, 0, sCol, sPrev, nullptr, sPartV, sPartA, sTri,
                                                 p.gtab, p.ltab, p.alpha_int, p.alpha, p.pen, -INFINITY, 0, 0);
-            if (pipelined && warp == 0) finish_block(jb);
-        }
-        PROF_T(6);
-        if (pipelined && jb < N) {
-            int spec_wait = 0, spec_back = 1;
-            if (warp == 0) prepare_rows(jb);
+        };
+        const bool pipelined = PRUNE && N > PR_MIN_N && p.cand != nullptr;
+        const int nblk = (N - 1 + DP_JB - 1) / DP_JB;
+        int k0 = 0;
+        for (; k0 < nblk && (!pipelined || k0 < BAND_BLOCKS); ++k0) {
+            plain_step(1 + DP_JB * k0);
+            if (pipelined && warp == 0) finish_block(1 + DP_JB * k0);
+        }
+        PROF_T(4);
+        int rollbacks = 0;
+        while (pipelined && k0 < nblk) {
+            if (tid == 0) {
+                sMisc[SY_CHAIN] = k0;
+                for (int h = 0; h < WD_HELP; ++h) sMisc[SY_BAND + h] = k0;
+                sMisc[SY_REC] = k0;
+                sMisc[SY_VER] = k0;
+                sMisc[SY_ABORT] = -1;
+            }
             __syncthreads();
-            if (warp > 0) run_far(jb);
-            else if (jb + DP_JB < N) prepare_rows(jb + DP_JB);
+            PROF_T(4);
+            if (warp == 0) {
+                for (int k = k0; k < nblk; ++k) {
+                    bool aborted = false;
+                    while (true) {
+                        const bool ready = lane >= WD_HELP || vload(sMisc + SY_BAND + lane) > k;
+                        if (__all_sync(0xffffffffu, ready) && k - vload_warp(sMisc + SY_VER) < RING) break;
+                        if (vload_warp(sMisc + SY_ABORT) >= 0) { aborted = true; break; }
+                    }
+                    if (aborted) break;
+                    __threadfence_block();
+                    PROF_T(3);
+                    const int jb = 1 + DP_JB * k;
+                    double *m = sRing + (k % RING) * 32;
+                    const double ib = sPartV[lane];
+                    const int ia = sPartA[lane];
+                    const bool resolved = p.speculate && block_chain_speculative<0>(jb, N, sCol, sPrev, sPartV, sPartA, sTri, p.pen, ib, ia, m);
+                    if (!resolved) block_chain<0>(jb, N, sCol, sPrev, nullptr, sPartV, sPartA, sTri, p.pen, ib, ia, 0, m);
+                    __syncwarp();
+                    __threadfence_block();
+                    if (lane == 0) vstore(sMisc + SY_CHAIN, k + 1);
+                    PROF_T(1);
+                }
+            } else if (warp <= WD_HELP) {
+                const int h = warp - 1;
+                for (int k = k0; k < nblk; ++k) {
+                    if (!band_help<AI>(h, k, N, sCol, sPartV, sPartA, sTri, sMisc, p.gtab, p.ltab, p.alpha_int, p.alpha)) break;
+                    PROF_T(1);
+                    if (h == 0 && k > k0) {
+                        const int jbr = 1 + DP_JB * (k - 1);
+                        build_coarse_record(jbr, sCol, sCoarse + (k - 1), sScal[2], sScal[3]);
+                        double ab = fabs(sCol[jbr + lane].P);
+#pragma unroll
+                        for (int off = 16; off > 0; off >>= 1) ab = fmax(ab, __shfl_xor_sync(0xffffffffu, ab, off));
+                        if (lane == 0) sScal[1] = fmax(sScal[1], ab);
+                        __syncwarp();
+                        __threadfence_block();
+                        if (lane == 0) vstore(sMisc + SY_REC, k);
+                    }
+                    PROF_T(2);
+                }
+            } else {
+                const int v = warp - 1 - WD_HELP;
+                int par = 0;
+                for (int kv = k0; kv < nblk; par ^= 1) {
+                    const int kend = verify_batch<AI>(v, kv, par, N, sCol, sCoarse, sRing, sRowV, sScal, sSurv, sMisc, p.pen,
+                                                      p.gtab, p.ltab, p.alpha_int, p.alpha);
+                    const int nb = kend - kv;
+                    PROF_T(1);
+                    int pass = 0;
+                    while (pass < nb && !sMisc[SY_VIO + VG * par + pass]) ++pass;
+                    if (v == 0 && lane == 0) {
+                        for (int bi = 0; bi < pass; ++bi) skipped += (unsigned)sMisc[SY_SKIP + VG * par + bi];
+                        __threadfence_block();
+                        vstore(sMisc + SY_VER, kv + pass);
+                        if (pass < nb) vstore(sMisc + SY_ABORT, kv + pass);
+                    }
+                    if (pass < nb) break;
+                    kv = kend;
+                }
+            }
             __syncthreads();
-            for (; jb < N; jb += DP_JB) {
-                const int k = (jb - 1) / DP_JB, buf = k & 1;
-                near_tri_farwarps<AI, WD_WARPS>(warp, jb, N, sCol, sPartV, sPartA, sTri, p.gtab, p.ltab, p.alpha_int, p.alpha);
-                PROF_T(1);
-                __syncthreads();
-                PROF_T(6);
-                if (warp == 0) {
-                    double fbest = -INFINITY;
-                    int farg = 0;
-#pragma unroll
-                    for (int w2 = 0; w2 < WD_FARW; ++w2) {
-                        const double v = sFarV[(buf * WD_FARW + w2) * 32 + lane];
-                        const int a = sFarA[(buf * WD_FARW + w2) * 32 + lane];
-                        if (v > fbest || (v == fbest && a < farg)) { fbest = v; farg = a; }
-                    }
-                    const double ib = jb + lane < N ? fbest : -INFINITY;
-                    const int ia = jb + lane < N ? farg : 0;
-                    bool resolved = false;
-                    if (p.speculate && spec_wait == 0) {
-                        resolved = block_chain_speculative<NEAR_Q>(jb, N, sCol, sPrev, sPartV, sPartA, sTri, p.pen, ib, ia);
-                        if (resolved) spec_back = 1;
-                        else { spec_wait = spec_back; spec_back = min(spec_back * 2, 16); }
-                    } else if (spec_wait > 0) {
-                        --spec_wait;
-                    }
-                    if (!resolved) block_chain<NEAR_Q>(jb, N, sCol, sPrev, nullptr, sPartV, sPartA, sTri, p.pen, ib, ia, 0, nullptr);
-                    __syncwarp();
-                    finish_block(jb);
-                    if (jb + 2 * DP_JB < N) prepare_rows(jb + 2 * DP_JB);
-                } else if (jb + DP_JB < N) {
-                    run_far(jb + DP_JB);
-                }
-                PROF_T(2);
-                __syncthreads();
-                PROF_T(7);
-            }
+            PROF_T(3);
+            const int kf = sMisc[SY_ABORT];
+            if (kf < 0) break;
+            if (tid == 0) atomicAdd(p.rollbacks, 1ull);
+            plain_step(1 + DP_JB * kf);
+            if (warp == 0) finish_block(1 + DP_JB * kf);
+            k0 = kf + 1;
+            if (++rollbacks == MAX_ROLLBACKS) {
+                if (tid == 0) atomicAdd(p.switchovers, 1ull);
+                for (; k0 < nblk; ++k0) plain_step(1 + DP_JB * k0);
+            }
+            __syncthreads();
+            PROF_T(4);
         }
 
         for (int k = tid; k < N; k += WD_THREADS) sMark[k] = (k == N - 1);
@@ -830,10 +843,15 @@
     p.cap = (int)cap;
     p.cells = ctx->scalars.as<u64>() + 10;
     p.cells_skipped = ctx->scalars.as<u64>() + 12;
+    p.rollbacks = ctx->scalars.as<u64>() + 16;
+    p.switchovers = ctx->scalars.as<u64>() + 17;
     p.work_counter = ctx->scalars.as<unsigned>() + 2 * 11;
     p.w_begin = w_begin;
     if (keep_cell_counters) CUDA_TRY(ctx, cudaMemsetAsync(ctx->scalars.as<u64>() + 11, 0, 8, ctx->stream));
-    else CUDA_TRY(ctx, cudaMemsetAsync(ctx->scalars.as<u64>() + 10, 0, 24, ctx->stream));
+    else {
+        CUDA_TRY(ctx, cudaMemsetAsync(ctx->scalars.as<u64>() + 10, 0, 24, ctx->stream));
+        CUDA_TRY(ctx, cudaMemsetAsync(ctx->scalars.as<u64>() + 16, 0, 16, ctx->stream));
+    }
     CUDA_TRY(ctx, cudaMemsetAsync(ctx->scalars.as<u64>() + 15, 0, 8, ctx->stream));
 
     static const int small_env = getenv("PASIO_WD_SMALL") ? atoi(getenv("PASIO_WD_SMALL")) : 1;
@@ -930,15 +948,19 @@
 #ifdef PASIO_WD_PROF
     {
         cudaStreamSynchronize(ctx->stream);
-        unsigned long long h[16], z[16] = {0};
+        unsigned long long h[8 * PROF_SIDES], z[8 * PROF_SIDES] = {0};
         cudaMemcpyFromSymbol(h, g_wd_prof, sizeof h);
         cudaMemcpyToSymbol(g_wd_prof, z, sizeof z);
-        static const char *names[8] = {"compact", "X:work", "Y:work(chain|far L3)", "far:listwait", "far:L1", "far:L2", "wait@X+plain", "wait@Y+rest"};
-        for (int side = 0; side < 2; ++side) {
+        static const char *side_names[PROF_SIDES] = {"chain", "band help", "verify"};
+        static const char *names[PROF_SIDES][8] = {
+            {"compact", "chain", "-", "wait(band|ring)", "plain+rollback", "-", "-", "back-trace+next"},
+            {"compact", "band help", "records", "wait(run end)", "plain+rollback", "-", "-", "back-trace+next"},
+            {"compact", "verify L1+L2+exact", "-", "wait(chain|run end)", "plain+rollback", "-", "-", "back-trace+next"}};
+        for (int side = 0; side < PROF_SIDES; ++side) {
             double tot = 0;
             for (int i = 0; i < 8; ++i) tot += (double)h[8 * side + i];
-            fprintf(stderr, "[wd_prof %s] nwin=%lld grid=%lld:", side ? "warp1" : "warp0", (long long)nwin, (long long)grid);
-            for (int i = 0; i < 8; ++i) if (h[8 * side + i]) fprintf(stderr, " %s=%.1f%%", names[i], 100.0 * (double)h[8 * side + i] / tot);
+            fprintf(stderr, "[wd_prof %s] nwin=%lld grid=%lld:", side_names[side], (long long)nwin, (long long)grid);
+            for (int i = 0; i < 8; ++i) if (h[8 * side + i]) fprintf(stderr, " %s=%.1f%%", names[side][i], 100.0 * (double)h[8 * side + i] / tot);
             fprintf(stderr, " | cycles/CTA=%.3g\n", tot / (double)grid);
         }
     }
```
